# steveschwarcz/Cuda-Path-Tracer-SS

Measured on AMD Instinct MI355X. Metric: Mrays/sec at 1920x1080, 8 bounces, 2072 spp run (BASELINE configs[2] asks 2000 spp; a rate metric); ray = one live ray processed in one bounce, higher is better.
Workload: dtype f32; 1 GPU; configs[2]: 1920x1080 'mixed' preset (22 spheres, 16 triangles, Lambert/Phong/Cook-Torrance/glass/mirror), 8 bounces, 2072 spp = 74 steps x 1 pass(es) x 28 sample lanes per pixel; samples_per_pass=28, frame_lanes=1, lanes_free_run=True, seed=24301

## Files before the change

### cuda-path-tracer-ss_amd/build.py

```python
import os
import shutil
import subprocess
import sys

HERE = os.path.dirname(os.path.abspath(__file__))
ROOT = os.path.dirname(HERE)
INC = os.path.join(ROOT, "include")
CSRC = os.path.join(HERE, "csrc")
HOST = os.path.join(HERE, "host")
LIBDIR = os.path.join(HERE, "lib")

FP_FLAGS = ["-ffp-contract=off", "-fno-fast-math"]
CPU_FLAGS = ["-O2", "-std=c++17", "-fPIC", "-mfma", "-mavx2", "-Wall", "-Wno-unused-function"] + FP_FLAGS
HIP_FLAGS = ["-O3", "-std=c++17", "-fPIC", "--offload-arch=gfx950", "-fhip-fp32-correctly-rounded-divide-sqrt",
             "-fno-gpu-flush-denormals-to-zero", "-fno-slp-vectorize", "-fno-vectorize", "-Wall",
             "-Wno-unused-function"] + FP_FLAGS


def _newer(target, sources):
    if not os.path.exists(target):
        return True
    t = os.path.getmtime(target)
    return any(os.path.getmtime(s) > t for s in sources)


def _run(cmd):
    print("+", " ".join(cmd), flush=True)
    subprocess.check_call(cmd)


def _headers():
    hs = []
    for d in (INC, CSRC, HOST):
        if os.path.isdir(d):
            hs += [os.path.join(d, f) for f in os.listdir(d) if f.endswith(".h")]
    return hs


def build_host(force=False):
    os.makedirs(LIBDIR, exist_ok=True)
    out = os.path.join(LIBDIR, "libptss_host.so")
    srcs = [os.path.join(HOST, f) for f in ("Scene.cpp", "HostOps.cpp", "host_capi.cpp")]
    if force or _newer(out, srcs + _headers()):
        _run(["g++"] + CPU_FLAGS + ["-shared", "-I", INC, "-I", CSRC, "-I", HOST] + srcs + ["-o", out])
    return out


def build_device(force=False, defines=(), name="libptss.so"):
    os.makedirs(LIBDIR, exist_ok=True)
    out = os.path.join(LIBDIR, name)
    srcs = [os.path.join(CSRC, f) for f in sorted(os.listdir(CSRC)) if f.endswith(".hip")]
    hipcc = shutil.which("hipcc") or "/opt/rocm/bin/hipcc"
    if force or _newer(out, srcs + _headers()):
        extra = os.environ.get("PTSS_EXTRA_HIPFLAGS", "").split()
        _run([hipcc] + HIP_FLAGS + extra + ["-D" + d for d in defines] + ["-shared", "-I", INC, "-I", CSRC] + srcs + ["-o", out])
    return out


def build_main(force=False):
    out = os.path.join(LIBDIR, "ptss_main")
    srcs = [os.path.join(HOST, f) for f in ("main.cpp", "CudaTracer.cpp", "MultiGpu.cpp", "Scene.cpp", "HostOps.cpp")]
    if force or _newer(out, srcs + _headers() + [os.path.join(LIBDIR, "libptss.so")]):
        _run(["g++"] + CPU_FLAGS + ["-D__HIP_PLATFORM_AMD__", "-I", INC, "-I", CSRC, "-I", HOST, "-I", "/opt/rocm/include"] + srcs +
             ["-L", LIBDIR, "-lptss", "-L/opt/rocm/lib", "-lamdhip64", "-lrccl", "-Wl,-rpath,$ORIGIN", "-Wl,-rpath,/opt/rocm/lib",
              "-o", out])
    return out


def build_mathcheck(force=False):
    out = os.path.join(LIBDIR, "ptss_mathcheck")
    src = os.path.join(ROOT, "tests", "csrc", "math_exhaustive.hip")
    hipcc = shutil.which("hipcc") or "/opt/rocm/bin/hipcc"
    if force or _newer(out, [src] + _headers()):
        _run([hipcc] + [f for f in HIP_FLAGS if f != "-fPIC"] + ["-I", INC, "-I", CSRC, src, "-o", out])
    return out


def build_all(force=False):
    return [build_host(force), build_device(force), build_main(force), build_mathcheck(force)]


if __name__ == "__main__":
    force = "--force" in sys.argv
    what = [a for a in sys.argv[1:] if not a.startswith("-")]
    table = {"host": build_host, "device": build_device, "main": build_main,
             "mathcheck": build_mathcheck}
    if not what:
        build_all(force)
    for w in what:
        table[w](force)
```

### cuda-path-tracer-ss_amd/csrc/ptmath.h

```cpp
#pragma once
#include <stdint.h>
#include "ptss_types.h"

#if defined(__HIPCC__)
#include <hip/hip_runtime.h>
#define PTM_HD __host__ __device__ __forceinline__
#else
#define PTM_HD inline __attribute__((always_inline))
#endif

namespace ptm {

constexpr float kPi = 3.14159265358979323846f;
constexpr float kInvPi = 0.31830988618f;
constexpr float kRayBump = 1e-4f;
constexpr float kGamma = (1 / 2.2f);

PTM_HD float fma(float a, float b, float c) { return __builtin_fmaf(a, b, c); }
PTM_HD float abs(float x) { return __builtin_fabsf(x); }

#if defined(__HIP_DEVICE_COMPILE__)
PTM_HD unsigned long long lanes(bool directCompare) { return __builtin_amdgcn_ballot_w64(directCompare); }
PTM_HD bool allLanes(unsigned long long m) { return m == __builtin_amdgcn_ballot_w64(true); }
#endif
PTM_HD float sqrt(float x) {
#if defined(__HIP_DEVICE_COMPILE__)
    const float y = __builtin_amdgcn_rsqf(x);
    const float s = x * y;
    const float h = 0.5f * y;
    const float r = __builtin_fmaf(-s, s, x);
    float out = __builtin_fmaf(r, h, s);
    const bool lo = x >= 2.5243549e-29f , hi = x < 7.9228163e28f ;
    if (__builtin_expect(!allLanes(lanes(lo) & lanes(hi)), 0)) out = (lo && hi) ? out : __builtin_sqrtf(x);
    return out;
#else
    return __builtin_sqrtf(x);
#endif
}
PTM_HD float rcp(float x) {
#if defined(__HIP_DEVICE_COMPILE__)
    const float r0 = __builtin_amdgcn_rcpf(x);
    const float e = __builtin_fmaf(-x, r0, 1.0f);
    float out = __builtin_fmaf(e, r0, r0);
    const float ax = __builtin_fabsf(x);
    const bool lo = ax >= 2.3509887e-38f , hi = ax < 8.5070592e37f ;
    if (__builtin_expect(!allLanes(lanes(lo) & lanes(hi)), 0)) out = (lo && hi) ? out : 1.0f / x;
    return out;
#else
    return 1.0f / x;
#endif
}
PTM_HD float rcp_if_above_1em7(float x) {
#if defined(__HIP_DEVICE_COMPILE__)
    const float r0 = __builtin_amdgcn_rcpf(x);
    const float e = __builtin_fmaf(-x, r0, 1.0f);
    float out = __builtin_fmaf(e, r0, r0);
    const bool inRange = __builtin_fabsf(x) < 8.5070592e37f ;
    if (__builtin_expect(!allLanes(lanes(inRange)), 0)) out = inRange ? out : 1.0f / x;
    return out;
#else
    return 1.0f / x;
#endif
}
PTM_HD float rcp_in_range(float x) {
#if defined(__HIP_DEVICE_COMPILE__)
    const float r0 = __builtin_amdgcn_rcpf(x);
    const float e = __builtin_fmaf(-x, r0, 1.0f);
    return __builtin_fmaf(e, r0, r0);
#else
    return 1.0f / x;
#endif
}
PTM_HD uint32_t f2u(float x) { return __builtin_bit_cast(uint32_t, x); }
PTM_HD float u2f(uint32_t x) { return __builtin_bit_cast(float, x); }
PTM_HD float inf() { return u2f(0x7f800000u); }
PTM_HD float qnan() { return u2f(0x7fc00000u); }

#if defined(__HIP_DEVICE_COMPILE__)
PTM_HD bool div_in_range(float x) {
    const float ax = __builtin_fabsf(x);
    return ax >= 8.6736174e-19f  && ax < 1.1529215e18f ;
}
PTM_HD unsigned long long div_range_lanes(float x) {
    const float ax = __builtin_fabsf(x);
    return lanes(ax >= 8.6736174e-19f) & lanes(ax < 1.1529215e18f);
}
PTM_HD float rcp_core(float b) {
    const float r0 = __builtin_amdgcn_rcpf(b);
    const float e = __builtin_fmaf(-b, r0, 1.0f);
    return __builtin_fmaf(e, r0, r0);
}
PTM_HD float div_core(float a, float b, float r) {
    const float q0 = a * r;
    const float rem = __builtin_fmaf(-b, q0, a);
    return __builtin_fmaf(rem, r, q0);
}
#endif
PTM_HD float div(float a, float b) {
#if defined(__HIP_DEVICE_COMPILE__)
    float q = div_core(a, b, rcp_core(b));
    if (__builtin_expect(!allLanes(div_range_lanes(a) & div_range_lanes(b)), 0)) q = (div_in_range(a) && div_in_range(b)) ? q : a / b;
    return q;
#else
    return a / b;
#endif
}
PTM_HD void div3(float ax, float ay, float az, float b, float& qx, float& qy, float& qz) {
#if defined(__HIP_DEVICE_COMPILE__)
    const float r = rcp_core(b);
    qx = div_core(ax, b, r);
    qy = div_core(ay, b, r);
    qz = div_core(az, b, r);
    if (__builtin_expect(!allLanes(div_range_lanes(b) & div_range_lanes(ax) & div_range_lanes(ay) & div_range_lanes(az)), 0)) {
        const bool inRange = div_in_range(b) && div_in_range(ax) && div_in_range(ay) && div_in_range(az);
        qx = inRange ? qx : ax / b;
        qy = inRange ? qy : ay / b;
        qz = inRange ? qz : az / b;
    }
#else
    qx = ax / b;
    qy = ay / b;
    qz = az / b;
#endif
}
PTM_HD float max(float a, float b) { return (a < b) ? b : a; }
PTM_HD float min(float a, float b) { return (b < a) ? b : a; }
PTM_HD float clamp(float x, float lo, float hi) { return min(max(x, lo), hi); }

PTM_HD void sincos(float x, float& s, float& c) {
    if (!(abs(x) <= 1.0e4f)) {
        s = qnan();
        c = qnan();
        return;
    }
    float fn = __builtin_rintf(x * 0.6366197466850281f);
    int n = (int)fn;
    float r = fma(fn, -1.5707963705062866f, x);
    r = fma(fn, 4.371138828673793e-08f, r);
    r = fma(fn, 1.7151245100058819e-15f, r);
    float z = r * r;
    float sp = fma(fma(-1.9515295891e-4f, z, 8.3321608736e-3f), z, -1.6666654611e-1f);
    sp = fma(sp * z, r, r);
    float cp = fma(fma(2.443315711809948e-5f, z, -1.388731625493765e-3f), z, 4.166664568298827e-2f);
    cp = fma(cp * z, z, fma(-0.5f, z, 1.0f));
    float ss = (n & 1) ? cp : sp;
    float cc = (n & 1) ? sp : cp;
    s = (n & 2) ? -ss : ss;
    c = ((n + 1) & 2) ? -cc : cc;
}
PTM_HD float tan(float x) {
    float s, c;
    sincos(x, s, c);
    return div(s, c);
}

PTM_HD float atan(float x) {
    if (x != x) return x;
    float ax = abs(x);
    float y, t;
    if (ax > 2.414213562373095f) {
        y = 1.5707963267948966f;
        t = -rcp(ax);
    } else if (ax > 0.4142135623730950f) {
        y = 0.7853981633974483f;
        t = div(ax - 1.0f, ax + 1.0f);
    } else {
        y = 0.0f;
        t = ax;
    }
    float z = t * t;
    float p = fma(fma(fma(8.05374449538e-2f, z, -1.38776856032e-1f), z, 1.99777106478e-1f), z, -3.33329491539e-1f);
    y = y + fma(p * z, t, t);
    return (x < 0.0f) ? -y : y;
}

PTM_HD float log(float x) {
    if (x != x) return x;
    if (x < 0.0f) return qnan();
    if (x == 0.0f) return -inf();
    if (x == inf()) return x;
    int e = 0;
    if (x < 1.17549435e-38f) {
        x = x * 8388608.0f;
        e = -23;
    }
    uint32_t b = f2u(x);
    e += (int)((b >> 23) & 0xffu) - 126;
    float m = u2f((b & 0x007fffffu) | 0x3f000000u);
    if (m < 0.707106781186547524f) {
        e -= 1;
        m = (m + m) - 1.0f;
    } else {
        m = m - 1.0f;
    }
    float z = m * m;
    float p = 7.0376836292e-2f;
    p = fma(p, m, -1.1514610310e-1f);
    p = fma(p, m, 1.1676998740e-1f);
    p = fma(p, m, -1.2420140846e-1f);
    p = fma(p, m, 1.4249322787e-1f);
    p = fma(p, m, -1.6668057665e-1f);
    p = fma(p, m, 2.0000714765e-1f);
    p = fma(p, m, -2.4999993993e-1f);
    p = fma(p, m, 3.3333331174e-1f);
    float y = (p * m) * z;
    float fe = (float)e;
    y = fma(-2.12194440e-4f, fe, y);
    y = fma(-0.5f, z, y);
    float r = m + y;
    return fma(0.693359375f, fe, r);
}

PTM_HD float exp(float x) {
    if (x != x) return x;
    if (x > 88.72283905206835f) return inf();
    if (x < -87.33654475055310f) return 0.0f;
    float fn = __builtin_rintf(x * 1.4426950216293335f);
    int n = (int)fn;
    float r = fma(fn, -0.693359375f, x);
    r = fma(fn, 2.12194440e-4f, r);
    float z = r * r;
    float p = 1.9875691500e-4f;
    p = fma(p, r, 1.3981999507e-3f);
    p = fma(p, r, 8.3334519073e-3f);
    p = fma(p, r, 4.1665795894e-2f);
    p = fma(p, r, 1.6666665459e-1f);
    p = fma(p, r, 5.0000001201e-1f);
    float y = fma(p, z, r) + 1.0f;
    int h = n / 2;
    float s1 = u2f((uint32_t)(h + 127) << 23);
    float s2 = u2f((uint32_t)((n - h) + 127) << 23);
    return (y * s1) * s2;
}

PTM_HD float pow(float x, float y) {
    if (x != x || y != y) return qnan();
    if (x < 0.0f) return qnan();
    if (y == 0.0f) return 1.0f;
    if (x == 0.0f) return (y > 0.0f) ? 0.0f : inf();
    if (x == 1.0f) return 1.0f;
    return exp(y * log(x));
}

}

namespace ptv {
using vec3 = ::ptss_vec3;
using quat = ::ptss_quat;


PTM_HD vec3 v3(float x, float y, float z) { return vec3{x, y, z}; }
PTM_HD vec3 v3(float s) { return vec3{s, s, s}; }
PTM_HD vec3 operator+(vec3 a, vec3 b) { return vec3{a.x + b.x, a.y + b.y, a.z + b.z}; }
PTM_HD vec3 operator-(vec3 a, vec3 b) { return vec3{a.x - b.x, a.y - b.y, a.z - b.z}; }
PTM_HD vec3 operator-(vec3 a) { return vec3{-a.x, -a.y, -a.z}; }
PTM_HD vec3 operator*(vec3 a, vec3 b) { return vec3{a.x * b.x, a.y * b.y, a.z * b.z}; }
PTM_HD vec3 operator*(vec3 a, float s) { return vec3{a.x * s, a.y * s, a.z * s}; }
PTM_HD vec3 operator*(float s, vec3 a) { return vec3{a.x * s, a.y * s, a.z * s}; }
PTM_HD vec3 operator/(vec3 a, float s) {
    vec3 q;
    ptm::div3(a.x, a.y, a.z, s, q.x, q.y, q.z);
    return q;
}
PTM_HD vec3 madd(vec3 v, float s, vec3 o) { return vec3{ptm::fma(v.x, s, o.x), ptm::fma(v.y, s, o.y), ptm::fma(v.z, s, o.z)}; }
PTM_HD vec3 madd(vec3 a, vec3 b, vec3 o) { return vec3{ptm::fma(a.x, b.x, o.x), ptm::fma(a.y, b.y, o.y), ptm::fma(a.z, b.z, o.z)}; }

PTM_HD float dot(vec3 a, vec3 b) { return ptm::fma(a.z, b.z, ptm::fma(a.y, b.y, a.x * b.x)); }
PTM_HD vec3 cross(vec3 a, vec3 b) {
    return vec3{ptm::fma(a.y, b.z, -(a.z * b.y)), ptm::fma(a.z, b.x, -(a.x * b.z)), ptm::fma(a.x, b.y, -(a.y * b.x))};
}
PTM_HD vec3 normalize(vec3 v) { return v * ptm::rcp(ptm::sqrt(dot(v, v))); }
PTM_HD float length(vec3 v) { return ptm::sqrt(dot(v, v)); }

PTM_HD quat q4(float w, float x, float y, float z) { return quat{x, y, z, w}; }
PTM_HD quat normalize(quat q) {
    float len = ptm::sqrt(ptm::fma(q.w, q.w, ptm::fma(q.z, q.z, ptm::fma(q.y, q.y, q.x * q.x))));
    if (len <= 0.0f) return q4(1, 0, 0, 0);
    float inv = ptm::rcp(len);
    return q4(q.w * inv, q.x * inv, q.y * inv, q.z * inv);
}
PTM_HD vec3 rotate(quat q, vec3 v) {
    vec3 u = v3(q.x, q.y, q.z);
    vec3 uv = cross(u, v);
    vec3 uuv = cross(u, uv);
    uv = uv * (2.0f * q.w);
    uuv = uuv * 2.0f;
    return (v + uv) + uuv;
}
PTM_HD quat mul(quat p, quat q) {
    return q4(p.w * q.w - p.x * q.x - p.y * q.y - p.z * q.z,
              p.w * q.x + p.x * q.w + p.y * q.z - p.z * q.y,
              p.w * q.y + p.y * q.w + p.z * q.x - p.x * q.z,
              p.w * q.z + p.z * q.w + p.x * q.y - p.y * q.x);
}

}
```

### cuda-path-tracer-ss_amd/csrc/ptpack.h

```cpp
#pragma once
#include <stddef.h>
#include <stdint.h>

#include <algorithm>
#include <array>
#include <cmath>
#include <utility>
#include <vector>

#include "ptmath.h"
#include "ptmesh.h"
#include "ptquant.h"
#include "ptscene.h"
#include "ptss_types.h"
#include "pttri.h"

namespace ptpack {
using namespace ptv;
using ptss::SceneLayout;

struct alignas(16) Row {
    float x, y, z, w;
};
static_assert(sizeof(Row) == ptss::kVec4Bytes, "a row is a float4");
// ... 118 lines not shown
            for (size_t q = 0; q < take; ++q) {
                const int b = near[q].second;
                int both[2 * kM], trial[2 * kM], keep[2 * kM];
                for (int j = 0; j < kM; ++j) { both[j] = order[(size_t)a * kM + j]; both[kM + j] = order[(size_t)b * kM + j]; }
                double bestCost = ball[(size_t)a].r * ball[(size_t)a].r + ball[(size_t)b].r * ball[(size_t)b].r;
                const double floor = bestCost * (1 - 1e-9);
                Ball keepA{}, keepB{};
                bool found = false;
                const double join[3] = {ball[(size_t)b].c[0] - ball[(size_t)a].c[0], ball[(size_t)b].c[1] - ball[(size_t)a].c[1], ball[(size_t)b].c[2] - ball[(size_t)a].c[2]};
                const double dirs[7][3] = {{join[0], join[1], join[2]}, {1, 0, 0}, {0, 1, 0}, {0, 0, 1}, {1, 1, 0}, {0, 1, 1}, {1, 0, 1}};
                for (const auto& dir : dirs) {
                    std::copy(both, both + 2 * kM, trial);
                    auto key = [&](int i) { return centre(i, 0) * dir[0] + centre(i, 1) * dir[1] + centre(i, 2) * dir[2]; };
                    std::sort(trial, trial + 2 * kM, [&](int x, int y) { return key(x) < key(y) || (key(x) == key(y) && x < y); });
                    const Ball ta = enclosingBall(s, trial, kM, 48), tb = enclosingBall(s, trial + kM, kM, 48);
                    const double cost = ta.r * ta.r + tb.r * tb.r;
                    if (cost < bestCost && cost < floor) {
                        bestCost = cost; keepA = ta; keepB = tb; found = true;
                        std::copy(trial, trial + 2 * kM, keep);
                    }
                }
                if (found) {
                    for (int j = 0; j < kM; ++j) { order[(size_t)a * kM + j] = keep[j]; order[(size_t)b * kM + j] = keep[kM + j]; }
                    ball[(size_t)a] = keepA; ball[(size_t)b] = keepB;
                    ++improved;
                }
            }
        }
        if (improved == 0) break;
    }
}
inline std::vector<int> spatialOrder(const ptss_scene_desc& s) {
    std::vector<int> order((size_t)s.numSpheres);
    std::vector<Point> centre((size_t)s.numSpheres);
    for (size_t i = 0; i < s.numSpheres; ++i) {
        order[i] = (int)i;
        centre[i] = Point{s.spheres[i].position.x, s.spheres[i].position.y, s.spheres[i].position.z};
    }
    kdOrder(centre, order, 0, (int)s.numSpheres, ptss::kChunkSpheres, 64);
    refineChunks(s, order);
    return order;
}


inline int sphereRowsOf(const SceneLayout& L) { return L.accelSpheres ? L.numChunks * ptss::kChunkSpheres : L.numSpheres; }
inline int sphereAllocOf(const SceneLayout& L) { return L.accelSpheres ? sphereRowsOf(L) : (sphereRowsOf(L) + 3) / 4 * 4; }

inline void setCounts(const ptss_scene_desc& s, bool accel, SceneLayout& L) {
    L.accelSpheres = accel ? 1 : 0;
    L.numChunks = accel ? (int)((s.numSpheres + ptss::kChunkSpheres - 1) / ptss::kChunkSpheres) : 0;
    L.numSpheres = (int)s.numSpheres;
    L.numTriangles = (int)s.numTriangles;
    L.numMaterials = (int)s.numMaterials;
    L.numPointLights = (int)s.numPointLights;
    L.numAreaLights = (int)s.numAreaLights;
}

inline void layoutPlain(const ptss_scene_desc& s, bool accel, SceneLayout& L) {
    setCounts(s, accel, L);
    const int sphereRows = sphereRowsOf(L), sphereAlloc = sphereAllocOf(L);
    int off = 0;
    L.offSphere = off;      off += sphereAlloc;
    if (!accel) { L.offSphereMat = off; off += (sphereRows + 3) / 4; }
    L.offChunk = off;       off += (L.numChunks + 3) / 4 * 4;
    L.offTri = off;         off += 3 * L.numTriangles;
    L.offTriNormal = off;   off += 3 * L.numTriangles;
    L.offTriVert = off;     off += 2 * L.numTriangles;
    L.offMaterial = off;    off += 5 * L.numMaterials;
    L.offPointLight = off;  off += 2 * L.numPointLights;
    L.offAreaLight = off;   off += 2 * L.numAreaLights;
    L.offTriPos = off;      off += (L.numTriangles + 3) / 4;
    L.offQuant = off;       off += ptq::kTableFloats / 4;
    L.offPrimSphere = off;  off += accel ? 0 : sphereAlloc;
    L.offPrimTri = off;     off += 2 * L.numTriangles;
    L.offPrimChunk = off;   off += accel ? (L.numChunks + 3) / 4 * 4 : 0;
    L.ldsVec4 = off;
    if (accel) {
        L.offSphereMat = off;   off += (sphereRows + 3) / 4;
        L.offSphereOrig = off;  off += (sphereRows + 3) / 4;
        L.offSpherePos = off;   off += (L.numSpheres + 3) / 4;
    } else {
        L.offSphereOrig = L.offSpherePos = 0;
    }
    L.totalVec4 = off;
    for (int k = 0; k < 5; ++k) L.triClassPack[k] = 0u;
}

inline void layoutMesh(const ptss_scene_desc& s, SceneLayout& L) {
    setCounts(s, false, L);
    const int sphereRows = sphereRowsOf(L), sphereAlloc = sphereAllocOf(L);
    const int numLeaves = (L.numTriangles + ptss::kMeshLeaf - 1) / ptss::kMeshLeaf;
    const int numGroups = (numLeaves + ptss::kMeshLeaf - 1) / ptss::kMeshLeaf;
    int off = 0;
    L.offSphere = off;      off += sphereAlloc;
    L.offSphereMat = off;   off += (sphereRows + 3) / 4;
    L.offChunk = off;
    const int offGroup = off;   off += 3 * ((numGroups + 3) / 4 * 4);
    const int leafRows = 3 * numLeaves;
    const int rest = 5 * L.numMaterials + 2 * L.numPointLights + 2 * L.numAreaLights + ptq::kTableFloats / 4 + sphereAlloc;
    SceneLayout probe{};
    probe.ldsVec4 = off + leafRows + rest;
    const bool leavesInLds = ptss::bounceLdsBytes(probe, true) <= 64 * 1024;
    int offLeaf = 0;
    if (leavesInLds) { offLeaf = off; off += leafRows; }
    L.offMaterial = off;    off += 5 * L.numMaterials;
    L.offPointLight = off;  off += 2 * L.numPointLights;
    L.offAreaLight = off;   off += 2 * L.numAreaLights;
    L.offQuant = off;       off += ptq::kTableFloats / 4;
    L.offPrimSphere = off;  off += sphereAlloc;
    L.offPrimChunk = off;
    L.ldsVec4 = off;
    if (!leavesInLds) { offLeaf = off; off += leafRows; }
    L.offTri = off;         off += 3 * L.numTriangles;
    L.offTriNormal = off;   off += 3 * L.numTriangles;
    L.offTriVert = off;     off += 2 * L.numTriangles;
    L.offTriPos = off;      off += (L.numTriangles + 3) / 4;
    L.offPrimTri = off;     off += 2 * L.numTriangles;
    L.offSphereOrig = L.offSpherePos = 0;
    L.totalVec4 = off;
    L.mesh.numLeaves = numLeaves;
    L.mesh.numGroups = numGroups;
    L.mesh.offGroup = offGroup;
    L.mesh.offLeaf = offLeaf;
    L.mesh.reserved = 0;
}

inline void setFlags(const ptss_scene_desc& s, SceneLayout& L) {
    auto finite3 = [](const ptss_vec3& v) { return v.x - v.x == 0.0f && v.y - v.y == 0.0f && v.z - v.z == 0.0f; };
    L.neeSkipSafe = 1;
    for (size_t i = 0; i < s.numMaterials; ++i)
        if (!finite3(s.materials[i].diffuseColor) || !(s.materials[i].diffAvg - s.materials[i].diffAvg == 0.0f)) L.neeSkipSafe = 0;
    for (size_t i = 0; i < s.numPointLights; ++i)
        if (!finite3(s.pointLights[i].power)) L.neeSkipSafe = 0;
    for (size_t i = 0; i < s.numAreaLights; ++i)
        if (!finite3(s.areaLights[i].power)) L.neeSkipSafe = 0;
    L.sphereBounded = geometryBounded(s) ? 1 : 0;
    {
        size_t diffuse = 0;
        for (size_t i = 0; i < s.numSpheres; ++i) diffuse += s.materials[s.spheres[i].materialIdx].diffAvg > 0.0f ? 1 : 0;
        for (size_t i = 0; i < s.numTriangles; ++i) diffuse += s.materials[s.triangles[i].materialIdx].diffAvg > 0.0f ? 1 : 0;
        L.neePairs = (L.sphereBounded && s.numPointLights + s.numAreaLights >= 2 && 5 * diffuse >= 4 * (s.numSpheres + s.numTriangles)) ? 1 : 0;
    }
    L.triDetBounded = 1;
    for (size_t i = 0; i < s.numTriangles; ++i) {
        const ptss_triangle& t = s.triangles[i];
        const vec3 e1 = t.vertex1 - t.vertex0, e2 = t.vertex2 - t.vertex0;
        const double n1 = std::sqrt((double)e1.x * e1.x + (double)e1.y * e1.y + (double)e1.z * e1.z);
        const double n2 = std::sqrt((double)e2.x * e2.x + (double)e2.y * e2.y + (double)e2.z * e2.z);
        if (!(n1 * n2 <= 0x1p100)) L.triDetBounded = 0;
    }
    L.triClassed = (L.triDetBounded && L.sphereBounded && L.numTriangles <= 255) ? 1 : 0;
}

inline std::vector<int> orderTriangles(const ptss_scene_desc& s, SceneLayout& L) {
    std::vector<int> triOrder((size_t)L.numTriangles), triCode((size_t)L.numTriangles, 0);
    for (int i = 0; i < L.numTriangles; ++i) {
        triOrder[(size_t)i] = i;
        const ptss_triangle& t = s.triangles[i];
        if (L.triClassed) triCode[(size_t)i] = pttri::triangleClass(t.vertex1 - t.vertex0, t.vertex2 - t.vertex0);
    }
    std::stable_sort(triOrder.begin(), triOrder.end(), [&](int a, int b) { return triCode[(size_t)a] < triCode[(size_t)b]; });
    for (int code = 0, pos = 0; code <= 16 && L.triClassed; ++code) {
        while (pos < L.numTriangles && triCode[(size_t)triOrder[(size_t)pos]] < code) ++pos;
        L.triClassPack[code / 4] |= (uint32_t)pos << (8 * (code % 4));
    }
    if (ptss::meshImage(L)) {
        std::vector<Point> centroid((size_t)L.numTriangles);
        for (int i = 0; i < L.numTriangles; ++i) {
            const ptss_triangle& t = s.triangles[i];
            for (int a = 0; a < 3; ++a) {
                const float* v0 = &t.vertex0.x, *v1 = &t.vertex1.x, *v2 = &t.vertex2.x;
                centroid[(size_t)i][a] = (float)(((double)v0[a] + v1[a] + v2[a]) / 3);
            }
        }
        kdOrder(centroid, triOrder, 0, L.numTriangles, ptss::kMeshLeaf, ptss::kMeshLeaf * ptss::kMeshLeaf);
    }
    return triOrder;
}

inline std::vector<int> packSpheres(const ptss_scene_desc& s, const SceneLayout& L, std::vector<Row>& blob) {
    const bool accel = L.accelSpheres != 0;
    const int sphereRows = sphereRowsOf(L);
    std::vector<int> order;
    if (accel) {
        order = spatialOrder(s);
        while ((int)order.size() < sphereRows) order.push_back(order.back());
    } else {
        order.resize(s.numSpheres);
        for (size_t i = 0; i < s.numSpheres; ++i) order[i] = (int)i;
    }
    for (int i = 0; i < sphereRows; ++i) {
        const ptss_sphere& sp = s.spheres[order[i]];
        blob[L.offSphere + i] = Row{sp.position.x, sp.position.y, sp.position.z, sp.radius * sp.radius};
        intsAt(blob, L.offSphereMat)[i] = sp.materialIdx;
        if (accel) intsAt(blob, L.offSphereOrig)[i] = order[i];
        if (accel && i < L.numSpheres) intsAt(blob, L.offSpherePos)[order[i]] = i;
    }
    return order;
}

inline void packChunkBounds(const ptss_scene_desc& s, const SceneLayout& L, const std::vector<int>& order, std::vector<Row>& blob) {
    for (int k = 0; k < L.numChunks; ++k) {
        const Ball ball = enclosingBall(s, &order[(size_t)k * ptss::kChunkSpheres], ptss::kChunkSpheres, 512);
        const float Cf[3] = {(float)ball.c[0], (float)ball.c[1], (float)ball.c[2]};
        double Rmax = 0;
        for (int j = 0; j < ptss::kChunkSpheres; ++j) {
            const ptss_sphere& sp = s.spheres[order[k * ptss::kChunkSpheres + j]];
            const double dx = (double)sp.position.x - Cf[0], dy = (double)sp.position.y - Cf[1], dz = (double)sp.position.z - Cf[2];
            Rmax = std::max(Rmax, std::sqrt(dx * dx + dy * dy + dz * dz) + std::fabs((double)sp.radius));
        }
        const double infl = Rmax * Rmax * (1 + kAccelM) * (1 + kAccelM) * (1 + kAccelM) * (1 + 4e-6) / (1 - (kAccelM + kAccelM * kAccelM)) * (1 + 1e-9);
        blob[L.offChunk + k] = Row{Cf[0], Cf[1], Cf[2], std::nextafter((float)infl, INFINITY)};
    }
}

inline void packTriangles(const ptss_scene_desc& s, const SceneLayout& L, const std::vector<int>& triOrder, std::vector<Row>& blob) {
    for (int pos = 0; pos < L.numTriangles; ++pos) {
        const int i = triOrder[(size_t)pos];
        const ptss_triangle& t = s.triangles[i];
        const vec3 e1 = t.vertex1 - t.vertex0;
        const vec3 e2 = t.vertex2 - t.vertex0;
        blob[L.offTri + 3 * pos + 0] = Row{t.vertex0.x, t.vertex0.y, t.vertex0.z, u2f((uint32_t)t.materialIdx)};
        blob[L.offTri + 3 * pos + 1] = Row{e1.x, e1.y, e1.z, u2f(0xfffffffeu - (uint32_t)i)};
        blob[L.offTri + 3 * pos + 2] = Row{e2.x, e2.y, e2.z, 0};
        blob[L.offTriNormal + 3 * pos + 0] = Row{t.normal0.x, t.normal0.y, t.normal0.z, 0};
        blob[L.offTriNormal + 3 * pos + 1] = Row{t.normal1.x, t.normal1.y, t.normal1.z, 0};
        blob[L.offTriNormal + 3 * pos + 2] = Row{t.normal2.x, t.normal2.y, t.normal2.z, 0};
        blob[L.offTriVert + 2 * pos + 0] = Row{t.vertex1.x, t.vertex1.y, t.vertex1.z, 0};
        blob[L.offTriVert + 2 * pos + 1] = Row{t.vertex2.x, t.vertex2.y, t.vertex2.z, 0};
        intsAt(blob, L.offTriPos)[i] = pos;
    }
}

inline void packMeshBounds(const ptss_scene_desc& s, const SceneLayout& L, const std::vector<int>& triOrder, std::vector<Row>& blob) {
    auto boundOf = [&](int first, int count, Row* rows) {
        std::vector<float> tri((size_t)count * 9);
        for (int k = 0; k < count; ++k) {
            const ptss_triangle& t = s.triangles[triOrder[(size_t)(first + k)]];
            const vec3 e1 = t.vertex1 - t.vertex0, e2 = t.vertex2 - t.vertex0;
            const float v[9] = {t.vertex0.x, t.vertex0.y, t.vertex0.z, e1.x, e1.y, e1.z, e2.x, e2.y, e2.z};
            std::copy(v, v + 9, tri.begin() + 9 * k);
        }
        float b[12];
        ptmesh::buildBound(tri.data(), count, b);
        for (int r = 0; r < 3; ++r) rows[r] = Row{b[4 * r], b[4 * r + 1], b[4 * r + 2], b[4 * r + 3]};
    };
    constexpr int kGroupTris = ptss::kMeshLeaf * ptss::kMeshLeaf;
    for (int k = 0; k < L.mesh.numLeaves; ++k)
        boundOf(k * ptss::kMeshLeaf, std::min(ptss::kMeshLeaf, L.numTriangles - k * ptss::kMeshLeaf), &blob[(size_t)(L.mesh.offLeaf + 3 * k)]);
    for (int g = 0; g < L.mesh.numGroups; ++g)
        boundOf(g * kGroupTris, std::min(kGroupTris, L.numTriangles - g * kGroupTris), &blob[(size_t)(L.mesh.offGroup + 3 * g)]);
}

inline void packMaterialsAndLights(const ptss_scene_desc& s, const SceneLayout& L, std::vector<Row>& blob) {
    for (int i = 0; i < L.numMaterials; ++i) {
        const ptss_material& m = s.materials[i];
        Row* o = &blob[L.offMaterial + 5 * i];
        o[0] = Row{m.diffuseColor.x, m.diffuseColor.y, m.diffuseColor.z, m.diffAvg};
        o[1] = Row{m.specularColor.x, m.specularColor.y, m.specularColor.z, m.specAvg};
        o[2] = Row{m.absorption.x, m.absorption.y, m.absorption.z, m.refrAvg};
        o[3] = Row{m.emmitance.x, m.emmitance.y, m.emmitance.z, m.roughness};
        o[4] = Row{m.specularExponent, m.indexOfRefraction, u2f((uint32_t)(unsigned char)m.flags), 0};
    }
    for (int i = 0; i < L.numPointLights; ++i) {
        const ptss_point_light& p = s.pointLights[i];
        blob[L.offPointLight + 2 * i + 0] = Row{p.position.x, p.position.y, p.position.z, 0};
        blob[L.offPointLight + 2 * i + 1] = Row{p.power.x, p.power.y, p.power.z, 0};
    }
    for (int i = 0; i < L.numAreaLights; ++i) {
        const ptss_area_light& a = s.areaLights[i];
        const int* triPos = intsAt(blob, L.offTriPos);
        blob[L.offAreaLight + 2 * i] = Row{a.power.x, a.power.y, a.power.z, u2f((uint32_t)triPos[a.triangleIdx])};
        blob[L.offAreaLight + 2 * i + 1] = Row{u2f((uint32_t)triPos[a.triangleIdx + 1]), 0, 0, 0};
    }
}

inline void packScene(const ptss_scene_desc& s, SceneLayout& L, std::vector<Row>& blob, bool accel, bool mesh) {
    if (mesh) layoutMesh(s, L);
    else layoutPlain(s, accel, L);
    setFlags(s, L);
    const std::vector<int> triOrder = orderTriangles(s, L);
    blob.assign((size_t)L.totalVec4 + 1, Row{0, 0, 0, 0});
    ptq::build_thresholds(reinterpret_cast<float*>(&blob[L.offQuant]));
    const std::vector<int> sphereOrder = packSpheres(s, L, blob);
    packChunkBounds(s, L, sphereOrder, blob);
    packTriangles(s, L, triOrder, blob);
    if (mesh) packMeshBounds(s, L, triOrder, blob);
    packMaterialsAndLights(s, L, blob);
}

struct ImagePlan {
    bool accel, mesh;
    int numImages;
};
inline ImagePlan planImages(const ptss_scene_desc& s, bool everySphereLoop) {
    const bool accel = accelEligible(s) && !everySphereLoop;
    const bool mesh = !accel && meshEligible(s) && !everySphereLoop;
    return ImagePlan{accel, mesh, accel ? 2 : 1};
}
struct PackedImage {
    SceneLayout layout{};
    std::vector<Row> blob;
    bool inLds = true;
};
inline std::vector<PackedImage> packImages(const ptss_scene_desc& s, bool everySphereLoop) {
    const ImagePlan plan = planImages(s, everySphereLoop);
// ... 26 lines not shown
```

### cuda-path-tracer-ss_amd/csrc/ptscene.h

```cpp
#pragma once
#include <stddef.h>
#include <stdint.h>

#if defined(__HIPCC__)
#define PTSCENE_HD __host__ __device__
#else
#define PTSCENE_HD
#endif

namespace ptss {

#ifndef PTSS_BLOCK
#define PTSS_BLOCK 256
#endif
#ifndef PTSS_CHUNK
#define PTSS_CHUNK 16
#endif
constexpr int kBlock = PTSS_BLOCK;
constexpr int kChunkSpheres = PTSS_CHUNK;
static_assert((kChunkSpheres & (kChunkSpheres - 1)) == 0, "chunk size must be a power of two");
constexpr int kWaves = kBlock / 64;

struct SceneLayout {
    int numSpheres, numTriangles, numMaterials, numPointLights, numAreaLights;
    int offSphere;
    int offSphereMat;
    int offTri;
    int offTriNormal;
    int offTriVert;
    int offMaterial;
    int offPointLight;
    int offAreaLight;
    int accelSpheres;
    int numChunks;
    int offChunk;
    int offSphereOrig;
    int offSpherePos;
    int offQuant;
    int offPrimSphere;
    int offPrimTri;
    int offPrimChunk;
    int totalVec4;
    int ldsVec4;
    int neeSkipSafe;
    int sphereBounded;
    int neePairs;
    int triDetBounded;
    int triClassed;
    union {
        uint32_t triClassPack[5];
        struct {
            int numLeaves, numGroups;
            int offGroup;
            int offLeaf;
            int reserved;
        } mesh;
    };
    int offTriPos;
};

constexpr int kMeshLeaf = 16;
PTSCENE_HD inline bool meshImage(const SceneLayout& L) { return !L.triClassed && L.mesh.numLeaves > 0; }

constexpr int kNeeLights = 2;
constexpr int kQueueCap = kNeeLights * 64;
constexpr int kWaveLdsWords = 8 * kQueueCap + kNeeLights * 64 / 4;
constexpr int kBlockScratchVec4 = 4;
constexpr int kBlockLdsVec4 = kBlockScratchVec4 + (kWaves * kWaveLdsWords + 3) / 4;

constexpr size_t kVec4Bytes = 16;
inline size_t bounceLdsBytes(const SceneLayout& layout, bool sceneInLds) {
    return ((sceneInLds ? (size_t)layout.ldsVec4 : 0) + kBlockLdsVec4) * kVec4Bytes;
}

}
```

### cuda-path-tracer-ss_amd/csrc/ptshade.h

```cpp
#pragma once
#include "ptaccel.h"
#include "ptquant.h"
#include "ptraypool.h"

namespace ptss {
namespace {

__device__ __forceinline__ void addLambertTerm(vec3& radiance, float cosI, vec3 power, float distance2,
                                               float4 diffuse ) {
    const vec3 L_i = power / (float)(4 * ptm::kPi * distance2);
    radiance.x += cosI * L_i.x * diffuse.x * diffuse.w * ptm::kInvPi;
    radiance.y += cosI * L_i.y * diffuse.y * diffuse.w * ptm::kInvPi;
    radiance.z += cosI * L_i.z * diffuse.z * diffuse.w * ptm::kInvPi;
}

__device__ __forceinline__ quat rotateVectorToVector(vec3 source, vec3 target) {
    const vec3 axis = cross(source, target);
    return normalize(q4(1.0f + dot(source, target), axis.x, axis.y, axis.z));
}

enum LobeKind { kLobeNone = 0, kLobeLambert = 1, kLobePhong = 2, kLobeBeckmann = 3 };

__device__ __forceinline__ vec3 scatter(const float4* mat, RayRegs& ray, vec3 point, vec3 normal, float cosI) {
    const float4 mDiffuse = mat[0];
    const float4 mSpecular = mat[1];
    const float4 mMisc = mat[4];
    const float refrAvg = mat[2].w;
    const int flags = (int)asU(mMisc.z);

    float r = ptrng::uniform(ray.rng);
    PTSS_DIAG_SCATTER(0, true);

    int kind = kLobeNone;
    bool decided = false;
    vec3 axis = normal;
    vec3 result = v3(0, 0, 0);
    const vec3 incident = ray.d;

    if (mDiffuse.w > 0.0f) {
        r -= mDiffuse.w;
        if (r < 0.0f) {
            ray.o = point + ptm::kRayBump * normal;
            kind = kLobeLambert;
            decided = true;
            result = xyz(mDiffuse);
        }
    }

    PTSS_DIAG_SCATTER(1, !decided);
    if (!decided) {
        float n1, n2;
        if (cosI > 0) {
            n2 = mMisc.y;
            n1 = 1.0f;
        } else {
            cosI = -cosI;
            n1 = mMisc.y;
            n2 = 1.0f;
        }
        const bool readsFresnel = (mSpecular.w > 0.0f && !(flags & PTSS_MAT_FLAG_PURE_REFLECTION)) || refrAvg > 0.0f;
        float n = 0.0f, sinT2 = 0.0f;
        float fresnelReflective = 1.0f;
        PTSS_DIAG_SCATTER(2, readsFresnel);
        if (readsFresnel) {
            n = ptm::div(n1, n2);
            sinT2 = n * n * (1.0f - cosI * cosI);
        }
        if (readsFresnel && !(sinT2 > 1.0f)) {
            const float cosT = ptm::sqrt(1.0f - sinT2);
            const float r_s = ptm::div(n1 * cosI - n2 * cosT, n1 * cosI + n2 * cosT);
            const float r_p = ptm::div(n2 * cosI - n1 * cosT, n2 * cosI + n1 * cosT);
            fresnelReflective = (r_s * r_s + r_p * r_p) * 0.5f;
        }

        if (mSpecular.w > 0.0f) {
            if (flags & PTSS_MAT_FLAG_PURE_REFLECTION)
                r -= mSpecular.w;
            else
                r -= mSpecular.w * fresnelReflective;

            if (r < 0.0f) {
                decided = true;
                if (flags & PTSS_MAT_FLAG_COOK_TORRANCE) {
                    kind = kLobeBeckmann;
                } else {
                    ray.d = ray.d - (2 * (-cosI)) * normal;
                    ray.o = point + (normal * ptm::kRayBump);
                    if (mMisc.x != ptm::inf()) {
                        kind = kLobePhong;
                        axis = ray.d;
                    }
                    result = xyz(mSpecular);
                }
            }
        }

        if (!decided && refrAvg > 0.0f) {
            const float fresnelRefractive = 1.0f - fresnelReflective;
            r -= refrAvg * fresnelRefractive;
            PTSS_DIAG_SCATTER(3, r < 0.0f);
            if (r < 0.0f) {
                decided = true;
                if (sinT2 > 1.0f) ray.active = false;
                const float cosT = ptm::sqrt(1.0f - sinT2);
                const vec3 w_o = normalize(n * ray.d + (n * cosI - cosT) * normal);
                ray.o = point + (w_o * ptm::kRayBump);
                ray.d = w_o;
                result = v3(1, 1, 1);
            }
        }

        if (!decided) ray.active = false;
    }

    PTSS_DIAG_SCATTER(4, kind != kLobeNone);
    PTSS_DIAG_SCATTER(5, kind == kLobeBeckmann);
    PTSS_DIAG_SCATTER(6, kind == kLobePhong);
    PTSS_DIAG_SCATTER(7, kind == kLobeLambert);
    if (kind != kLobeNone) {
        const float u1 = ptrng::uniform(ray.rng);
        const float u2 = ptrng::uniform(ray.rng);
        float azimuth, a, y;
        if (kind == kLobeBeckmann) {
            const float roughness = mat[3].w;
            const float theta = ptm::atan(-roughness * roughness * ptm::log(1.0f - u1));
            azimuth = u2 * 2 * ptm::kPi;
            ptm::sincos(theta, a, y);
        } else {
            azimuth = u1 * 2 * ptm::kPi;
            y = (kind == kLobeLambert) ? ptm::sqrt(u2) : ptm::pow(u2, ptm::rcp(mMisc.x + 1));
            a = ptm::sqrt(1 - y * y);
        }
        float sn, cs;
        ptm::sincos(azimuth, sn, cs);
        const vec3 sampled = rotate(rotateVectorToVector(v3(0, 1, 0), axis), v3(a * cs, y, a * sn));
        if (kind == kLobeBeckmann) {
            const vec3 beckmannNormal = sampled;
            const float cosB = ptm::abs(dot(ray.d, beckmannNormal));
            ray.d = ray.d - (2 * (-cosB)) * beckmannNormal;
            ray.o = point + (beckmannNormal * ptm::kRayBump);

            const vec3 half = normalize(ray.d - incident);
            const float nh = ptm::abs(dot(normal, half));
            const float nl = ptm::abs(dot(normal, ray.d));
            const float vh = ptm::abs(dot(incident, half));
            const float nv = ptm::abs(cosI);
            const float geometric = ptm::min(ptm::min(1.0f, ptm::div(2 * nh * nl, vh)), ptm::div(2 * nh * nv, vh));
            result = xyz(mSpecular) * geometric / nv;
        } else {
            ray.d = sampled;
        }
    }
    return result;
}

__device__ __forceinline__ uint32_t quantizeSample(float radiance, const float* T) { return ptq::quantize_fast(radiance, T); }

__device__ __forceinline__ void loadHome(const uint32_t* __restrict__ home, uint32_t p, ptrng::State& s) {
    const uint4 a = reinterpret_cast<const uint4*>(home)[2 * p];
    const uint4 b = reinterpret_cast<const uint4*>(home)[2 * p + 1];
    s.v[0] = a.x; s.v[1] = a.y; s.v[2] = a.z; s.v[3] = a.w;
    s.v[4] = b.x; s.d = b.y;
}
__device__ __forceinline__ void storeHome(uint32_t* __restrict__ home, uint32_t p, const ptrng::State& s) {
    reinterpret_cast<uint4*>(home)[2 * p] = uint4{s.v[0], s.v[1], s.v[2], s.v[3]};
    reinterpret_cast<uint4*>(home)[2 * p + 1] = uint4{s.v[4], s.d, 0u, 0u};
}

struct U3 {
    uint32_t x, y, z;
};

__device__ __forceinline__ void finishPath(const FrameBuffers& fb, const RayRegs& r, const float* quantT) {
    const uint32_t p = pixOf(r.pix), lane = laneOf(r.pix);
    const uint32_t stream = lane * fb.plane + p;
    const uint32_t qx = quantizeSample(r.L0.x, quantT), qy = quantizeSample(r.L0.y, quantT), qz = quantizeSample(r.L0.z, quantT);
    if (fb.samples == 1) {
        U3* acc = reinterpret_cast<U3*>(fb.accum) + p;
        U3 t = *acc;
        t.x += qx;
        t.y += qy;
        t.z += qz;
        *acc = t;
        if (fb.pixels) {
            const uint32_t px = (uint32_t)(unsigned char)(t.x * fb.inverseTicks + 0.5f) |
                                ((uint32_t)(unsigned char)(t.y * fb.inverseTicks + 0.5f) << 8) |
                                ((uint32_t)(unsigned char)(t.z * fb.inverseTicks + 0.5f) << 16) | (255u << 24);
            reinterpret_cast<uint32_t*>(fb.pixels)[p] = px;
        }
    } else {
        fb.staged[stream] = qx | (qy << 8) | (qz << 16);
    }
    if (fb.fsum) {
        float* fs = fb.fsum + 3u * stream;
        fs[0] += r.L0.x;
        fs[1] += r.L0.y;
        fs[2] += r.L0.z;
    }
    storeHome(fb.rngHome, stream, r.rng);
}

constexpr unsigned long long kPeerWaitTicks = 200000000ull;
__device__ __forceinline__ bool peerWaitExpired(unsigned long long& since) {
    const unsigned long long now = wall_clock64();
    if (since == 0ull) {
        since = now | 1ull;
        return false;
    }
    return now > since && now - since > kPeerWaitTicks;
}

__device__ __forceinline__ uint32_t frameLiveCount(const FrameBuffers& fb, int bounce, uint32_t own, const uint32_t* target) {
    uint32_t total = own;
    for (uint32_t p = 0; p < fb.numPeers; ++p) {
        unsigned long long since = 0ull;
        for (;;) {
            uint32_t ended = 0;
            for (int s = 0; s < kShards; ++s)
                ended += __hip_atomic_load(fb.peerDone[p] + countIndex(bounce - 1, s), __ATOMIC_ACQUIRE, __HIP_MEMORY_SCOPE_AGENT);
            if ((int32_t)(ended - target[p]) >= 0) break;
            __builtin_amdgcn_s_sleep(64);
            if (peerWaitExpired(since)) {
                if (threadIdx.x == 0) atomicAdd(fb.guardTimeouts, 1u);
                break;
            }
        }
        for (int s = 0; s < kShards; ++s)
            total += __hip_atomic_load(fb.peerCounts[p] + countIndex(bounce, s), __ATOMIC_RELAXED, __HIP_MEMORY_SCOPE_AGENT);
    }
    return total;
}

}
}
```

### cuda-path-tracer-ss_amd/csrc/ptss_api.hip

```cpp
#include <stdio.h>
#include <stdlib.h>
#include <string.h>

#include <new>
#include <string>
#include <vector>

#include "ptss.h"
#include "ptss_device.h"
#include <algorithm>
#include "ptdenoise.h"
#include "ptreproject.h"
#include "ptspecular.h"
#include "ptpack.h"

using namespace ptv;
using ptpack::cameraInRange;
static_assert(sizeof(ptpack::Row) == sizeof(float4) && alignof(ptpack::Row) == alignof(float4), "a packed row is uploaded as a float4");

#if PTSS_DIAG
namespace ptss { hipError_t readDiagCounters(unsigned long long* out8); }
#endif
namespace {

thread_local std::string g_detail;

int fail(int code, const char* what, hipError_t e = hipSuccess) {
    char buf[512];
    if (e != hipSuccess)
        snprintf(buf, sizeof(buf), "%s: %s (%s)", what, hipGetErrorString(e), hipGetErrorName(e));
    else
        snprintf(buf, sizeof(buf), "%s", what);
    g_detail = buf;
    return code;
}

#define HIP_TRY(expr)                                        \
    do {                                                     \
        hipError_t _e = (expr);                              \
        if (_e != hipSuccess) return fail(PTSS_EHIP, #expr, _e); \
    } while (0)

#define RC_TRY(expr) do { if (int _rc = (expr)) return _rc; } while (0)

struct EventPair {
    hipEvent_t a, b;
};

}

struct Lane {
    hipStream_t stream = nullptr;
    float* dPool[2] = {nullptr, nullptr};
    uint32_t* dCounts[2] = {nullptr, nullptr};
    uint32_t* dShardCount0 = nullptr;
    uint32_t* dLastCounts = nullptr;
    uint32_t* dDone = nullptr;
    uint32_t doneTarget[ptss::kMaxBounces + 1] = {};
    hipEvent_t evDone[2] = {nullptr, nullptr};
    uint32_t regionCap = 0;
    int maxBlocks = 0;
    uint32_t hint[ptss::kMaxBounces + 1] = {0};
    bool haveHint = false;
    uint32_t* hCounts = nullptr;
    hipEvent_t hintEvent[4] = {nullptr, nullptr, nullptr, nullptr};
    bool hintPending[4] = {false, false, false, false};
};

struct SceneImage {
    float4* dBlob = nullptr;
    ptss::SceneLayout layout{};
    bool inLds = true;
    bool oneLaunch = false;
};

struct ptss_context {
    ptss_render_config cfg{};
    hipStream_t stream = nullptr;
    ptss::TileMap tile{};
    SceneImage images[2];
    int active = 0;
    const SceneImage& image() const { return images[active]; }
    std::vector<Lane> lanes;
    hipEvent_t evFork = nullptr;
    int countParity = 0;
    uint32_t* dRngHome = nullptr;
    unsigned long long* dTotal = nullptr;
    uint32_t* dAccumOwned = nullptr;
    uint32_t* dAccum = nullptr;
    float* dFsum = nullptr;
    uint32_t* dStaged = nullptr;
    bool stagedTwice = false;
    hipEvent_t evDisplay[2] = {nullptr, nullptr};
    uint32_t capacity = 0, numPixels = 0;
    uint32_t samples = 1;
    bool cameraDirty = true;
    float defaultColor[3] = {0, 0, 0};
    ptss_camera camera{};
    int lastResetTick = 0;
    int lastTicks = 0;
    unsigned maxIterations = 15;
    bool resetTicksThisFrame = true;
    bool usePathTracer = true;
    hipEvent_t evStart = nullptr, evStop = nullptr;
    float lastMs = 0.0f;
    int gridCap = 0;
    unsigned frameIndex = 0;
    std::vector<EventPair> evFree, evBusy;
    std::vector<std::pair<double, double>> kernelSpans;
    hipEvent_t evEpoch = nullptr;
    unsigned int timeoutsSeen = 0;
    unsigned long long launchedKernels = 0;
    unsigned long long specularFeatureLaunches[2] = {0, 0};
    float4* dDenoise[2] = {nullptr, nullptr};
    int denoiseLastPlane = -1;
    int denoiseLastLevel = -1;
    hipStream_t denoiseStream = nullptr;
    int numCUs = 0;
    hipStream_t updateStream = nullptr;
    bool updated = false;
};
constexpr int kTotalWords = ptss::kMaxLanes + 8 + 1;
constexpr int kRejectedWord = ptss::kMaxLanes;

namespace {

int validateScene(const ptss_scene_desc& s) {
    const char* what = ptpack::validateScene(s);
    return what ? fail(PTSS_EINVAL, what) : PTSS_OK;
}

int localRows(const ptss_render_config& cfg) {
    int rows = 0;
    for (int y = 0; y < cfg.height; ++y)
        if ((y / cfg.bandRows) % cfg.tileWorld == cfg.tileRank) ++rows;
    return rows;
}

int createCheck(hipError_t e, const char* what) { return e == hipSuccess ? PTSS_OK : fail(e == hipErrorOutOfMemory ? PTSS_ENOMEM : PTSS_EHIP, what, e); }
#define ALLOC_TRY(expr) RC_TRY(createCheck((expr), #expr))
template <class T>
hipError_t mallocZeroed(T** p, size_t bytes) {
    const hipError_t e = hipMalloc(p, bytes);
    return e == hipSuccess ? hipMemset(*p, 0, bytes) : e;
}

struct SceneState {
    SceneImage images[2];
    int gridCap = 0;
    float defaultColor[3] = {0, 0, 0};
};
void releaseSceneState(SceneState& st) {
    for (SceneImage& im : st.images) {
        (void)hipFree(im.dBlob);
        im = SceneImage{};
    }
}
int buildSceneState(const ptss_scene_desc& scene, const ptss_render_config& cfg, int numLanes, int maxBlocks0, int numCUs, SceneState& st) {
    std::vector<ptpack::PackedImage> packed;
    try {
        packed = ptpack::packImages(scene, cfg.everySphereLoop != 0);
    } catch (const std::bad_alloc&) {
        return fail(PTSS_ENOMEM, "scene image (host)");
    }
    const int numImages = (int)packed.size();
    for (int i = 0; i < numImages; ++i) {
        SceneImage& im = st.images[i];
        im.layout = packed[(size_t)i].layout;
        im.inLds = packed[(size_t)i].inLds;
        const std::vector<ptpack::Row>& blob = packed[(size_t)i].blob;
        hipError_t e = hipMalloc(&im.dBlob, blob.size() * sizeof(float4));
        if (e == hipSuccess) e = hipMemcpy(im.dBlob, blob.data(), blob.size() * sizeof(float4), hipMemcpyHostToDevice);
        if (e != hipSuccess) {
            releaseSceneState(st);
            return createCheck(e, "scene image (device)");
        }
    }
    st.defaultColor[0] = scene.defaultColor.x;
    st.defaultColor[1] = scene.defaultColor.y;
    st.defaultColor[2] = scene.defaultColor.z;
    const SceneImage& primary = st.images[0];
    const int perCU = ptss::bounceOccupancyBlocksPerCU(primary.layout, primary.inLds, primary.layout.sphereBounded != 0);
    st.gridCap = numCUs * (perCU > 0 ? perCU : 4) * 16 / ptss::kShards;
    auto qualifies = [&](const SceneImage& im) {
        if (cfg.oneLaunchFrames <= 0 || numLanes != 1 || !im.inLds) return false;
        if (ptss::meshImage(im.layout)) return false;
        int perCU = ptss::frameOccupancyBlocksPerCU(im.layout, false);
        if (im.layout.sphereBounded) perCU = std::min(perCU, ptss::frameOccupancyBlocksPerCU(im.layout, true));
        const int resident = perCU - 1;
        return resident >= 1 && maxBlocks0 <= numCUs * resident;
    };
    for (int i = 0; i < numImages; ++i) st.images[i].oneLaunch = qualifies(st.images[i]);
#ifdef PTSS_TUNING_KNOBS
    if (const char* e = getenv("PTSS_SCENE_PATH")) {
        if (!strcmp(e, "scalar"))
            for (int i = 0; i < numImages; ++i) st.images[i].inLds = false;
    }
    if (const char* e = getenv("PTSS_GRID_CAP")) st.gridCap = atoi(e);
#endif
    return PTSS_OK;
}
void adoptSceneState(ptss_context* c, const SceneState& st) {
    for (int i = 0; i < 2; ++i) c->images[i] = st.images[i];
    c->gridCap = st.gridCap;
    for (int k = 0; k < 3; ++k) c->defaultColor[k] = st.defaultColor[k];
    c->active = 0;
}

int allocLane(Lane& ln, const uint32_t (&shardCount0)[ptss::kShards], bool ownStream) {
    const size_t poolBytes = (size_t)ptss::kRayPlanes * ln.regionCap * ptss::kShards * sizeof(float);
    for (float*& pool : ln.dPool) ALLOC_TRY(hipMalloc(&pool, poolBytes));
    for (uint32_t*& counts : ln.dCounts) ALLOC_TRY(mallocZeroed(&counts, ptss::kCountWords * sizeof(uint32_t)));
    ALLOC_TRY(mallocZeroed(&ln.dLastCounts, ptss::kCountWords * sizeof(uint32_t)));
    for (int s = 0; s < ptss::kShards; ++s)
        ALLOC_TRY(hipMemcpy(ln.dCounts[0] + ptss::countIndex(0, s), &shardCount0[s], sizeof(uint32_t), hipMemcpyHostToDevice));
    ALLOC_TRY(hipMalloc(&ln.dShardCount0, sizeof(shardCount0)));
    ALLOC_TRY(hipMemcpy(ln.dShardCount0, shardCount0, sizeof(shardCount0), hipMemcpyHostToDevice));
    ALLOC_TRY(mallocZeroed(&ln.dDone, (ptss::kCountWords + ptss::kCountStride) * sizeof(uint32_t)));
    if (ownStream) {
        ALLOC_TRY(hipStreamCreateWithFlags(&ln.stream, hipStreamNonBlocking));
        for (hipEvent_t& ev : ln.evDone) ALLOC_TRY(hipEventCreateWithFlags(&ev, hipEventDisableTiming));
    }
    ALLOC_TRY(hipHostMalloc(&ln.hCounts, 4 * ptss::kCountWords * sizeof(uint32_t), hipHostMallocDefault));
    for (hipEvent_t& ev : ln.hintEvent) ALLOC_TRY(hipEventCreateWithFlags(&ev, hipEventDisableTiming));
    return PTSS_OK;
}
#undef ALLOC_TRY

hipError_t seedStreams(ptss_context* c, unsigned long long seed, hipStream_t st) {
    std::vector<uint32_t> table(ptrng::kJumpTableWords);
    ptrng::build_subsequence_table(table.data());
    uint32_t* dTable = nullptr;
    hipError_t e = hipMalloc(&dTable, table.size() * sizeof(uint32_t));
    if (e != hipSuccess) return e;
    e = hipMemcpy(dTable, table.data(), table.size() * sizeof(uint32_t), hipMemcpyHostToDevice);
    if (e == hipSuccess && c->numPixels > 0) e = ptss::launchRngInit(st, c->dRngHome, c->capacity, c->samples, c->tile, seed, dTable);
    if (e == hipSuccess) e = hipStreamSynchronize(st);
    (void)hipFree(dTable);
    return e;
}

int quiesce(ptss_context* c) {
    HIP_TRY(hipStreamSynchronize(c->stream));
    for (const Lane& ln : c->lanes)
        if (ln.stream) HIP_TRY(hipStreamSynchronize(ln.stream));
    return PTSS_OK;
}

void releaseLane(Lane& ln) {
    for (hipEvent_t ev : ln.hintEvent)
        if (ev) (void)hipEventDestroy(ev);
    if (ln.hCounts) (void)hipHostFree(ln.hCounts);
    (void)hipFree(ln.dDone);
    for (hipEvent_t ev : ln.evDone)
        if (ev) (void)hipEventDestroy(ev);
    if (ln.stream) (void)hipStreamDestroy(ln.stream);
    for (float* pool : ln.dPool) (void)hipFree(pool);
    for (uint32_t* counts : ln.dCounts) (void)hipFree(counts);
    (void)hipFree(ln.dShardCount0);
    (void)hipFree(ln.dLastCounts);
}

ptss::FrameBuffers frameBuffers(const ptss_context* c, int laneIdx, ptss_uchar4* pixels, int sample) {
    const Lane& ln = c->lanes[(size_t)laneIdx];
    ptss::FrameBuffers fb{};
    fb.pool[0] = ln.dPool[0];
    fb.pool[1] = ln.dPool[1];
    fb.rngHome = c->dRngHome;
    fb.counts = ln.dCounts[c->countParity];
    fb.countsNext = ln.dCounts[1 - c->countParity];
    fb.shardCount0 = ln.dShardCount0;
    fb.lastCounts = ln.dLastCounts;
    fb.totalRayBounces = c->dTotal + laneIdx;
    fb.guardTimeouts = reinterpret_cast<uint32_t*>(c->dTotal + ptss::kMaxLanes + 8);
    fb.accum = c->dAccum;
    fb.fsum = c->dFsum;
    fb.staged = c->dStaged ? c->dStaged + (c->stagedTwice ? (size_t)(c->frameIndex & 1u) * c->capacity * c->samples : 0) : nullptr;
    fb.quantTable = reinterpret_cast<const float*>(c->image().dBlob + c->image().layout.offQuant);
    fb.pixels = pixels;
    fb.regionCap = ln.regionCap;
    fb.numPixels = c->numPixels;
    fb.plane = c->capacity;
    fb.samples = c->samples;
    fb.firstTiles = c->samples * (c->capacity / ptss::kBlock);
    fb.minLive = c->tile.world > 1 ? 0u : ptss::kMinLiveRays;
    fb.inverseTicks = 1.f / (float)((int)c->samples * (sample + 1));
    fb.defaultColor[0] = c->defaultColor[0];
    fb.defaultColor[1] = c->defaultColor[1];
    fb.defaultColor[2] = c->defaultColor[2];
    fb.laneIndex = (uint32_t)laneIdx;
    fb.laneCount = (uint32_t)c->lanes.size();
    fb.frameRays = c->numPixels * c->samples;
    fb.numPeers = fb.laneCount - 1;
    fb.myDone = ln.dDone;
    fb.myFrameDone = ln.dDone + ptss::kCountWords;
    fb.frameSeq = c->frameIndex;
    fb.joinsFrame = (laneIdx + 1 == (int)c->lanes.size()) ? 1u : 0u;
    uint32_t p = 0;
    for (size_t k = 0; k < c->lanes.size(); ++k) {
        if ((int)k == laneIdx) continue;
        fb.peerCounts[p] = c->lanes[k].dCounts[c->countParity];
        fb.peerDone[p] = c->lanes[k].dDone;
        fb.peerFrameDone[p] = c->lanes[k].dDone + ptss::kCountWords;
        ++p;
    }
    return fb;
}

void drainKernelEvents(ptss_context* c, bool wait) {
    size_t k = 0;
    for (size_t i = 0; i < c->evBusy.size(); ++i) {
        EventPair p = c->evBusy[i];
        hipError_t q = wait ? hipEventSynchronize(p.b) : hipEventQuery(p.b);
        if (q == hipSuccess) {
            float start = 0, ms = 0;
            if (hipEventElapsedTime(&start, c->evEpoch, p.a) == hipSuccess && hipEventElapsedTime(&ms, p.a, p.b) == hipSuccess)
            {
                if (c->kernelSpans.size() >= (1u << 20)) c->kernelSpans.clear();
                c->kernelSpans.emplace_back((double)start, (double)start + (double)ms);
            }
            c->evFree.push_back(p);
        } else {
            c->evBusy[k++] = p;
        }
    }
    c->evBusy.resize(k);
    (void)hipGetLastError();
}

int checkLaneTimeouts(ptss_context* c) {
    if (c->lanes.size() < 2 && !c->images[0].oneLaunch && !c->images[1].oneLaunch) return PTSS_OK;
    uint32_t v = 0;
    HIP_TRY(hipMemcpy(&v, c->dTotal + ptss::kMaxLanes + 8, sizeof(v), hipMemcpyDeviceToHost));
    if (v != c->timeoutsSeen) {
        c->timeoutsSeen = v;
        return fail(PTSS_ETIMEOUT, "a bounded wait on the device expired (a frame lane for a peer lane, or a workgroup of the one-launch "
                                   "frame kernel for its shard): the frame was not traced as specified");
    }
    return PTSS_OK;
}

void selectImage(ptss_context* c) {
    if (!c->images[1].dBlob) return;
    const int want = cameraInRange(c->camera) ? 0 : 1;
    if (want != c->active) {
        c->active = want;
        c->cameraDirty = true;
    }
}

ptss::EyeParams eyeParams(const ptss_context* c) {
    return {c->camera, -2 * ptm::tan(c->camera.fieldOfView * 0.5f), (float)c->tile.height / (float)c->tile.width, 1.0f / c->tile.width,
            1.0f / c->tile.height};
}

void harvestHints(ptss_context* c) {
    for (Lane& ln : c->lanes)
        for (int q = 0; q < 4; ++q) {
            if (!ln.hintPending[q] || hipEventQuery(ln.hintEvent[q]) != hipSuccess) continue;
            const uint32_t* src = ln.hCounts + (size_t)q * ptss::kCountWords;
            for (int b = 0; b <= ptss::kMaxBounces; ++b) {
                uint32_t mx = 0;
                for (int s = 0; s < ptss::kShards; ++s) mx = std::max(mx, src[ptss::countIndex(b, s)]);
                ln.hint[b] = mx;
            }
            ln.haveHint = true;
            ln.hintPending[q] = false;
        }
    (void)hipGetLastError();
}

int forkLanes(ptss_context* c, bool forkNeeded) {
    if (c->lanes.size() > 1 && (forkNeeded || c->frameIndex == 0 || !c->cfg.lanesFreeRun)) {
        HIP_TRY(hipEventRecord(c->evFork, c->stream));
        for (Lane& ln : c->lanes) HIP_TRY(hipStreamWaitEvent(ln.stream, c->evFork, 0));
    }
    if (c->stagedTwice && c->frameIndex >= 2)
        for (Lane& ln : c->lanes) HIP_TRY(hipStreamWaitEvent(ln.stream, c->evDisplay[c->frameIndex & 1u], 0));
    return PTSS_OK;
}

template <class Launch>
int timedLaunch(ptss_context* c, hipStream_t s, Launch launch) {
    if (!c->cfg.timeKernels) return launch();
    EventPair ev{nullptr, nullptr};
    if (c->evFree.empty() && c->evBusy.size() >= 4096) drainKernelEvents(c, true);
    if (c->evFree.empty()) {
        HIP_TRY(hipEventCreate(&ev.a));
        HIP_TRY(hipEventCreate(&ev.b));
    } else {
        ev = c->evFree.back();
        c->evFree.pop_back();
    }
    HIP_TRY(hipEventRecord(ev.a, s));
    RC_TRY(launch());
    HIP_TRY(hipEventRecord(ev.b, s));
    c->evBusy.push_back(ev);
    return PTSS_OK;
}

int traceOneLaunch(ptss_context* c, const ptss::FrameBuffers& fb, int numIterations, bool bounded, const ptss::EyeParams& eye) {
    const SceneImage& im = c->image();
    return timedLaunch(c, c->stream, [&] {
        HIP_TRY(ptss::launchFrame(c->stream, fb, im.dBlob, im.layout, numIterations, bounded, c->lanes[0].maxBlocks, c->tile, eye,
                                          &c->launchedKernels));
        return PTSS_OK;
    });
}

int traceBounces(ptss_context* c, ptss::FrameBuffers* fbs, int numIterations, bool bounded, const ptss::EyeParams& eye) {
    const SceneImage& im = c->image();
    const int K = (int)c->lanes.size();
    for (int i = 0; i < numIterations; ++i)
        for (int k = 0; k < K; ++k) {
            Lane& ln = c->lanes[(size_t)k];
            const hipStream_t ls = K > 1 ? ln.stream : c->stream;
            int blocks = ln.maxBlocks;
            if (i > 0 && ln.haveHint) {
                const unsigned long long tilesPerShard = ((unsigned long long)ln.hint[i] * 65 / 64 + ptss::kBlock) / ptss::kBlock + 1;
                const unsigned long long want = tilesPerShard * ptss::kShards;
                if (want < (unsigned long long)blocks) blocks = (int)want;
            }
            if (c->gridCap > 0 && c->gridCap * ptss::kShards < blocks) blocks = c->gridCap * ptss::kShards;
            if (i > 0)
                for (int j = 0, p = 0; j < K; ++j)
                    if (j != k) fbs[k].peerTarget[p++] = c->lanes[(size_t)j].doneTarget[i - 1];
            RC_TRY(timedLaunch(c, ls, [&] {
                HIP_TRY(ptss::launchBounce(ls, fbs[k], im.dBlob, im.layout, i, i == numIterations - 1, im.inLds, bounded, blocks, c->tile, eye,
                                               &c->launchedKernels));
                return PTSS_OK;
            }));
            ln.doneTarget[i] += (uint32_t)blocks;
        }
    return PTSS_OK;
}

int flushAndJoin(ptss_context* c, const ptss::FrameBuffers* fbs, int numIterations) {
    const int K = (int)c->lanes.size();
    for (int k = 0; k < K; ++k) {
        Lane& ln = c->lanes[(size_t)k];
        const hipStream_t ls = K > 1 ? ln.stream : c->stream;
        ptss::FlushTargets targets{};
// ... 319 lines not shown
    HIP_TRY(hipMalloc(out, (size_t)c->capacity * sizeof(ptss_uchar4)));
    HIP_TRY(hipMemset(*out, 0, (size_t)c->capacity * sizeof(ptss_uchar4)));
    return PTSS_OK;
}

int ptss_free_pixels(ptss_context* c, ptss_uchar4* dev) {
    if (!c) return fail(PTSS_EINVAL, "ctx is null");
    HIP_TRY(hipFree(dev));
    return PTSS_OK;
}

int ptss_local_pixels(const ptss_context* c, size_t* out) {
    if (!c || !out) return fail(PTSS_EINVAL, "null argument");
    *out = c->numPixels;
    return PTSS_OK;
}

int ptss_local_rows(const ptss_context* c, int* rows, int cap, int* count) {
    if (!c || !count) return fail(PTSS_EINVAL, "null argument");
    int n = 0;
    for (int y = 0; y < c->tile.height; ++y) {
        if ((y / c->tile.bandRows) % c->tile.world != c->tile.rank) continue;
        if (rows) {
            if (n >= cap) return fail(PTSS_ERANGE, "rows[] too small");
            rows[n] = y;
        }
        ++n;
    }
    *count = n;
    return PTSS_OK;
}

int ptss_synchronize(ptss_context* c) {
    if (!c) return fail(PTSS_EINVAL, "ctx is null");
    HIP_TRY(hipStreamSynchronize(c->stream));
    return checkLaneTimeouts(c);
}

int ptss_read_accumulator(ptss_context* c, uint32_t* host, size_t count) {
    if (!c || !host) return fail(PTSS_EINVAL, "null argument");
    if (count != (size_t)3 * c->numPixels) return fail(PTSS_ERANGE, "count must be 3 * local pixels");
    HIP_TRY(hipStreamSynchronize(c->stream));
    HIP_TRY(hipMemcpy(host, c->dAccum, count * sizeof(uint32_t), hipMemcpyDeviceToHost));
    return checkLaneTimeouts(c);
}

int ptss_read_float_accumulator(ptss_context* c, float* host, size_t count) {
    if (!c || !host) return fail(PTSS_EINVAL, "null argument");
    if (!c->dFsum) return fail(PTSS_EINVAL, "context was created without floatAccumulator");
    if (count != (size_t)3 * c->numPixels) return fail(PTSS_ERANGE, "count must be 3 * local pixels");
    HIP_TRY(hipStreamSynchronize(c->stream));
    if (c->samples == 1) {
        HIP_TRY(hipMemcpy(host, c->dFsum, count * sizeof(float), hipMemcpyDeviceToHost));
    } else {
        std::vector<float> lane(count);
        for (size_t k = 0; k < count; ++k) host[k] = 0.0f;
        for (uint32_t l = 0; l < c->samples; ++l) {
            HIP_TRY(hipMemcpy(lane.data(), c->dFsum + (size_t)3 * l * c->capacity, count * sizeof(float), hipMemcpyDeviceToHost));
            for (size_t k = 0; k < count; ++k) host[k] = host[k] + lane[k];
        }
    }
    return checkLaneTimeouts(c);
}

int ptss_read_pixels(ptss_context* c, const ptss_uchar4* dev, ptss_uchar4* host, size_t count) {
    if (!c || !dev || !host) return fail(PTSS_EINVAL, "null argument");
    if (count > c->numPixels) return fail(PTSS_ERANGE, "count exceeds local pixels");
    HIP_TRY(hipStreamSynchronize(c->stream));
    HIP_TRY(hipMemcpy(host, dev, count * sizeof(ptss_uchar4), hipMemcpyDeviceToHost));
    return checkLaneTimeouts(c);
}

int ptss_read_rng_state(ptss_context* c, size_t local_pixel, uint32_t* out6) { return ptss_read_rng_state_lane(c, local_pixel, 0, out6); }

int ptss_read_rng_state_lane(ptss_context* c, size_t local_pixel, unsigned int lane, uint32_t* out6) {
    if (!c || !out6) return fail(PTSS_EINVAL, "null argument");
    if (local_pixel >= c->numPixels || lane >= c->samples) return fail(PTSS_ERANGE, "pixel or lane out of range");
    HIP_TRY(hipStreamSynchronize(c->stream));
    HIP_TRY(hipMemcpy(out6, c->dRngHome + (size_t)ptss::kHomeWords * ((size_t)lane * c->capacity + local_pixel), 6 * sizeof(uint32_t),
                      hipMemcpyDeviceToHost));
    return PTSS_OK;
}

int ptss_last_pass_ms(ptss_context* c, float* out) {
    if (!c || !out) return fail(PTSS_EINVAL, "null argument");
    *out = c->lastMs;
    return PTSS_OK;
}

int ptss_samples_since_reset(const ptss_context* c, int* out) {
    if (!c || !out) return fail(PTSS_EINVAL, "null argument");
    *out = c->resetTicksThisFrame ? 0 : (c->lastTicks - c->lastResetTick + 1) * (int)c->samples;
    return PTSS_OK;
}

int ptss_live_counts(ptss_context* c, uint32_t* out, int cap, int* n) {
    if (!c || !out || !n) return fail(PTSS_EINVAL, "null argument");
    const int numIterations = c->usePathTracer ? (int)c->maxIterations : 1;
    if (cap < numIterations) return fail(PTSS_ERANGE, "out[] too small");
    std::vector<uint32_t> raw(ptss::kCountWords), sum(ptss::kCountWords, 0u);
    HIP_TRY(hipStreamSynchronize(c->stream));
    for (const Lane& ln : c->lanes) {
        HIP_TRY(hipMemcpy(raw.data(), ln.dLastCounts, raw.size() * sizeof(uint32_t), hipMemcpyDeviceToHost));
        for (size_t k = 0; k < raw.size(); ++k) sum[k] += raw[k];
    }
    bool stopped = false;
    for (int i = 0; i < numIterations; ++i) {
        uint32_t total = 0;
        for (int s = 0; s < ptss::kShards; ++s) total += sum[ptss::countIndex(i, s)];
        if (total <= (c->tile.world > 1 ? 0u : ptss::kMinLiveRays)) stopped = true;
        out[i] = stopped ? 0u : total;
    }
    *n = numIterations;
    return checkLaneTimeouts(c);
}

int ptss_total_ray_bounces(ptss_context* c, unsigned long long* out) {
    if (!c || !out) return fail(PTSS_EINVAL, "null argument");
    HIP_TRY(hipStreamSynchronize(c->stream));
    unsigned long long perLane[ptss::kMaxLanes];
    HIP_TRY(hipMemcpy(perLane, c->dTotal, sizeof(perLane), hipMemcpyDeviceToHost));
    *out = 0;
    for (size_t k = 0; k < c->lanes.size(); ++k) *out += perLane[k];
    return checkLaneTimeouts(c);
}

int ptss_guard_timeouts(ptss_context* c, unsigned int* out) {
    if (!c || !out) return fail(PTSS_EINVAL, "null argument");
    HIP_TRY(hipStreamSynchronize(c->stream));
    uint32_t v = 0;
    HIP_TRY(hipMemcpy(&v, c->dTotal + ptss::kMaxLanes + 8, sizeof(v), hipMemcpyDeviceToHost));
    *out = v;
    return PTSS_OK;
}

int ptss_one_launch_frames(const ptss_context* c, int* out) {
    if (!c || !out) return fail(PTSS_EINVAL, "null argument");
    *out = (c->image().oneLaunch && c->lanes.size() == 1) ? 1 : 0;
    return PTSS_OK;
}

int ptss_frame_lanes(const ptss_context* c, int* out) {
    if (!c || !out) return fail(PTSS_EINVAL, "null argument");
    *out = (int)c->lanes.size();
    return PTSS_OK;
}

int ptss_launched_kernels(const ptss_context* c, unsigned long long* out) {
    if (!c || !out) return fail(PTSS_EINVAL, "null argument");
    *out = c->launchedKernels;
    return PTSS_OK;
}

static int rayQuery(ptss_context* c, bool any, const ptss_ray_query* rays, void* out, size_t n, void* hipStream) {
    if (!c) return fail(PTSS_EINVAL, "ctx is null");
    if (n == 0) return PTSS_OK;
    if (!rays || !out) return fail(PTSS_EINVAL, "null buffer with n > 0");
    if (n >= (size_t(1) << 31)) return fail(PTSS_ERANGE, "n must be below 2^31");
    if (((uintptr_t)rays | (uintptr_t)out) & (any ? 3u : 15u) || (uintptr_t)rays & 15u)
        return fail(PTSS_EINVAL, "rays and hits must be 16-byte aligned, verdicts 4-byte aligned");
    const SceneImage& im = c->images[0];
    if (!im.dBlob) return fail(PTSS_EINVAL, "context has no scene image");
    HIP_TRY(hipSetDevice(c->cfg.device));
    hipStream_t st = hipStream ? static_cast<hipStream_t>(hipStream) : c->stream;
    HIP_TRY(ptss::launchQuery(st, any, im.dBlob, im.layout, im.inLds, rays, out, (uint32_t)n, c->gridCap * ptss::kShards,
                              &c->launchedKernels));
    return PTSS_OK;
}

int ptss_intersect(ptss_context* c, const ptss_ray_query* dev_rays, ptss_ray_hit* dev_hits, size_t n, void* hipStream) {
    return rayQuery(c, false, dev_rays, dev_hits, n, hipStream);
}

int ptss_occluded(ptss_context* c, const ptss_ray_query* dev_rays, uint32_t* dev_occluded, size_t n, void* hipStream) {
    return rayQuery(c, true, dev_rays, dev_occluded, n, hipStream);
}

int ptss_render_features(ptss_context* c, ptss_pixel_feature* dev_features, void* hipStream) {
    if (!c) return fail(PTSS_EINVAL, "ctx is null");
    if (!dev_features) return fail(PTSS_EINVAL, "dev_features is null");
    if ((uintptr_t)dev_features & 15u) return fail(PTSS_EINVAL, "dev_features must be 16-byte aligned");
    if (c->numPixels == 0) return PTSS_OK;
    const SceneImage& im = c->images[0];
    if (!im.dBlob) return fail(PTSS_EINVAL, "context has no scene image");
    HIP_TRY(hipSetDevice(c->cfg.device));
    hipStream_t st = hipStream ? static_cast<hipStream_t>(hipStream) : c->stream;
    const ptss_vec3 defaultColor{c->defaultColor[0], c->defaultColor[1], c->defaultColor[2]};
    HIP_TRY(ptss::launchFeatures(st, im.dBlob, im.layout, im.inLds, c->tile, eyeParams(c), defaultColor, dev_features, c->numPixels,
                                 c->gridCap * ptss::kShards, &c->launchedKernels));
    return PTSS_OK;
}

int ptss_render_features_motion(ptss_context* c, const ptss_triangle* dev_triangles_prev, size_t first, size_t count,
                                ptss_pixel_feature* dev_features, ptss_pixel_motion* dev_motion, void* hipStream) {
    if (!c) return fail(PTSS_EINVAL, "ctx is null");
    if (!dev_features || !dev_motion) return fail(PTSS_EINVAL, "dev_features or dev_motion is null");
    if (count > 0 && !dev_triangles_prev) return fail(PTSS_EINVAL, "dev_triangles_prev is null with count > 0");
    if (((uintptr_t)dev_features | (uintptr_t)dev_motion) & 15u) return fail(PTSS_EINVAL, "dev_features and dev_motion must be 16-byte aligned");
    if ((uintptr_t)dev_triangles_prev & 3u) return fail(PTSS_EINVAL, "dev_triangles_prev must be 4-byte aligned");
    if (count > 0) {
        const size_t T = (size_t)c->images[0].layout.numTriangles;
        if (first >= T || count > T - first) return fail(PTSS_ERANGE, "first .. first + count - 1 leaves the scene's triangles");
    }
    if (c->numPixels == 0) return PTSS_OK;
    const SceneImage& im = c->images[0];
    if (!im.dBlob) return fail(PTSS_EINVAL, "context has no scene image");
    HIP_TRY(hipSetDevice(c->cfg.device));
    hipStream_t st = hipStream ? static_cast<hipStream_t>(hipStream) : c->stream;
    const ptss_vec3 defaultColor{c->defaultColor[0], c->defaultColor[1], c->defaultColor[2]};
    HIP_TRY(ptss::launchFeaturesMotion(st, im.dBlob, im.layout, im.inLds, c->tile, eyeParams(c), defaultColor, dev_features, c->numPixels,
                                       c->gridCap * ptss::kShards, dev_triangles_prev, count ? (uint32_t)first : 0u, (uint32_t)count, dev_motion,
                                       &c->launchedKernels));
    return PTSS_OK;
}

int ptss_render_features_specular(ptss_context* c, int maxSteps, ptss_pixel_feature* dev_features, uint32_t* dev_steps, void* hipStream) {
    if (!c) return fail(PTSS_EINVAL, "ctx is null");
    if (!dev_features) return fail(PTSS_EINVAL, "dev_features is null");
    if (maxSteps < 0 || maxSteps > ptsp::kMaxSteps) return fail(PTSS_EINVAL, "maxSteps must be in [0, 8]");
    if (((uintptr_t)dev_features & 15u) || ((uintptr_t)dev_steps & 3u))
        return fail(PTSS_EINVAL, "dev_features must be 16-byte aligned, dev_steps 4-byte aligned");
    if (c->numPixels == 0) return PTSS_OK;
    const SceneImage& im = c->images[0];
    if (!im.dBlob) return fail(PTSS_EINVAL, "context has no scene image");
    HIP_TRY(hipSetDevice(c->cfg.device));
    hipStream_t st = hipStream ? static_cast<hipStream_t>(hipStream) : c->stream;
    const ptss_vec3 defaultColor{c->defaultColor[0], c->defaultColor[1], c->defaultColor[2]};
    HIP_TRY(ptss::launchFeaturesSpecular(st, im.dBlob, im.layout, im.inLds, c->tile, eyeParams(c), defaultColor, dev_features, dev_steps,
                                         c->numPixels, maxSteps, c->gridCap * ptss::kShards, c->specularFeatureLaunches));
    return PTSS_OK;
}

int ptss_specular_feature_launches(const ptss_context* c, unsigned long long* out2) {
    if (!c || !out2) return fail(PTSS_EINVAL, "null argument");
    out2[0] = c->specularFeatureLaunches[0];
    out2[1] = c->specularFeatureLaunches[1];
    return PTSS_OK;
}

int ptss_default_denoise_params(ptss_denoise_params* p) {
    if (!p) return fail(PTSS_EINVAL, "params is null");
    p->structSize = (unsigned int)sizeof(*p);
    p->levels = 5;
    p->sigmaColor = 64.0f;
    p->sigmaNormal = 0.1f;
    p->sigmaDepth = 4.0f;
    return PTSS_OK;
}

static int denoisePasses(ptss_context* c, const char* what, const void* input, bool fromAccumulator, const ptss_pixel_feature* dev_features,
                         const ptss_denoise_params* params, ptss_uchar4* dev_out, void* hipStream) {
    if (!c) return fail(PTSS_EINVAL, "ctx is null");
    if (!dev_features || !params || !dev_out || (!fromAccumulator && !input)) return fail(PTSS_EINVAL, "null argument");
    if (params->structSize != (unsigned int)sizeof(ptss_denoise_params))
        return fail(PTSS_EINVAL, "params->structSize is not this library's sizeof(ptss_denoise_params): start from ptss_default_denoise_params");
    if (params->levels < 0 || params->levels > PTSS_DENOISE_MAX_LEVELS) return fail(PTSS_EINVAL, "levels must be in [0, 6]");
    if (!(params->sigmaColor > 0.0f) || !(params->sigmaNormal > 0.0f) || !(params->sigmaDepth >= 0.0f))
        return fail(PTSS_EINVAL, "sigmaColor and sigmaNormal must be positive, sigmaDepth not negative");
    if (((uintptr_t)dev_features & 15u) || ((uintptr_t)dev_out & 3u)) return fail(PTSS_EINVAL, "dev_features must be 16-byte aligned, dev_out 4-byte aligned");
    if (!fromAccumulator && ((uintptr_t)input & 15u)) return fail(PTSS_EINVAL, "dev_history must be 16-byte aligned");
    if (c->tile.world > 1)
        return fail(PTSS_EINVAL, (std::string(what) + " needs the whole frame: this context is a pixel-band shard (tileWorld > 1), whose bands of "
                                                       "rows have no neighbours to filter with").c_str());
    if (fromAccumulator) input = c->dAccum;
    HIP_TRY(hipSetDevice(c->cfg.device));
    hipStream_t st = hipStream ? static_cast<hipStream_t>(hipStream) : c->stream;
    const int levels = params->levels;
    if (levels >= 2)
        for (float4*& plane : c->dDenoise)
            if (!plane) {
                const hipError_t e = hipMalloc(&plane, (size_t)c->numPixels * sizeof(float4));
                if (e != hipSuccess) return fail(e == hipErrorOutOfMemory ? PTSS_ENOMEM : PTSS_EHIP, "ptss_denoise: colour planes", e);
            }
    const float inverseTicks = 1.f / (float)((int)c->samples * (c->lastTicks - c->lastResetTick + 1));
    const int width = c->tile.width, height = c->tile.height;
    c->denoiseLastPlane = levels >= 2 ? (levels - 2) & 1 : -1;
    c->denoiseLastLevel = levels - 2;
    c->denoiseStream = st;
    for (int i = 0; i < (levels > 0 ? levels : 1); ++i) {
        const bool first = i == 0, last = i + 1 >= levels;
        const void* src = first ? input : c->dDenoise[(i - 1) & 1];
        void* dst = last ? static_cast<void*>(dev_out) : c->dDenoise[i & 1];
        HIP_TRY(ptss::launchDenoise(st, first && fromAccumulator, last, src, dst, dev_features, width, height, ptdn::levelOf(*params, i), inverseTicks,
                                    &c->launchedKernels));
    }
    return PTSS_OK;
}

int ptss_denoise(ptss_context* c, const ptss_pixel_feature* dev_features, const ptss_denoise_params* params, ptss_uchar4* dev_out,
                 void* hipStream) {
    return denoisePasses(c, "ptss_denoise", nullptr, true, dev_features, params, dev_out, hipStream);
}

int ptss_denoise_history(ptss_context* c, const ptss_history_entry* dev_history, const ptss_pixel_feature* dev_features,
                         const ptss_denoise_params* params, ptss_uchar4* dev_out, void* hipStream) {
    return denoisePasses(c, "ptss_denoise_history", dev_history, false, dev_features, params, dev_out, hipStream);
}

int ptss_default_reproject_params(ptss_reproject_params* p) {
    if (!p) return fail(PTSS_EINVAL, "params is null");
    p->structSize = (unsigned int)sizeof(*p);
    p->cosNormal = 0.9f;
    p->depthTolerance = 0.02f;
    p->maxHistory = 64.0f;
    p->minCoverage = 0.25f;
    return PTSS_OK;
// ... 203 lines not shown
```

### cuda-path-tracer-ss_amd/csrc/ptss_device.h

```cpp
#pragma once
#include <hip/hip_runtime.h>
#include <stdint.h>

#include "ptmath.h"
#include "ptscene.h"
#include "ptss_types.h"
#include "xorwow.h"

namespace ptdn { struct Level; }
namespace ptrp { struct View; struct Params; }

namespace ptss {

enum RayPlane : int {
    kOx = 0, kOy, kOz,
    kDx, kDy, kDz,
    kL0x, kL0y, kL0z,
    kTx, kTy, kTz,
    kPix,
    kR0, kR1, kR2, kR3, kR4,
    kRd,
    kRayPlanes
};
constexpr int kHomeWords = 8;
constexpr int kMaxBounces = 64;
#ifndef PTSS_SHARDS
#define PTSS_SHARDS 16
#endif
#ifndef PTSS_MINWAVES
#define PTSS_MINWAVES 7
#endif
#ifndef PTSS_MINWAVES_BOUNDED
#define PTSS_MINWAVES_BOUNDED 6
#endif
#ifndef PTSS_MINWAVES_FIRST
#define PTSS_MINWAVES_FIRST 6
#endif
#ifndef PTSS_ABLATE
#define PTSS_ABLATE 0
#endif
#ifndef PTSS_DIAG
#define PTSS_DIAG 0
#endif
constexpr int kShards = PTSS_SHARDS;
constexpr int kCountStride = 32;
constexpr int kCountWords = (kMaxBounces + 1) * kShards * kCountStride;
__host__ __device__ inline int countIndex(int bounce, int shard) { return (bounce * kShards + shard) * kCountStride; }
constexpr uint32_t kMinLiveRays = 128;

struct TileMap {
    int width, height;
    int localRows;
    int rank, world, bandRows;
};

struct EyeParams {
    ptss_camera camera;
    float s;
    float aspect;
    float invW, invH;
};

constexpr int kMaxLanes = 4;

struct FrameBuffers {
    float* pool[2];
    uint32_t* rngHome;
    uint32_t* counts;
    uint32_t* countsNext;
    const uint32_t* shardCount0;
    uint32_t* lastCounts;
    unsigned long long* totalRayBounces;
    uint32_t* accum;
    float* fsum;
    const float* quantTable;
    uint32_t* staged;
    ptss_uchar4* pixels;
    uint32_t regionCap;
    uint32_t numPixels;
    uint32_t plane;
    uint32_t samples;
    uint32_t firstTiles;
    uint32_t minLive;
    float inverseTicks;
    float defaultColor[3];
    uint32_t laneIndex, laneCount;
    uint32_t frameRays;
    uint32_t numPeers;
    const uint32_t* peerCounts[kMaxLanes - 1];
    const uint32_t* peerDone[kMaxLanes - 1];
    uint32_t peerTarget[kMaxLanes - 1];
    uint32_t* myDone;
    uint32_t* myFrameDone;
    const uint32_t* peerFrameDone[kMaxLanes - 1];
    uint32_t frameSeq;
    uint32_t joinsFrame;
    uint32_t* guardTimeouts;
};

inline void markLaunched(unsigned long long* launched, int base, int index = 0) { *launched |= 1ull << (base + index); }
hipError_t launchRngInit(hipStream_t st, uint32_t* rngHome, uint32_t plane, uint32_t samples, TileMap tile, uint64_t seed,
                         const uint32_t* jumpTable);
hipError_t launchDisplay(hipStream_t st, const FrameBuffers& fb);
hipError_t launchClear(hipStream_t st, const FrameBuffers& fb);
hipError_t launchPrimaryPrep(hipStream_t st, float4* sceneBlob, const SceneLayout& layout, ptss_vec3 origin);
hipError_t launchBounce(hipStream_t st, const FrameBuffers& fb, const float4* sceneBlob, SceneLayout layout, int bounce,
                        bool isLast, bool sceneInLds, bool bounded, int gridBlocks, TileMap tile, EyeParams eye, unsigned long long* launched);
hipError_t launchFrame(hipStream_t st, const FrameBuffers& fb, const float4* sceneBlob, SceneLayout layout, int numBounces, bool bounded, int gridBlocks,
                       TileMap tile, EyeParams eye, unsigned long long* launched);
int frameOccupancyBlocksPerCU(const SceneLayout& layout, bool bounded);
struct FlushTargets {
    uint32_t target[kMaxLanes - 1][kMaxBounces + 1];
};
hipError_t launchFlush(hipStream_t st, const FrameBuffers& fb, int numBounces, const FlushTargets& targets);
int bounceOccupancyBlocksPerCU(const SceneLayout& layout, bool sceneInLds, bool bounded);
hipError_t launchQuery(hipStream_t st, bool any, const float4* sceneBlob, SceneLayout layout, bool sceneInLds, const void* rays, void* out,
                       uint32_t n, int maxBlocks, unsigned long long* launched);
hipError_t launchFeatures(hipStream_t st, const float4* sceneBlob, SceneLayout layout, bool sceneInLds, TileMap tile, EyeParams eye,
                          ptss_vec3 defaultColor, void* out, uint32_t n, int maxBlocks, unsigned long long* launched);
hipError_t launchFeaturesMotion(hipStream_t st, const float4* sceneBlob, SceneLayout layout, bool sceneInLds, TileMap tile, EyeParams eye,
                                ptss_vec3 defaultColor, void* out, uint32_t n, int maxBlocks, const void* prevRecords, uint32_t first,
                                uint32_t count, void* motionOut, unsigned long long* launched);
hipError_t launchFeaturesSpecular(hipStream_t st, const float4* sceneBlob, SceneLayout layout, bool sceneInLds, TileMap tile, EyeParams eye,
                                  ptss_vec3 defaultColor, void* out, void* steps, uint32_t n, int maxSteps, int maxBlocks,
                                  unsigned long long* launches);
hipError_t launchDenoise(hipStream_t st, bool first, bool last, const void* src, void* dst, const void* features, int width, int height,
                         const ptdn::Level& level, float inverseTicks, unsigned long long* launched);
hipError_t launchSceneUpdate(hipStream_t st, float4* sceneBlob, const SceneLayout& layout, const void* records, uint32_t first, uint32_t count,
                             unsigned long long* rejected, unsigned long long* launched);
hipError_t launchMeshRefit(hipStream_t st, float4* sceneBlob, const SceneLayout& layout, unsigned long long* launched);
hipError_t launchReproject(hipStream_t st, const uint32_t* accum, const void* featuresNow, const void* featuresPrev, const void* historyPrev,
                           void* historyOut, int width, int height, const ptrp::View& now, const ptrp::View& prev, const ptrp::Params& params,
                           float inverseTicks, float n, unsigned long long* launched);
hipError_t launchReprojectMotion(hipStream_t st, const uint32_t* accum, const void* featuresNow, const void* motionNow, const void* featuresPrev,
                                 const void* historyPrev, void* historyOut, int width, int height, const ptrp::View& now, const ptrp::View& prev,
                                 const ptrp::Params& params, float inverseTicks, float n, unsigned long long* launched);

}
```

### cuda-path-tracer-ss_amd/csrc/ptss_diag.h

```cpp
#pragma once

#if PTSS_DIAG
__device__ unsigned long long g_diag[8];
#endif

#if PTSS_DIAG & 1
__device__ __forceinline__ void diagCandidates(uint32_t mask, bool live, int slot) {
    const uint32_t pc = (uint32_t)__builtin_popcount(mask);
    uint32_t mx = 0;
    while (__any(pc > mx)) ++mx;
    uint32_t total = 0;
    for (uint32_t b = 0; b < 6; ++b) total += (uint32_t)__popcll(__ballot((pc >> b) & 1u)) << b;
    if (__lane_id() == 0) {
        atomicAdd(&g_diag[slot + 0], (unsigned long long)mx);
        atomicAdd(&g_diag[slot + 1], (unsigned long long)total);
        atomicAdd(&g_diag[slot + 2], 1ull);
        atomicAdd(&g_diag[slot + 3], (unsigned long long)__popcll(__ballot(live)));
    }
}
#define PTSS_DIAG_CANDIDATES(mask, live, slot) diagCandidates(mask, live, slot)
#else
#define PTSS_DIAG_CANDIDATES(mask, live, slot) do {} while (0)
#endif

#if PTSS_DIAG & 2
#define PTSS_DIAG_SCATTER(k, cond)                                                             \
    do {                                                                                       \
        const unsigned long long _m = __ballot(cond);                                          \
        if (_m != 0ull && __lane_id() == (unsigned)(__ffsll((long long)__ballot(true)) - 1)) { \
            atomicAdd(&g_diag[k], 1ull + ((unsigned long long)__popcll(_m) << 32));            \
        }                                                                                      \
    } while (0)
#else
#define PTSS_DIAG_SCATTER(k, cond) do {} while (0)
#endif

#if PTSS_DIAG & 4
__device__ __forceinline__ void diagCull(const float4* sc, const SceneLayout& L, vec3 o, vec3 d, bool unitDir, bool live, unsigned long long won) {
    const float T = (won == ~0ull) ? ptm::inf() : asF((uint32_t)(won >> 32));
    uint32_t touched = 0, needed = 0;
    for (int g = 0; g < L.numChunks && g < 128; g += 32) {
        const int left = L.numChunks - g;
        const uint32_t bits = live ? chunkMask<false>(sc + L.offChunk + g, left < 32 ? left : 32, o, d, unitDir) : 0u;
        uint32_t rev = 0;
        const int trips = ((left < 32 ? left : 32) + 3) >> 2;
        for (int q = 0; q < 4 * trips; ++q) {
            const float4 b = sc[L.offChunk + g + q];
            const vec3 v = o - xyz(b);
            const float dv = dot(d, v), vv = dot(v, v), a = -dv - T;
            const bool ahead = unitDir && (a > 0.0f) && ((a * a) * (1.0f - 2e-5f) > (1.0f - kAccelMu) * b.w + kAccelMu * vv);
            rev |= ahead ? 0u : (1u << q);
        }
        touched += (uint32_t)__builtin_popcount(bits);
        needed += (uint32_t)__builtin_popcount(bits & rev);
    }
    uint32_t st = 0, sn = 0;
    for (uint32_t bit = 0; bit < 7; ++bit) {
        st += (uint32_t)__popcll(__ballot((touched >> bit) & 1u)) << bit;
        sn += (uint32_t)__popcll(__ballot((needed >> bit) & 1u)) << bit;
    }
    const uint32_t hits = (uint32_t)__popcll(__ballot(live && won != ~0ull));
    const uint32_t rays = (uint32_t)__popcll(__ballot(live));
    if (__lane_id() == 0) {
        atomicAdd(&g_diag[0], (unsigned long long)st);
        atomicAdd(&g_diag[1], (unsigned long long)sn);
        atomicAdd(&g_diag[2], (unsigned long long)rays);
        atomicAdd(&g_diag[3], (unsigned long long)hits);
    }
}
#define PTSS_DIAG_CULL(sc, L, o, d, unitDir, live, won) diagCull(sc, L, o, d, unitDir, live, won)
#else
#define PTSS_DIAG_CULL(sc, L, o, d, unitDir, live, won) do {} while (0)
#endif

#if PTSS_DIAG & 8
#define PTSS_DIAG_PAIRS(needA, needB, lit)                                                                              \
    do {                                                                                                                \
        const unsigned long long _mb = __ballot((needA) && (needB)), _mo = __ballot((needA) != (needB)), _ml = __ballot(lit); \
        if (__lane_id() == 0) {                                                                                         \
            atomicAdd(&g_diag[4], (unsigned long long)__popcll(_mb));                                                   \
            atomicAdd(&g_diag[5], (unsigned long long)__popcll(_mo));                                                   \
            atomicAdd(&g_diag[6], (unsigned long long)__popcll(_ml));                                                   \
            atomicAdd(&g_diag[7], 1ull);                                                                                \
        }                                                                                                               \
    } while (0)
#else
#define PTSS_DIAG_PAIRS(needA, needB, lit) do {} while (0)
#endif

#if PTSS_DIAG & 16
#define PTSS_DIAG_QUEUE(queued)                                                                                               \
    do {                                                                                                                      \
        if (__lane_id() == 0)                                                                                                 \
            atomicAdd(&g_diag[(queued) == 0 ? 0 : ((queued) <= 8 ? 1 : ((queued) <= 16 ? 2 : ((queued) <= 32 ? 3 : ((queued) <= 64 ? 4 : ((queued) <= 72 ? 5 : ((queued) <= 96 ? 6 : 7))))))], 1ull); \
    } while (0)
#else
#define PTSS_DIAG_QUEUE(queued) do {} while (0)
#endif
```

### cuda-path-tracer-ss_amd/csrc/ptss_kernels.hip

```cpp
#include "ptss_device.h"
#include "ptmotion.h"
#include "ptspecular.h"
#include "pthit.h"
#include "ptshade.h"

#include <array>
#include <utility>

namespace ptss {

__global__ void rngInitKernel(uint32_t* __restrict__ rngHome, uint32_t plane, uint32_t samples, TileMap tile, uint64_t seed,
                              const uint32_t* __restrict__ jumpTable) {
    const uint32_t i = blockIdx.x * blockDim.x + threadIdx.x;
    const uint32_t n = (uint32_t)tile.width * (uint32_t)tile.localRows;
    const uint32_t lane = i / plane, p = i - lane * plane;
    if (lane >= samples || p >= n) return;
    const PixelCoord pc = locate(tile, p);
    ptrng::State s = ptrng::seeded(seed);
    ptrng::skip_subsequences(s, pc.globalIndex * samples + lane, jumpTable);
    storeHome(rngHome, i, s);
}

__global__ void clearKernel(FrameBuffers fb) {
    const uint32_t i = blockIdx.x * blockDim.x + threadIdx.x;
// ... 33 lines not shown
        t.y += (q >> 8) & 255u;
        t.z += (q >> 16) & 255u;
    }
    reinterpret_cast<U3*>(fb.accum)[p] = t;
    if (fb.pixels) {
        const uint32_t px = (uint32_t)(unsigned char)(t.x * fb.inverseTicks + 0.5f) |
                            ((uint32_t)(unsigned char)(t.y * fb.inverseTicks + 0.5f) << 8) |
                            ((uint32_t)(unsigned char)(t.z * fb.inverseTicks + 0.5f) << 16) | (255u << 24);
        reinterpret_cast<uint32_t*>(fb.pixels)[p] = px;
    }
}

__global__ void primaryPrepKernel(float4* __restrict__ blob, SceneLayout L, vec3 origin) {
    const int i = blockIdx.x * blockDim.x + threadIdx.x;
    if (i < L.numSpheres && !L.accelSpheres) {
        const float4 sp = blob[L.offSphere + i];
        const vec3 v = origin - xyz(sp);
        blob[L.offPrimSphere + i] = float4{v.x, v.y, v.z, dot(v, v) - sp.w};
    }
    if (L.accelSpheres && i < L.numChunks) {
        const float4 b = blob[L.offChunk + i];
        const vec3 v = origin - xyz(b);
        const float x = dot(v, v) - b.w;
        blob[L.offPrimChunk + i] = float4{v.x, v.y, v.z, x - ptm::abs(x) * 2.4e-7f};
    }
    if (i < L.numTriangles) {
        const vec3 v0 = xyz(blob[L.offTri + 3 * i]), e1 = xyz(blob[L.offTri + 3 * i + 1]), e2 = xyz(blob[L.offTri + 3 * i + 2]);
        const vec3 s = origin - v0;
        const vec3 r = cross(s, e1);
        blob[L.offPrimTri + 2 * i] = float4{s.x, s.y, s.z, dot(e2, r)};
        blob[L.offPrimTri + 2 * i + 1] = float4{r.x, r.y, r.z, 0.0f};
    }
}

struct TileEnv {
    const float4* sc;
    const float4* sceneBlob;
    const float* quantT;
    const float* in;
    float* out;
    float* wq;
    uint32_t* wqOwner;
    unsigned char* wqAnswer;
    uint32_t shard, lane, n;
    int numLights, bounce;
};

template <bool kLast, bool kFirst, bool kAccel, bool kBounded, bool kPairs, bool kCoherentIo, bool kMesh = false>
__device__ __forceinline__ void bounceTile(const FrameBuffers& fb, const SceneLayout& L, const TileMap& tile, const EyeParams& eye, const TileEnv& env,
                                           uint32_t base) {
    const float4* sc = env.sc;
    const float4* sceneBlob = env.sceneBlob;
    const float* quantT = env.quantT;
    const float* __restrict__ in = env.in;
    float* __restrict__ out = env.out;
    float* wq = env.wq;
    uint32_t* wqOwner = env.wqOwner;
    unsigned char* wqAnswer = env.wqAnswer;
    const uint32_t shard = env.shard, lane = env.lane, n = env.n;
    const int numLights = env.numLights, bounce = env.bounce;
    {
        const uint32_t i = base + threadIdx.x;
        uint32_t firstPixel = 0, firstLane = 0;
        bool valid = i < n;
        if constexpr (kFirst) {
            const uint32_t start = (((base / kBlock) * fb.laneCount + fb.laneIndex) * kShards + shard) * kBlock;
            firstLane = start / fb.plane;
            firstPixel = start - firstLane * fb.plane + threadIdx.x;
            valid = firstPixel < fb.numPixels;
        }

        RayRegs ray;
        ray.o = ray.d = ray.L0 = ray.T = v3(0, 0, 0);
        ray.pix = 0;
        ray.active = false;
        if constexpr (kFirst) {
            if (valid) {
                const uint32_t pixel = firstPixel;
                const PixelCoord pc = locate(tile, pixel);
                loadHome(fb.rngHome, firstLane * fb.plane + pixel, ray.rng);
                const float jitteredX = pc.x + ptrng::uniform(ray.rng);
                const float jitteredY = pc.gy + ptrng::uniform(ray.rng);
                const vec3 start = v3(((jitteredX * eye.invW) - 0.5f) * eye.s,
                                      1 * ((jitteredY * eye.invH) - 0.5f) * eye.s * eye.aspect, 1.0f) *
                                   eye.camera.zNear;
                ray.o = eye.camera.position;
                ray.d = normalize(rotate(eye.camera.rotation, start));
                ray.L0 = v3(0, 0, 0);
                ray.T = v3(1, 1, 1);
                ray.pix = pixel | (firstLane << kLaneShift);
                ray.active = true;
            }
        } else {
            if (valid) loadRayGeometry<kCoherentIo>(tileBlock(in, base), threadIdx.x, ray);
        }
#if PTSS_ABLATE & 2
        Hit h;
        h.kind = 2; h.idx = (int)(pixOf(ray.pix) % (uint32_t)L.numTriangles); h.distance = 1.0f + ray.d.x;
        h.w0 = 0.3f; h.w1 = 0.3f; h.w2 = 0.4f;
#else
        const Hit h = closestHit<kFirst, kAccel, kBounded, kMesh>(sc, sceneBlob, L, ray.o, ray.d, valid, reinterpret_cast<uint32_t*>(wq));
#endif
        const bool hit = valid && h.kind != 0;
        if constexpr (!kFirst) {
            if (valid) loadRayRng<kCoherentIo>(tileBlock(in, base), threadIdx.x, ray);
        }
        const float4* td = kMesh ? sceneBlob : sc;
        vec3 point = v3(0, 0, 0), normal = v3(0, 0, 0);
        float cosI = 0;
        int materialIdx = 0;
        if (hit) {
            point = ray.o + ray.d * h.distance;
            if (h.kind == 1) {
                normal = normalize(point - xyz(loadRow16(sc + L.offSphere + h.idx)));
                materialIdx = reinterpret_cast<const int*>((kAccel ? sceneBlob : sc) + L.offSphereMat)[h.idx];
            } else {
                const float4* nn = td + L.offTriNormal + 3 * h.idx;
                normal = (xyz(loadRow16(nn)) * h.w0 + xyz(loadRow16(nn + 1)) * h.w1) + xyz(loadRow16(nn + 2)) * h.w2;
                materialIdx = (int)asU(td[L.offTri + 3 * h.idx].w);
            }
            cosI = dot(-ray.d, normal);
        }
        const bool inside = cosI <= 0.0f;
        const bool lit = hit && !inside && !(PTSS_ABLATE & 1);
        const float4* mat = sc + L.offMaterial + 5 * materialIdx;

        vec3 radiance = v3(0, 0, 0);
        for (int l0 = 0; l0 < numLights; l0 += kNeeLights) {
            uint32_t queued = 0;
            bool need[kNeeLights];
            float cosL[kNeeLights], distance2[kNeeLights];
            [[maybe_unused]] vec3 pairW[kNeeLights];
            [[maybe_unused]] float pairReach[kNeeLights];
#pragma unroll
            for (int k = 0; k < kNeeLights; ++k) {
                need[k] = false;
                cosL[k] = 0;
                distance2[k] = 0;
                pairW[k] = v3(0, 0, 0);
                pairReach[k] = 0;
                const int li = l0 + k;
                if (li >= numLights) continue;
                vec3 lo = v3(0, 0, 0), w_i = v3(0, 0, 0);
                float distance = 0;
                if (lit) {
                    vec3 lightPoint;
                    if (li < L.numPointLights) {
                        lightPoint = xyz(loadRow16(sc + L.offPointLight + 2 * li));
                    } else {
                        const float4 light = sc[L.offAreaLight + 2 * (li - L.numPointLights)];
                        const float u1 = ptrng::uniform(ray.rng);
                        const float u2 = ptrng::uniform(ray.rng);
                        const float u3 = ptrng::uniform(ray.rng);
                        const float inverseTotal = ptm::rcp(u1 + u2 + u3);
                        const float weight0 = u1 * inverseTotal, weight1 = u2 * inverseTotal, weight2 = u3 * inverseTotal;
                        const int tri = (ptrng::uniform(ray.rng) > .5f) ? (int)asU(light.w) : (int)asU(sc[L.offAreaLight + 2 * (li - L.numPointLights) + 1].x);
                        const vec3 a = xyz(loadRow16(td + L.offTri + 3 * tri));
                        const vec3 b = xyz(loadRow16(td + L.offTriVert + 2 * tri));
                        const vec3 c = xyz(loadRow16(td + L.offTriVert + 2 * tri + 1));
                        lightPoint = (a * weight0 + b * weight1) + c * weight2;
                    }
                    const vec3 offset = lightPoint - point;
                    distance2[k] = dot(offset, offset);
                    distance = ptm::sqrt(distance2[k]);
                    w_i = offset / distance;
                    cosL[k] = ptm::max(0.0f, dot(normal, w_i));
                    const bool zeroTerm = L.neeSkipSafe && (distance2[k] > 0.0f) && (distance2[k] < ptm::inf()) &&
                                          (cosL[k] == 0.0f || mat[0].w == 0.0f);
                    need[k] = !zeroTerm;
                    lo = point + (ptm::kRayBump * normal);
                    distance -= 2 * ptm::kRayBump;
                }
                if constexpr (kPairs) {
                    pairW[k] = w_i;
                    pairReach[k] = distance;
                    continue;
                }
                const unsigned long long m = __ballot(need[k]);
                if (need[k]) {
                    const uint32_t slot = queued + __popcll(m & ((1ull << lane) - 1ull));
                    wq[0 * kQueueCap + slot] = lo.x;
                    wq[1 * kQueueCap + slot] = lo.y;
                    wq[2 * kQueueCap + slot] = lo.z;
                    wq[3 * kQueueCap + slot] = w_i.x;
                    wq[4 * kQueueCap + slot] = w_i.y;
                    wq[5 * kQueueCap + slot] = w_i.z;
                    wq[6 * kQueueCap + slot] = distance;
                    wqOwner[slot] = lane | ((uint32_t)k << 8);
                    wqAnswer[k * 64 + lane] = 0;
                }
                queued += (uint32_t)__popcll(m);
            }
            PTSS_DIAG_PAIRS(need[0], need[1], lit);
            waveLdsFence();
            PTSS_DIAG_QUEUE(queued);
            if constexpr (kPairs) {
                constexpr int kPairCap = 64;
                const bool needAny = need[0] || need[1];
                const unsigned long long m = __ballot(needAny);
                const uint32_t pairs = (uint32_t)__popcll(m);
                uint32_t* pairOwner = reinterpret_cast<uint32_t*>(wq + 11 * kPairCap);
                if (needAny) {
                    const uint32_t slot = __popcll(m & ((1ull << lane) - 1ull));
                    const vec3 lo = point + (ptm::kRayBump * normal);
                    wq[0 * kPairCap + slot] = lo.x;
                    wq[1 * kPairCap + slot] = lo.y;
                    wq[2 * kPairCap + slot] = lo.z;
                    wq[3 * kPairCap + slot] = pairW[0].x;
                    wq[4 * kPairCap + slot] = pairW[0].y;
                    wq[5 * kPairCap + slot] = pairW[0].z;
                    wq[6 * kPairCap + slot] = pairReach[0];
                    wq[7 * kPairCap + slot] = pairW[1].x;
                    wq[8 * kPairCap + slot] = pairW[1].y;
                    wq[9 * kPairCap + slot] = pairW[1].z;
                    wq[10 * kPairCap + slot] = pairReach[1];
                    pairOwner[slot] = lane | ((need[0] ? 1u : 0u) << 8) | ((need[1] ? 1u : 0u) << 9);
                    wqAnswer[0 * 64 + lane] = 0;
                    wqAnswer[1 * 64 + lane] = 0;
                }
                waveLdsFence();
                for (uint32_t e0 = 0; e0 < pairs;) {
                    const uint32_t rem = pairs - e0;
                    const uint32_t units = (rem + 7u) >> 3;
                    const int chunkLog = (units >= 7u) ? 6 : (units >= 4u ? 5 : (units >= 2u ? 4 : 3));
                    const int shift = 6 - chunkLog;
                    const uint32_t mine = lane >> shift;
                    const uint32_t sub = lane & ((1u << shift) - 1u);
                    const bool have = mine < rem;
                    const uint32_t es = have ? e0 + mine : 0u;
                    const vec3 lo = v3(wq[0 * kPairCap + es], wq[1 * kPairCap + es], wq[2 * kPairCap + es]);
                    const vec3 wA = v3(wq[3 * kPairCap + es], wq[4 * kPairCap + es], wq[5 * kPairCap + es]);
                    const float dA = wq[6 * kPairCap + es];
                    const vec3 wB = v3(wq[7 * kPairCap + es], wq[8 * kPairCap + es], wq[9 * kPairCap + es]);
                    const float dB = wq[10 * kPairCap + es];
                    const uint32_t ow = pairOwner[es];
                    const bool liveA = have && ((ow >> 8) & 1u) != 0u, liveB = have && ((ow >> 9) & 1u) != 0u;
                    bool occA, occB;
                    if (shift == 0) pairAnyHit<kBounded, false>(sc, L, lo, wA, dA, liveA, wB, dB, liveB, 0, 0, occA, occB);
                    else pairAnyHit<kBounded, true>(sc, L, lo, wA, dA, liveA, wB, dB, liveB, shift, (int)sub, occA, occB);
                    const unsigned long long verdictsA = __ballot(occA), verdictsB = __ballot(occB);
                    const unsigned long long group = ((1ull << (1u << shift)) - 1ull) << (mine << shift);
                    if (have && sub == 0u) {
                        if ((verdictsA & group) != 0ull) wqAnswer[0 * 64 + (ow & 63u)] = 1;
                        if ((verdictsB & group) != 0ull) wqAnswer[1 * 64 + (ow & 63u)] = 1;
                    }
                    e0 += 1u << chunkLog;
                }
            } else {
            for (uint32_t e0 = 0; e0 < queued;) {
                const uint32_t rem = queued - e0;
                const uint32_t units = (rem + 7u) >> 3;
                const int chunkLog = (units >= 7u || kAccel || kMesh) ? 6 : (units >= 4u ? 5 : (units >= 2u ? 4 : 3));
                const int shift = 6 - chunkLog;
                const uint32_t mine = lane >> shift;
                const uint32_t sub = lane & ((1u << shift) - 1u);
                const bool have = mine < rem;
                const uint32_t es = have ? e0 + mine : 0u;
                const vec3 lo = v3(wq[0 * kQueueCap + es], wq[1 * kQueueCap + es], wq[2 * kQueueCap + es]);
                const vec3 wi = v3(wq[3 * kQueueCap + es], wq[4 * kQueueCap + es], wq[5 * kQueueCap + es]);
                const float reach = wq[6 * kQueueCap + es];
                bool occ;
                if (kAccel && (e0 != 0u || queued <= 64u)) {
                    occ = anySpheresHybrid(sc, L, wq + e0, wq + (e0 == 0u ? 64 : 0), lo, wi, reach, have);
                    occ = occ || anyTriangles(sc, L, lo, wi, reach, have && !occ);
                } else {
                    occ = (shift == 0) ? anyHit<kAccel, kBounded, kMesh>(sc, L, lo, wi, reach, have, sceneBlob)
                                       : anyHitSplit<kBounded>(sc, L, lo, wi, reach, have, shift, (int)sub);
                }
                const unsigned long long verdicts = __ballot(occ);
                const unsigned long long group = ((1ull << (1u << shift)) - 1ull) << (mine << shift);
                if (have && sub == 0u && (verdicts & group) != 0ull) {
                    const uint32_t ow = wqOwner[es];
                    wqAnswer[(ow >> 8) * 64 + (ow & 63u)] = 1;
                }
                e0 += 1u << chunkLog;
            }
            }
            waveLdsFence();
#pragma unroll
            for (int k = 0; k < kNeeLights; ++k) {
                const int li = l0 + k;
                if (li >= numLights) continue;
                if (need[k] && wqAnswer[k * 64 + lane] == 0) {
                    const vec3 power = (li < L.numPointLights) ? xyz(loadRow16(sc + L.offPointLight + 2 * li + 1))
                                                               : xyz(loadRow16(sc + L.offAreaLight + 2 * (li - L.numPointLights)));
                    addLambertTerm(radiance, cosL[k], power, distance2[k], mat[0]);
                }
            }
            waveLdsFence();
        }

        bool alive = false;
        if constexpr (!kFirst) {
            if (valid) loadRayRadiance<kCoherentIo>(tileBlock(in, base), threadIdx.x, ray);
        }
        if (valid) {
            if (hit) {
                vec3 directRadiance = v3(0, 0, 0) + xyz(mat[3]);
                if (lit) directRadiance = directRadiance + radiance;
                vec3 indirectRadiance = v3(1, 1, 1);
                if (!kLast && !(PTSS_ABLATE & 4)) indirectRadiance = scatter(mat, ray, point, normal, cosI);
                if (inside) {
                    const float4 ab = mat[2];
                    ray.T = ray.T * v3(ptm::exp(-h.distance * ab.x), ptm::exp(-h.distance * ab.y),
                                       ptm::exp(-h.distance * ab.z));
                }
                ray.L0 = ray.L0 + ray.T * directRadiance;
                ray.T = ray.T * indirectRadiance;
            } else {
                const vec3 dc = v3(fb.defaultColor[0], fb.defaultColor[1], fb.defaultColor[2]);
                ray.L0 = ray.L0 + dc * ray.T;
                ray.active = false;
            }
            alive = ray.active && !kLast;
        }

        uint32_t slot = 0;
        if constexpr (!kLast) {
            const unsigned long long live = __ballot(alive);
            if (live) {
                const int leader = __ffsll((long long)live) - 1;
                uint32_t base0 = 0;
                if ((int)lane == leader)
                    base0 = atomicAdd(&fb.counts[countIndex(bounce + 1, (int)shard)], (uint32_t)__popcll(live));
                slot = base0;
                if (valid && !alive && !(PTSS_ABLATE & 8)) finishPath(fb, ray, quantT);
                slot = __shfl(slot, leader) + __popcll(live & ((1ull << lane) - 1ull));
                if (alive) storeRay<kCoherentIo>(out, slot, ray);
            } else if (valid && !(PTSS_ABLATE & 8)) {
                finishPath(fb, ray, quantT);
            }
        } else {
            if (valid && !(PTSS_ABLATE & 8)) finishPath(fb, ray, quantT);
        }
    }
}

template <bool kLast, bool kSceneInLds, bool kFirst, bool kAccel, bool kBounded, bool kPairsWanted, bool kMesh>
__device__ __forceinline__ void bounceBody(const FrameBuffers& fb, const float4* __restrict__ sceneBlob, const SceneLayout& L, int bounce,
                                           const TileMap& tile, const EyeParams& eye) {
    extern __shared__ __attribute__((aligned(256))) float4 lds[];
    constexpr bool kPairs = kPairsWanted && !kAccel;
    const uint32_t shard = blockIdx.x % kShards;
    const uint32_t n = fb.counts[countIndex(bounce, (int)shard)];
    if constexpr (kFirst) {
        if (fb.frameRays <= fb.minLive) return;
    } else {
        if (n == 0) return;
        if (n <= fb.minLive) {
            uint32_t own = 0;
            for (int s = 0; s < kShards; ++s) own += fb.counts[countIndex(bounce, s)];
            if (own <= fb.minLive && frameLiveCount(fb, bounce, own, fb.peerTarget) <= fb.minLive) return;
        }
    }

    const uint32_t lane = __lane_id();
    const uint32_t wave = threadIdx.x >> 6;
    float4* work = lds + (kSceneInLds ? L.ldsVec4 : 0);
    float* wq = reinterpret_cast<float*>(work + kBlockScratchVec4) + wave * kWaveLdsWords;
    uint32_t* wqOwner = reinterpret_cast<uint32_t*>(wq + 7 * kQueueCap);
    unsigned char* wqAnswer = reinterpret_cast<unsigned char*>(wqOwner + kQueueCap);

    const float4* sc;
    if constexpr (kSceneInLds) {
        for (int k = threadIdx.x; k < L.ldsVec4; k += kBlock) lds[k] = sceneBlob[k];
        __syncthreads();
        sc = lds;
    } else {
        sc = sceneBlob;
    }
    const float* quantT = reinterpret_cast<const float*>(sc + L.offQuant);

    const size_t regionWords = (size_t)fb.regionCap * kRayPlanes;
    const float* __restrict__ in = fb.pool[bounce & 1] + shard * regionWords;
    float* __restrict__ out = fb.pool[(bounce + 1) & 1] + shard * regionWords;
    const int numLights = L.numPointLights + L.numAreaLights;
    const TileEnv env{sc, sceneBlob, quantT, in, out, wq, wqOwner, wqAnswer, shard, lane, n, numLights, bounce};

    const uint32_t roundsOfShard = (fb.firstTiles + kShards - 1 - shard) / kShards;
    const uint32_t span = kFirst ? ((roundsOfShard + fb.laneCount - 1 - fb.laneIndex) / fb.laneCount) * kBlock : n;
    for (uint32_t base = (blockIdx.x / kShards) * kBlock; base < span; base += (gridDim.x / kShards) * kBlock) {
        bounceTile<kLast, kFirst, kAccel, kBounded, kPairs, false, kMesh>(fb, L, tile, eye, env, base);
    }
}

template <bool kLast, bool kSceneInLds, bool kFirst, bool kAccel, bool kBounded, bool kPairs, bool kMesh>
__global__ __launch_bounds__(kBlock, (kAccel || kMesh) ? 4 : (kFirst ? PTSS_MINWAVES_FIRST : (kBounded ? PTSS_MINWAVES_BOUNDED : PTSS_MINWAVES))) void bounceKernel(
    FrameBuffers fb, const float4* __restrict__ sceneBlob, SceneLayout L, int bounce, TileMap tile, EyeParams eye) {
    bounceBody<kLast, kSceneInLds, kFirst, kAccel, kBounded, kPairs, kMesh>(fb, sceneBlob, L, bounce, tile, eye);
    if (fb.numPeers != 0) {
        __syncthreads();
        if (threadIdx.x == 0)
            __hip_atomic_fetch_add(fb.myDone + countIndex(bounce, (int)(blockIdx.x % kShards)), 1u, __ATOMIC_RELAXED, __HIP_MEMORY_SCOPE_AGENT);
    }
}

constexpr int kDoneWord = 1;
static_assert((kShards & (kShards - 1)) == 0 && kShards <= 64, "frameKernel's guard needs a power-of-two shard count of at most 64");

__device__ __forceinline__ bool waitForCount(const uint32_t* word, uint32_t target) {
    unsigned long long since = 0ull;
    while (__hip_atomic_load(word, __ATOMIC_RELAXED, __HIP_MEMORY_SCOPE_AGENT) < target) {
        __builtin_amdgcn_s_sleep(8);
        if (peerWaitExpired(since)) return false;
    }
    return true;
}

template <bool kAccel, bool kBounded, bool kPairsWanted>
__global__ __launch_bounds__(kBlock, kAccel ? 4 : (kBounded ? PTSS_MINWAVES_BOUNDED : PTSS_MINWAVES)) void frameKernel(
    FrameBuffers fb, const float4* __restrict__ sceneBlob, SceneLayout L, int numBounces, TileMap tile, EyeParams eye) {
    extern __shared__ __attribute__((aligned(256))) float4 lds[];
    constexpr bool kPairs = kPairsWanted && !kAccel;
    if (fb.frameRays <= fb.minLive) return;
    const uint32_t shard = blockIdx.x % kShards, myTile = blockIdx.x / kShards;
    const uint32_t rounds = (fb.firstTiles + kShards - 1 - shard) / kShards;
    if (myTile >= rounds) return;

    const uint32_t lane = __lane_id();
    const uint32_t wave = threadIdx.x >> 6;
    float4* work = lds + L.ldsVec4;
    uint32_t* bcast = reinterpret_cast<uint32_t*>(work);
    float* wq = reinterpret_cast<float*>(work + kBlockScratchVec4) + wave * kWaveLdsWords;
    uint32_t* wqOwner = reinterpret_cast<uint32_t*>(wq + 7 * kQueueCap);
    unsigned char* wqAnswer = reinterpret_cast<unsigned char*>(wqOwner + kQueueCap);
    for (int k = threadIdx.x; k < L.ldsVec4; k += kBlock) lds[k] = sceneBlob[k];
    __syncthreads();
    const size_t regionWords = (size_t)fb.regionCap * kRayPlanes;
    TileEnv env{lds, sceneBlob, reinterpret_cast<const float*>(lds + L.offQuant), nullptr, nullptr, wq, wqOwner, wqAnswer, shard, lane, 0u,
                L.numPointLights + L.numAreaLights, 0};
    uint32_t tilesNow = rounds, raysNow = 0;
    int verified = 0;
    for (int b = 0; b < numBounces; ++b) {
        const bool last = b == numBounces - 1;
        env.bounce = b;
        env.n = raysNow;
        env.in = fb.pool[b & 1] + shard * regionWords;
        env.out = fb.pool[(b + 1) & 1] + shard * regionWords;
        const uint32_t base = myTile * kBlock;
        if (b == 0) {
            if (last) bounceTile<true, true, kAccel, kBounded, kPairs, true>(fb, L, tile, eye, env, base);
            else bounceTile<false, true, kAccel, kBounded, kPairs, true>(fb, L, tile, eye, env, base);
        } else if (last) {
            bounceTile<true, false, kAccel, kBounded, kPairs, true>(fb, L, tile, eye, env, base);
        } else {
            bounceTile<false, false, kAccel, kBounded, kPairs, true>(fb, L, tile, eye, env, base);
        }
        if (last) break;
        asm volatile("s_waitcnt vmcnt(0)" ::: "memory");
        __syncthreads();
        if (threadIdx.x == 0) {
            __hip_atomic_fetch_add(fb.counts + countIndex(b, (int)shard) + kDoneWord, 1u, __ATOMIC_RELAXED, __HIP_MEMORY_SCOPE_AGENT);
            const uint32_t* done = fb.counts + countIndex(b, (int)shard) + kDoneWord;
            uint32_t next = ~0u;
// ... 504 lines not shown
```

### cuda-path-tracer-ss_amd/host/host_capi.cpp

```cpp
#include "ptss_host.h"

#include <cstdio>
#include <cstring>
#include <new>
#include <vector>

#include "HostOps.h"
#include "Scene.h"
#include "ptdenoise.h"
#include "ptreproject.h"
#include "ptmotion.h"
#include "ptspecular.h"
#include "ptquant.h"
#include "ptmesh.h"
#include "ptpack.h"
#include "pttri.h"
#include "xorwow.h"

struct ptss_scene {
    Scene scene;
};

namespace {
using namespace ptv;
template <int kC1, int kC2>
void triangleForm(const float* t, const float* o3, const float* d3, float limit, bool primary, float* out) {
    const vec3 v0 = v3(t[0], t[1], t[2]), e1 = v3(t[3], t[4], t[5]), e2 = v3(t[6], t[7], t[8]);
    const vec3 o = v3(o3[0], o3[1], o3[2]), d = v3(d3[0], d3[1], d3[2]);
    pttri::Head h;
    if (primary) {
        const vec3 s = o - v0, r = cross(s, e1);
        h = pttri::head<kC1, kC2, true>(v0, e1, e2, s, r, dot(e2, r), o, d);
    } else {
        h = pttri::head<kC1, kC2, false>(v0, e1, e2, v3(0, 0, 0), v3(0, 0, 0), 0.0f, o, d);
    }
    float b0 = 0, b1 = 0, b2 = 0;
    const bool pass = pttri::passesHead(h, limit);
    if (pass) pttri::weights<kC1, kC2>(h, d, b0, b1, b2);
    out[0] = (pass && pttri::passesWeights(b0, b1, b2)) ? 1.0f : 0.0f;
    out[1] = h.dist;
    out[2] = b0;
    out[3] = b1;
    out[4] = b2;
    out[5] = h.det;
}
}

extern "C" {

int ptss_scene_create(const char* preset, ptss_scene** out) {
    if (!preset || !out) return PTSS_HOST_EINVAL;
    ptss_scene* s = new (std::nothrow) ptss_scene();
    if (!s) return PTSS_HOST_EINVAL;
    if (!s->scene.buildPreset(preset)) {
        delete s;
        return PTSS_HOST_EINVAL;
    }
    *out = s;
    return PTSS_HOST_OK;
}

void ptss_scene_destroy(ptss_scene* s) { delete s; }

int ptss_scene_describe(const ptss_scene* s, ptss_scene_desc* out) {
    if (!s || !out) return PTSS_HOST_EINVAL;
    *out = s->scene.desc();
    return PTSS_HOST_OK;
}

int ptss_scene_add_obj(ptss_scene* s, const char* path, const float* m, int materialIdx, size_t* added) {
    if (!s || !path || materialIdx < 0 || (size_t)materialIdx >= s->scene.materialsVec.size()) return PTSS_HOST_EINVAL;
    mat4 t = mat4::identity();
    if (m)
        for (int r = 0; r < 4; ++r)
            for (int c = 0; c < 4; ++c) t.c[c][r] = m[4 * r + c];
    const long n = s->scene.addObjModel(path, t, materialIdx);
    if (n < 0) return n == -2 ? PTSS_HOST_EIO : PTSS_HOST_EINVAL;
    if (added) *added = (size_t)n;
    return PTSS_HOST_OK;
}

int ptss_camera_default(ptss_camera* out) {
    if (!out) return PTSS_HOST_EINVAL;
    *out = Camera();
    return PTSS_HOST_OK;
}

int ptss_camera_ray(const ptss_camera* cam, int width, int height, int x, int y, float jx, float jy, ptss_ray_query* out) {
    if (!cam || !out || width <= 0 || height <= 0) return PTSS_HOST_EINVAL;
    *out = cameraRay(*cam, width, height, x, y, jx, jy);
    return PTSS_HOST_OK;
}

int ptss_camera_move(ptss_camera* cam, unsigned char key, int* moved) {
    if (!cam) return PTSS_HOST_EINVAL;
    Camera c;
    static_cast<ptss_camera&>(c) = *cam;
    const bool m = moveCamera(c, key);
    *cam = c;
    if (moved) *moved = m ? 1 : 0;
    return PTSS_HOST_OK;
}

int ptss_write_tga(const char* filename, const ptss_uchar4* rgba, int width, int height) {
    if (!filename || !rgba || width <= 0 || height <= 0) return PTSS_HOST_EINVAL;
    return writeTga(filename, rgba, width, height) ? PTSS_HOST_OK : PTSS_HOST_EIO;
}

int ptss_tile_rows(int height, int band_rows, int rank, int world, int* rows, int cap) {
    if (height < 0 || band_rows <= 0 || world <= 0 || rank < 0 || rank >= world) return PTSS_HOST_EINVAL;
    int n = 0;
    for (int y = 0; y < height; ++y) {
        if ((y / band_rows) % world != rank) continue;
        if (rows && n < cap) rows[n] = y;
        ++n;
    }
    return n;
}

int ptss_probe_math(int op, const float* x, const float* y, float* out, size_t n) {
    if (!x || !out) return PTSS_HOST_EINVAL;
    for (size_t i = 0; i < n; ++i) {
        float s, c;
        switch (op) {
            case 0: ptm::sincos(x[i], s, c); out[i] = s; break;
            case 1: ptm::sincos(x[i], s, c); out[i] = c; break;
            case 2: out[i] = ptm::tan(x[i]); break;
            case 3: out[i] = ptm::atan(x[i]); break;
            case 4: out[i] = ptm::log(x[i]); break;
            case 5: out[i] = ptm::exp(x[i]); break;
            case 6: if (!y) return PTSS_HOST_EINVAL; out[i] = ptm::pow(x[i], y[i]); break;
            case 7: out[i] = ptm::sqrt(x[i]); break;
            default: return PTSS_HOST_EINVAL;
        }
    }
    return PTSS_HOST_OK;
}

int ptss_probe_triangle_forms(const float* tri9, const float* o3, const float* d3, const float* limit, int primary, size_t n, int* cls,
                              float* general6, float* classed6) {
    if (!tri9 || !o3 || !d3 || !limit || !cls || !general6 || !classed6) return PTSS_HOST_EINVAL;
    for (size_t i = 0; i < n; ++i) {
        const float* t = tri9 + 9 * i;
        const int c = pttri::triangleClass(v3(t[3], t[4], t[5]), v3(t[6], t[7], t[8]));
        cls[i] = c;
        triangleForm<0, 0>(t, o3 + 3 * i, d3 + 3 * i, limit[i], primary != 0, general6 + 6 * i);
        float* out = classed6 + 6 * i;
        switch (c) {
#define PTSS_TRI_CASE(c1, c2) \
    case (c1) * 4 + (c2): triangleForm<c1, c2>(t, o3 + 3 * i, d3 + 3 * i, limit[i], primary != 0, out); break;
            PTSS_TRI_CASE(0, 1) PTSS_TRI_CASE(0, 2) PTSS_TRI_CASE(0, 3)
            PTSS_TRI_CASE(1, 0) PTSS_TRI_CASE(1, 2) PTSS_TRI_CASE(1, 3)
            PTSS_TRI_CASE(2, 0) PTSS_TRI_CASE(2, 1) PTSS_TRI_CASE(2, 3)
            PTSS_TRI_CASE(3, 0) PTSS_TRI_CASE(3, 1) PTSS_TRI_CASE(3, 2)
#undef PTSS_TRI_CASE
            default: triangleForm<0, 0>(t, o3 + 3 * i, d3 + 3 * i, limit[i], primary != 0, out); break;
        }
    }
    return PTSS_HOST_OK;
}

int ptss_probe_quantize(const float* x, unsigned int* out, size_t n) {
    if (!x || !out) return PTSS_HOST_EINVAL;
    for (size_t i = 0; i < n; ++i) out[i] = ptq::quantize_literal(x[i]);
    return PTSS_HOST_OK;
}

int ptss_probe_quant_table(float* out257) {
    if (!out257) return PTSS_HOST_EINVAL;
    float T[ptq::kTableFloats];
    if (!ptq::build_thresholds(T)) return PTSS_HOST_EINVAL;
    for (int k = 0; k <= 256; ++k) out257[k] = T[k];
    return PTSS_HOST_OK;
}

static const uint32_t* jumpTable() {
    static std::vector<uint32_t> table;
    if (table.empty()) {
        table.resize(ptrng::kJumpTableWords);
        ptrng::build_subsequence_table(table.data());
    }
    return table.data();
}

int ptss_probe_mesh_bound(const float* tri9, size_t ntri, const float* o3, const float* d3, size_t n, float margin, int* out, float* bound12) {
    if (!tri9 || ntri == 0 || ntri > (1u << 20) || (n && (!o3 || !d3 || !out))) return PTSS_HOST_EINVAL;
    float b[12];
    ptmesh::buildBound(tri9, (int)ntri, b);
    if (bound12)
        for (int k = 0; k < 12; ++k) bound12[k] = b[k];
    for (size_t i = 0; i < n; ++i) {
        const vec3 o = v3(o3[3 * i], o3[3 * i + 1], o3[3 * i + 2]), d = v3(d3[3 * i], d3[3 * i + 1], d3[3 * i + 2]);
        out[i] = ptmesh::mayTouch(v3(b[0], b[1], b[2]), b[3], v3(b[4], b[5], b[6]), b[7], b[8], b[9], b[10], b[11], o, d, margin) ? 1 : 0;
    }
    return PTSS_HOST_OK;
}

int ptss_probe_mesh_refit(const float* tri9, size_t ntri, float* bounds12) {
    if (!tri9 || !bounds12 || ntri == 0 || ntri > (1u << 20)) return PTSS_HOST_EINVAL;
    const size_t leaves = (ntri + 15) / 16, groups = (leaves + 15) / 16;
    for (size_t k = 0; k < leaves; ++k)
        ptmesh::refitBound(tri9 + 9 * 16 * k, (int)(ntri - 16 * k < 16 ? ntri - 16 * k : 16), 16, bounds12 + 12 * k);
    for (size_t g = 0; g < groups; ++g)
        ptmesh::refitBound(tri9 + 9 * 256 * g, (int)(ntri - 256 * g < 256 ? ntri - 256 * g : 256), ptmesh::kRefitSlots, bounds12 + 12 * (leaves + g));
    return PTSS_HOST_OK;
}

int ptss_probe_mesh_touch(const float* b, const float* o3, const float* d3, size_t n, float margin, int* out) {
    if (!b || (n && (!o3 || !d3 || !out))) return PTSS_HOST_EINVAL;
    for (size_t i = 0; i < n; ++i) {
        const vec3 o = v3(o3[3 * i], o3[3 * i + 1], o3[3 * i + 2]), d = v3(d3[3 * i], d3[3 * i + 1], d3[3 * i + 2]);
        out[i] = ptmesh::mayTouch(v3(b[0], b[1], b[2]), b[3], v3(b[4], b[5], b[6]), b[7], b[8], b[9], b[10], b[11], o, d, margin) ? 1 : 0;
    }
    return PTSS_HOST_OK;
}

int ptss_probe_pack_scene(const ptss_scene_desc* scene, int everySphereLoop, int image, int* numImages, int* inLds, void* layout,
                          size_t layoutBytes, float* blob, size_t blobCapacity, size_t* blobWords) {
    if (!scene || ptpack::validateScene(*scene) || (everySphereLoop != 0 && everySphereLoop != 1)) return PTSS_HOST_EINVAL;
    const int n = ptpack::planImages(*scene, everySphereLoop != 0).numImages;
    if (numImages) *numImages = n;
    if (image < 0 || image >= n || (layout && layoutBytes != sizeof(ptss::SceneLayout))) return PTSS_HOST_EINVAL;
    if (!layout && !blob && !inLds && !blobWords) return PTSS_HOST_OK;
    std::vector<ptpack::PackedImage> images;
    try {
        images = ptpack::packImages(*scene, everySphereLoop != 0);
    } catch (const std::bad_alloc&) {
        return PTSS_HOST_EINVAL;
    }
    const ptpack::PackedImage& im = images[(size_t)image];
    const size_t words = im.blob.size() * 4;
    if (inLds) *inLds = im.inLds ? 1 : 0;
    if (layout) std::memcpy(layout, &im.layout, sizeof(im.layout));
    if (blobWords) *blobWords = words;
    if (blob) {
        if (blobCapacity < words) return PTSS_HOST_EINVAL;
        std::memcpy(blob, im.blob.data(), words * sizeof(float));
    }
    return PTSS_HOST_OK;
}

static int denoiseColours(std::vector<vec3> (&plane)[2], const ptss_pixel_feature* features, int width, int height, const ptss_denoise_params* params,
                          unsigned char* out_rgba, float* out_float) {
    const size_t n = (size_t)width * (size_t)height;
    auto featureAt = [&](int q) { return ptdn::Feature{features[q].normal, features[q].depth, features[q].materialIdx}; };
    auto depthAt = [&](int q) { return features[q].depth; };
    int cur = 0;
    for (int i = 0; i < params->levels; ++i) {
        const ptdn::Level lv = ptdn::levelOf(*params, i);
        const std::vector<vec3>& src = plane[cur];
        std::vector<vec3>& dst = plane[1 - cur];
        dst.resize(n);
        auto colourAt = [&](int q) { return src[(size_t)q]; };
        for (int y = 0; y < height; ++y)
            for (int x = 0; x < width; ++x) dst[(size_t)y * width + x] = ptdn::filterPixel(x, y, width, height, lv, colourAt, featureAt, depthAt);
        cur = 1 - cur;
    }
    for (size_t p = 0; p < n; ++p) {
        const vec3 v = plane[cur][p];
        if (out_float) { out_float[3 * p] = v.x; out_float[3 * p + 1] = v.y; out_float[3 * p + 2] = v.z; }
        if (out_rgba) { out_rgba[4 * p] = ptdn::toByte(v.x); out_rgba[4 * p + 1] = ptdn::toByte(v.y); out_rgba[4 * p + 2] = ptdn::toByte(v.z); out_rgba[4 * p + 3] = 255; }
    }
    return PTSS_HOST_OK;
}

static bool denoiseArgumentsOk(const void* input, const ptss_pixel_feature* features, int width, int height, const ptss_denoise_params* params) {
    if (!input || !features || !params || width <= 0 || height <= 0) return false;
    if (params->structSize != (unsigned int)sizeof(ptss_denoise_params) || params->levels < 0 || params->levels > PTSS_DENOISE_MAX_LEVELS)
        return false;
    return params->sigmaColor > 0.0f && params->sigmaNormal > 0.0f && params->sigmaDepth >= 0.0f;
// ... 144 lines not shown
```

### cuda-path-tracer-ss_amd/ptss.py

```python
import ctypes as C
import os

import numpy as np

from ptss_types import (KERNEL_BITS, SCENE_LAYOUT_FIELDS, SCENE_LAYOUT_MESH_FIELDS, AreaLight, Camera, DenoiseParams, HistoryEntry, Material, PixelFeature,
                        PixelMotion, PointLight, RayHit, RayQuery, ReprojectParams, SceneDesc, Sphere, Triangle, UChar4, Vec3, struct_to_dict)

_HERE = os.path.dirname(os.path.abspath(__file__))
LIBDIR = os.path.join(_HERE, "lib")
HOST_LIB = os.path.join(LIBDIR, "libptss_host.so")
DEVICE_LIB = os.path.join(LIBDIR, os.environ.get("PTSS_LIBNAME", "libptss.so"))

_u32p = C.POINTER(C.c_uint32)
_f32p = C.POINTER(C.c_float)


class PtssError(RuntimeError):
    pass


class RenderConfig(C.Structure):
    _fields_ = [("structSize", C.c_uint), ("width", C.c_int), ("height", C.c_int), ("seed", C.c_ulonglong), ("maxIterations", C.c_uint),
                ("device", C.c_int), ("tileRank", C.c_int), ("tileWorld", C.c_int), ("bandRows", C.c_int),
                ("syncEachFrame", C.c_int), ("floatAccumulator", C.c_int), ("timeKernels", C.c_int),
                ("samplesPerPass", C.c_int), ("everySphereLoop", C.c_int), ("frameLanes", C.c_int),
                ("lanesFreeRun", C.c_int), ("oneLaunchFrames", C.c_int)]


KERNEL_VARIANTS = ("accel", "bounded+pairs", "bounded", "plain")


def _bounce(variant, j):
    return ("bounce", variant, bool(j & 4), bool(j & 2), bool(j & 1))


_KERNEL_NAMES = {
    "BOUNCE": lambda j: _bounce(KERNEL_VARIANTS[j // 8], j % 8),
    "FRAME": lambda j: ("frame", KERNEL_VARIANTS[j]),
    "BOUNCE_MESH": lambda j: _bounce("mesh", j),
    "QUERY": lambda j: ("query", "any" if j & 2 else "closest", bool(j & 1)),
    "FEATURES": lambda j: ("features", bool(j)),
    "DENOISE": lambda j: ("denoise",),
    "UPDATE": lambda j: ("update",),
    "REFIT": lambda j: ("refit",),
    "REPROJECT": lambda j: ("reproject",),
    "FEATURES_MOTION": lambda j: ("features_motion", bool(j)),
    "REPROJECT_MOTION": lambda j: ("reproject_motion",),
}
KERNEL_OF_BIT = {base + j: _KERNEL_NAMES[rng](j) for rng, (base, width) in KERNEL_BITS.items() for j in range(width)}


def _kernels_of(*ranges):
    return {KERNEL_OF_BIT[KERNEL_BITS[r][0] + j] for r in ranges for j in range(KERNEL_BITS[r][1])}


def decode_launched_kernels(mask):
    return {name for bit, name in KERNEL_OF_BIT.items() if mask >> bit & 1}


def all_kernels():
    return _kernels_of("BOUNCE", "FRAME")


def mesh_kernels():
    return _kernels_of("BOUNCE_MESH")


def query_kernels():
    return _kernels_of("QUERY")


def feature_kernels():
    return _kernels_of("FEATURES")


def reproject_kernels():
    return _kernels_of("REPROJECT")


def motion_kernels():
    return _kernels_of("FEATURES_MOTION", "REPROJECT_MOTION")


_host = None
_dev = None
_hip = None


def _hip_lib():
    global _hip
    if _hip is None:
        device_lib()
        L = C.CDLL("libamdhip64.so.7", mode=C.RTLD_GLOBAL)
        L.hipMalloc.argtypes = [C.POINTER(C.c_void_p), C.c_size_t]
        L.hipFree.argtypes = [C.c_void_p]
        L.hipMemcpy.argtypes = [C.c_void_p, C.c_void_p, C.c_size_t, C.c_int]
        L.hipSetDevice.argtypes = [C.c_int]
        L.hipDeviceSynchronize.argtypes = []
        _hip = L
    return _hip


def _hip_check(rc, what):
    if rc != 0:
        raise PtssError(f"{what} failed (hipError {rc})")


def host_lib():
    global _host
    if _host is None:
        if not os.path.exists(HOST_LIB):
            raise PtssError(f"{HOST_LIB} missing: run `python __graft_entry__.py build` first")
        L = C.CDLL(HOST_LIB)
        L.ptss_scene_create.argtypes = [C.c_char_p, C.POINTER(C.c_void_p)]
        L.ptss_scene_destroy.argtypes = [C.c_void_p]
        L.ptss_scene_destroy.restype = None
        L.ptss_scene_describe.argtypes = [C.c_void_p, C.POINTER(SceneDesc)]
        L.ptss_camera_default.argtypes = [C.POINTER(Camera)]
        L.ptss_camera_move.argtypes = [C.POINTER(Camera), C.c_ubyte, C.POINTER(C.c_int)]
        L.ptss_write_tga.argtypes = [C.c_char_p, C.c_void_p, C.c_int, C.c_int]
        L.ptss_tile_rows.argtypes = [C.c_int, C.c_int, C.c_int, C.c_int, C.POINTER(C.c_int), C.c_int]
        L.ptss_probe_math.argtypes = [C.c_int, _f32p, _f32p, _f32p, C.c_size_t]
        L.ptss_probe_quantize.argtypes = [_f32p, C.POINTER(C.c_uint), C.c_size_t]
        L.ptss_probe_triangle_forms.argtypes = [_f32p, _f32p, _f32p, _f32p, C.c_int, C.c_size_t, C.POINTER(C.c_int), _f32p, _f32p]
        L.ptss_probe_quant_table.argtypes = [_f32p]
        L.ptss_probe_rng_init.argtypes = [C.c_ulonglong, C.c_uint, _u32p]
        L.ptss_scene_add_obj.argtypes = [C.c_void_p, C.c_char_p, _f32p, C.c_int, C.POINTER(C.c_size_t)]
        L.ptss_probe_mesh_bound.argtypes = [_f32p, C.c_size_t, _f32p, _f32p, C.c_size_t, C.c_float, C.POINTER(C.c_int), _f32p]
        L.ptss_probe_rng_draw.argtypes = [_u32p, _u32p, _f32p, C.c_size_t]
        L.ptss_probe_rng_jump_table.argtypes = [_u32p, C.c_size_t]
        L.ptss_camera_ray.argtypes = [C.POINTER(Camera), C.c_int, C.c_int, C.c_int, C.c_int, C.c_float, C.c_float, C.POINTER(RayQuery)]
        L.ptss_probe_mesh_refit.argtypes = [_f32p, C.c_size_t, _f32p]
        L.ptss_probe_mesh_touch.argtypes = [_f32p, _f32p, _f32p, C.c_size_t, C.c_float, C.POINTER(C.c_int)]
        L.ptss_probe_pack_scene.argtypes = [C.POINTER(SceneDesc), C.c_int, C.c_int, C.POINTER(C.c_int), C.POINTER(C.c_int), C.c_void_p,
                                            C.c_size_t, _f32p, C.c_size_t, C.POINTER(C.c_size_t)]
        L.ptss_probe_denoise.argtypes = [_u32p, C.c_float, C.c_void_p, C.c_int, C.c_int, C.POINTER(DenoiseParams), C.c_void_p, _f32p]
        L.ptss_probe_denoise_history.argtypes = [C.c_void_p, C.c_void_p, C.c_int, C.c_int, C.POINTER(DenoiseParams), C.c_void_p, _f32p]
        L.ptss_probe_reproject.argtypes = [_u32p, C.c_float, C.c_int, C.POINTER(Camera), C.POINTER(Camera), C.c_int, C.c_int, C.c_void_p,
                                           C.c_void_p, C.c_void_p, C.POINTER(ReprojectParams), C.c_void_p]
        L.ptss_probe_reproject_motion.argtypes = [_u32p, C.c_float, C.c_int, C.POINTER(Camera), C.POINTER(Camera), C.c_int, C.c_int, C.c_void_p,
                                                  C.c_void_p, C.c_void_p, C.c_void_p, C.POINTER(ReprojectParams), C.c_void_p]
        L.ptss_probe_motion.argtypes = [C.c_void_p, C.c_void_p, C.c_size_t, C.c_void_p, C.c_size_t, C.c_size_t, C.c_size_t, C.c_void_p]
        L.ptss_probe_specular_step.argtypes = [C.c_void_p, C.c_void_p, C.c_size_t, C.c_void_p, C.c_size_t, C.c_void_p, C.POINTER(C.c_int)]
        L.ptss_probe_specular_class.argtypes = [C.c_void_p]
        _host = L
    return _host


def _torch_first():
    import sys
    torch = sys.modules.get("torch")
    if torch is None:
        return
    try:
        if torch.cuda.is_available() and not torch.cuda.is_initialized():
            torch.cuda.init()
    except Exception as e:
        raise PtssError("torch is imported but torch.cuda could not be initialised before libptss.so's HIP runtime "
                        f"(INTEGRATION.md §5, two HIP runtimes in one process): {e}")


def device_lib():
    global _dev
    _torch_first()
    if _dev is None:
        if not os.path.exists(DEVICE_LIB):
            raise PtssError(f"{DEVICE_LIB} missing: the HIP extension was not built (no CPU fallback exists)")
        L = C.CDLL(DEVICE_LIB)
        vp = C.c_void_p
        L.ptss_default_config.argtypes = [C.POINTER(RenderConfig)]
        L.ptss_create.argtypes = [C.POINTER(SceneDesc), C.POINTER(RenderConfig), C.POINTER(vp)]
        L.ptss_destroy.argtypes = [vp]
        L.ptss_generate_frame.argtypes = [vp, vp, C.c_int]
        L.ptss_set_camera.argtypes = [vp, C.POINTER(Camera)]
        L.ptss_get_camera.argtypes = [vp, C.POINTER(Camera)]
        L.ptss_request_reset.argtypes = [vp]
        L.ptss_set_mode.argtypes = [vp, C.c_int]
        L.ptss_set_max_iterations.argtypes = [vp, C.c_uint]
        L.ptss_set_stream.argtypes = [vp, vp]
        L.ptss_bind_accumulator.argtypes = [vp, vp]
        L.ptss_accumulator_devptr.argtypes = [vp, C.POINTER(vp)]
        L.ptss_float_accumulator_devptr.argtypes = [vp, C.POINTER(vp)]
        L.ptss_alloc_pixels.argtypes = [vp, C.POINTER(vp)]
        L.ptss_free_pixels.argtypes = [vp, vp]
        L.ptss_local_pixels.argtypes = [vp, C.POINTER(C.c_size_t)]
        L.ptss_local_rows.argtypes = [vp, C.POINTER(C.c_int), C.c_int, C.POINTER(C.c_int)]
        L.ptss_read_accumulator.argtypes = [vp, _u32p, C.c_size_t]
        L.ptss_read_float_accumulator.argtypes = [vp, _f32p, C.c_size_t]
        L.ptss_read_pixels.argtypes = [vp, vp, vp, C.c_size_t]
        L.ptss_read_rng_state.argtypes = [vp, C.c_size_t, _u32p]
        L.ptss_read_rng_state_lane.argtypes = [vp, C.c_size_t, C.c_uint, _u32p]
        L.ptss_synchronize.argtypes = [vp]
        L.ptss_last_pass_ms.argtypes = [vp, _f32p]
        L.ptss_samples_since_reset.argtypes = [vp, C.POINTER(C.c_int)]
        L.ptss_live_counts.argtypes = [vp, _u32p, C.c_int, C.POINTER(C.c_int)]
        L.ptss_total_ray_bounces.argtypes = [vp, C.POINTER(C.c_ulonglong)]
        L.ptss_frame_lanes.argtypes = [vp, C.POINTER(C.c_int)]
        L.ptss_one_launch_frames.argtypes = [vp, C.POINTER(C.c_int)]
        L.ptss_guard_timeouts.argtypes = [vp, C.POINTER(C.c_uint)]
        L.ptss_bounce_kernel_time.argtypes = [vp, C.POINTER(C.c_double), C.POINTER(C.c_ulonglong)]
        L.ptss_launched_kernels.argtypes = [vp, C.POINTER(C.c_ulonglong)]
        L.ptss_debug_counters.argtypes = [vp, C.POINTER(C.c_ulonglong)]
        L.ptss_triangle_leaves.argtypes = [vp, C.POINTER(C.c_int)]
        L.ptss_intersect.argtypes = [vp, vp, vp, C.c_size_t, vp]
        L.ptss_occluded.argtypes = [vp, vp, vp, C.c_size_t, vp]
        L.ptss_render_features.argtypes = [vp, vp, vp]
        L.ptss_default_denoise_params.argtypes = [C.POINTER(DenoiseParams)]
        L.ptss_denoise.argtypes = [vp, vp, C.POINTER(DenoiseParams), vp, vp]
        L.ptss_read_denoise_plane.argtypes = [vp, _f32p, C.c_size_t, C.POINTER(C.c_int)]
        L.ptss_default_reproject_params.argtypes = [C.POINTER(ReprojectParams)]
        L.ptss_reproject.argtypes = [vp, vp, C.POINTER(Camera), vp, vp, C.POINTER(ReprojectParams), vp, vp]
        L.ptss_denoise_history.argtypes = [vp, vp, vp, C.POINTER(DenoiseParams), vp, vp]
        L.ptss_render_features_motion.argtypes = [vp, vp, C.c_size_t, C.c_size_t, vp, vp, vp]
        L.ptss_reproject_motion.argtypes = [vp, vp, vp, C.POINTER(Camera), vp, vp, C.POINTER(ReprojectParams), vp, vp]
        L.ptss_render_features_specular.argtypes = [vp, C.c_int, vp, vp, vp]
        L.ptss_specular_feature_launches.argtypes = [vp, C.POINTER(C.c_ulonglong)]
        L.ptss_set_scene.argtypes = [vp, C.POINTER(SceneDesc)]
        L.ptss_update_triangles.argtypes = [vp, vp, C.c_size_t, C.c_size_t, vp]
        L.ptss_update_rejected.argtypes = [vp, C.POINTER(C.c_ulonglong)]
        L.ptss_reseed.argtypes = [vp, C.c_ulonglong]
        L.ptss_read_triangle_bounds.argtypes = [vp, _f32p, C.c_size_t]
        L.ptss_read_triangle_positions.argtypes = [vp, C.POINTER(C.c_int), C.c_size_t]
        L.ptss_error_string.argtypes = [C.c_int]
        L.ptss_error_string.restype = C.c_char_p
        L.ptss_last_error_detail.restype = C.c_char_p
        _dev = L
    return _dev


def _check(rc):
    if rc != 0:
        L = device_lib()
        raise PtssError(f"ptss error {rc} ({L.ptss_error_string(rc).decode()}): {L.ptss_last_error_detail().decode()}")


class Scene:

    def __init__(self, preset="default"):
        self._h = C.c_void_p()
        rc = host_lib().ptss_scene_create(preset.encode(), C.byref(self._h))
        if rc != 0:
            raise PtssError(f"unknown scene preset {preset!r}")
        self.preset = preset
        self.desc = SceneDesc()
        host_lib().ptss_scene_describe(self._h, C.byref(self.desc))
        self.desc._owner = self

    def add_obj(self, path, transform=None, material=0):
        m = None
        if transform is not None:
            t = np.ascontiguousarray(np.asarray(transform, dtype=np.float32).reshape(4, 4))
            m = t.ctypes.data_as(_f32p)
        added = C.c_size_t()
        rc = host_lib().ptss_scene_add_obj(self._h, os.fsencode(path), m, int(material), C.byref(added))
        if rc != 0:
            raise PtssError(f"add_obj({path!r}) failed: {'cannot read the file' if rc == -2 else 'malformed OBJ or bad argument'} ({rc})")
        owner = self
        self.desc = SceneDesc()
        host_lib().ptss_scene_describe(self._h, C.byref(self.desc))
        self.desc._owner = owner
        return added.value

    def __del__(self):
        if getattr(self, "_h", None) and self._h.value and host_lib is not None:
            host_lib().ptss_scene_destroy(self._h)
            self._h = C.c_void_p()

    def _arr(self, ptr, n):
        return [ptr[i] for i in range(n)]

    @property
    def spheres(self):
        return self._arr(self.desc.spheres, self.desc.numSpheres)

    @property
    def triangles(self):
        return self._arr(self.desc.triangles, self.desc.numTriangles)

    @property
    def materials(self):
        return self._arr(self.desc.materials, self.desc.numMaterials)

    @property
    def area_lights(self):
        return self._arr(self.desc.areaLights, self.desc.numAreaLights)

    @property
    def point_lights(self):
        return self._arr(self.desc.pointLights, self.desc.numPointLights)

    def table(self):
        return {
            "spheres": [struct_to_dict(s) for s in self.spheres],
            "triangles": [struct_to_dict(s) for s in self.triangles],
            "materials": [struct_to_dict(s) for s in self.materials],
            "pointLights": [struct_to_dict(s) for s in self.point_lights],
            "areaLights": [struct_to_dict(s) for s in self.area_lights],
        }


def probe_mesh_bound(tris, origins, directions, margin=1.0):
    t = np.ascontiguousarray(np.asarray(tris, dtype=np.float32).reshape(-1, 9))
    o = np.ascontiguousarray(np.asarray(origins, dtype=np.float32).reshape(-1, 3))
    d = np.ascontiguousarray(np.asarray(directions, dtype=np.float32).reshape(-1, 3))
    out = np.zeros(len(o), dtype=np.int32)
    bound = np.zeros(12, dtype=np.float32)
    rc = host_lib().ptss_probe_mesh_bound(t.ctypes.data_as(_f32p), len(t), o.ctypes.data_as(_f32p), d.ctypes.data_as(_f32p), len(o),
                                          float(margin), out.ctypes.data_as(C.POINTER(C.c_int)), bound.ctypes.data_as(_f32p))
    if rc != 0:
        raise PtssError(f"ptss_probe_mesh_bound: {rc}")
    return out, bound


def probe_mesh_refit(tris):
    t = np.ascontiguousarray(np.asarray(tris, dtype=np.float32).reshape(-1, 9))
    leaves = (len(t) + 15) // 16
    out = np.zeros((leaves + (leaves + 15) // 16, 12), dtype=np.float32)
    rc = host_lib().ptss_probe_mesh_refit(t.ctypes.data_as(_f32p), len(t), out.ctypes.data_as(_f32p))
    if rc != 0:
        raise PtssError(f"ptss_probe_mesh_refit: {rc}")
    return out


def probe_mesh_touch(bound, origins, directions, margin=1.0):
    b = np.ascontiguousarray(np.asarray(bound, dtype=np.float32).reshape(12))
    o = np.ascontiguousarray(np.asarray(origins, dtype=np.float32).reshape(-1, 3))
    d = np.ascontiguousarray(np.asarray(directions, dtype=np.float32).reshape(-1, 3))
    out = np.zeros(len(o), dtype=np.int32)
    rc = host_lib().ptss_probe_mesh_touch(b.ctypes.data_as(_f32p), o.ctypes.data_as(_f32p), d.ctypes.data_as(_f32p), len(o), float(margin),
                                          out.ctypes.data_as(C.POINTER(C.c_int)))
    if rc != 0:
        raise PtssError(f"ptss_probe_mesh_touch: {rc}")
    return out


def probe_pack_scene_images(scene, every_sphere_loop=False):
    n = C.c_int()
    rc = host_lib().ptss_probe_pack_scene(C.byref(scene.desc), 1 if every_sphere_loop else 0, 0, C.byref(n), None, None, 0, None, 0, None)
    if rc != 0:
        raise PtssError(f"ptss_probe_pack_scene: {rc}")
    return n.value


def probe_pack_scene(scene, every_sphere_loop=False, image=0):
    every = 1 if every_sphere_loop else 0
    raw = np.zeros(len(SCENE_LAYOUT_FIELDS), dtype=np.int32)
    in_lds, words = C.c_int(), C.c_size_t()
    blob = np.empty(1 << 16, dtype=np.float32)
    for _ in range(2):
        rc = host_lib().ptss_probe_pack_scene(C.byref(scene.desc), every, int(image), None, C.byref(in_lds), raw.ctypes.data_as(C.c_void_p),
                                              raw.nbytes, blob.ctypes.data_as(_f32p), blob.size, C.byref(words))
        if rc == 0 or words.value <= blob.size:
            break
        blob = np.empty(words.value, dtype=np.float32)
# ... 238 lines not shown
        cfg.device = device
        cfg.tileRank, cfg.tileWorld, cfg.bandRows = tile_rank, tile_world, band_rows
        cfg.syncEachFrame = 1 if sync_each_frame else 0
        cfg.floatAccumulator = 1 if float_accumulator else 0
        cfg.timeKernels = 1 if time_kernels else 0
        cfg.samplesPerPass = samples_per_pass
        cfg.everySphereLoop = 1 if every_sphere_loop else 0
        cfg.frameLanes = frame_lanes
        cfg.lanesFreeRun = 1 if lanes_free_run else 0
        cfg.oneLaunchFrames = one_launch_frames
        self.cfg = cfg
        self._scene = scene
        self._ctx = C.c_void_p()
        _check(L.ptss_create(C.byref(scene.desc), C.byref(cfg), C.byref(self._ctx)))
        n = C.c_size_t()
        _check(L.ptss_local_pixels(self._ctx, C.byref(n)))
        self.local_pixels = n.value
        self.width, self.height = width, height
        self.local_rows = self.local_pixels // width
        self._own_pixels = None
        self._buffers = {}
        self._have_features = False
        self.ticks = 1

    def close(self):
        if self._ctx:
            L = device_lib()
            if self._own_pixels:
                L.ptss_free_pixels(self._ctx, self._own_pixels)
                self._own_pixels = None
            for p in self._buffers.values():
                _hip_lib().hipFree(p)
            self._buffers = {}
            L.ptss_destroy(self._ctx)
            self._ctx = C.c_void_p()

    def __del__(self):
        try:
            self.close()
        except Exception:
            pass

    def pixels_devptr(self):
        if self._own_pixels is None:
            p = C.c_void_p()
            _check(device_lib().ptss_alloc_pixels(self._ctx, C.byref(p)))
            self._own_pixels = p
        return self._own_pixels

    def set_stream(self, raw_stream):
        _check(device_lib().ptss_set_stream(self._ctx, C.c_void_p(raw_stream)))

    def bind_accumulator(self, devptr):
        _check(device_lib().ptss_bind_accumulator(self._ctx, C.c_void_p(devptr)))

    def rows(self):
        cnt = C.c_int()
        rows = (C.c_int * max(self.local_rows, 1))()
        _check(device_lib().ptss_local_rows(self._ctx, rows, self.local_rows, C.byref(cnt)))
        return np.array(rows[:cnt.value], dtype=np.int64)

    def generate_frame(self, dev_pixels=None, ticks=None):
        if ticks is None:
            ticks = self.ticks
            self.ticks += 1
        if dev_pixels is None:
            dev_pixels = self.pixels_devptr()
        elif isinstance(dev_pixels, int):
            dev_pixels = C.c_void_p(dev_pixels)
        _check(device_lib().ptss_generate_frame(self._ctx, dev_pixels, ticks))

    def set_camera(self, cam):
        _check(device_lib().ptss_set_camera(self._ctx, C.byref(cam)))
        self._have_features = False

    def get_camera(self):
        cam = Camera()
        _check(device_lib().ptss_get_camera(self._ctx, C.byref(cam)))
        return cam

    def request_reset(self):
        _check(device_lib().ptss_request_reset(self._ctx))

    def set_mode(self, use_path_tracer):
        _check(device_lib().ptss_set_mode(self._ctx, 1 if use_path_tracer else 0))

    def set_max_iterations(self, n):
        _check(device_lib().ptss_set_max_iterations(self._ctx, n))

    def synchronize(self):
        _check(device_lib().ptss_synchronize(self._ctx))

    def accumulator(self):
        out = np.empty((self.local_pixels, 3), dtype=np.uint32)
        _check(device_lib().ptss_read_accumulator(self._ctx, out.ctypes.data_as(_u32p), out.size))
        return out

    def float_accumulator(self):
        out = np.empty((self.local_pixels, 3), dtype=np.float32)
        _check(device_lib().ptss_read_float_accumulator(self._ctx, out.ctypes.data_as(_f32p), out.size))
        return out

    def pixels(self, dev_pixels=None):
        if dev_pixels is None:
            dev_pixels = self.pixels_devptr()
        elif isinstance(dev_pixels, int):
            dev_pixels = C.c_void_p(dev_pixels)
        out = np.empty((self.local_pixels, 4), dtype=np.uint8)
        _check(device_lib().ptss_read_pixels(self._ctx, dev_pixels, out.ctypes.data_as(C.c_void_p), self.local_pixels))
        return out

    def rng_state(self, local_pixel, lane=0):
        out = np.empty(6, dtype=np.uint32)
        _check(device_lib().ptss_read_rng_state_lane(self._ctx, local_pixel, lane, out.ctypes.data_as(_u32p)))
        return out

    def last_pass_ms(self):
        v = C.c_float()
        _check(device_lib().ptss_last_pass_ms(self._ctx, C.byref(v)))
        return v.value

    def live_counts(self):
        out = (C.c_uint32 * 65)()
        n = C.c_int()
        _check(device_lib().ptss_live_counts(self._ctx, out, 65, C.byref(n)))
        return np.array(out[:n.value], dtype=np.uint32)

    def total_ray_bounces(self):
        v = C.c_ulonglong()
        _check(device_lib().ptss_total_ray_bounces(self._ctx, C.byref(v)))
        return v.value

    @property
    def one_launch_frames(self):
        v = C.c_int()
        _check(device_lib().ptss_one_launch_frames(self._ctx, C.byref(v)))
        return bool(v.value)

    @property
    def frame_lanes(self):
        v = C.c_int()
        _check(device_lib().ptss_frame_lanes(self._ctx, C.byref(v)))
        return v.value

    def guard_timeouts(self):
        v = C.c_uint()
        _check(device_lib().ptss_guard_timeouts(self._ctx, C.byref(v)))
        return v.value

    def launched_kernels(self):
        v = C.c_ulonglong()
        _check(device_lib().ptss_launched_kernels(self._ctx, C.byref(v)))
        return decode_launched_kernels(v.value)

    def set_scene(self, scene):
        _check(device_lib().ptss_set_scene(self._ctx, C.byref(scene.desc)))
        self._scene = scene
        self._have_features = False

    def update_triangles(self, triangles, first=0, stream=None):
        L = device_lib()
        if type(triangles).__module__.split(".")[0] == "torch":
            import sys
            torch = sys.modules["torch"]
            if triangles.dtype != torch.float32 or not triangles.is_contiguous() or not triangles.is_cuda or triangles.numel() % 19:
                raise ValueError("triangles: a contiguous float32 device tensor of n x 19 words")
            if stream is None:
                stream = torch.cuda.current_stream(triangles.device).cuda_stream
            _check(L.ptss_update_triangles(self._ctx, C.c_void_p(triangles.data_ptr()), first, triangles.numel() // 19, C.c_void_p(stream)))
        else:
            a = np.ascontiguousarray(triangles, dtype=TRIANGLE_DTYPE).reshape(-1)
            d = self._device_buffer_at_least("triangles_upload", a.nbytes) if len(a) else None
            if len(a):
                _hip_check(_hip_lib().hipMemcpy(d, a.ctypes.data, a.nbytes, 1), "hipMemcpy")
            _check(L.ptss_update_triangles(self._ctx, d, first, len(a), C.c_void_p(stream) if stream else None))
            if len(a):
                if stream:
                    _hip_check(_hip_lib().hipDeviceSynchronize(), "hipDeviceSynchronize")
                self.synchronize()
        self._have_features = False

    def reseed(self, seed):
        _check(device_lib().ptss_reseed(self._ctx, seed))

    def update_rejected(self):
        v = C.c_ulonglong()
        _check(device_lib().ptss_update_rejected(self._ctx, C.byref(v)))
        return v.value

    def triangle_bounds(self):
        leaves = self.triangle_leaves()
        out = np.empty((leaves + (leaves + 15) // 16, 12), dtype=np.float32)
        _check(device_lib().ptss_read_triangle_bounds(self._ctx, out.ctypes.data_as(_f32p), out.size))
        return out

    def triangle_positions(self, count):
        out = np.empty(count, dtype=np.int32)
        _check(device_lib().ptss_read_triangle_positions(self._ctx, out.ctypes.data_as(C.POINTER(C.c_int)), out.size))
        return out

    def intersect(self, rays):
        return self._query(rays, any_hit=False)

    def occluded(self, rays):
        return self._query(rays, any_hit=True)

    def _query(self, rays, any_hit):
        L = device_lib()
        fn = L.ptss_occluded if any_hit else L.ptss_intersect
        if type(rays).__module__.split(".")[0] == "torch":
            import sys
            torch = sys.modules["torch"]
            if rays.dtype != torch.float32 or rays.dim() != 2 or rays.shape[1] != 8 or not rays.is_contiguous() or not rays.is_cuda:
                raise ValueError("rays: a contiguous (N, 8) float32 device tensor")
            n = rays.shape[0]
            out = (torch.empty(n, dtype=torch.int32, device=rays.device) if any_hit
                   else torch.empty((n, 12), dtype=torch.float32, device=rays.device))
            stream = torch.cuda.current_stream(rays.device).cuda_stream
            _check(fn(self._ctx, C.c_void_p(rays.data_ptr()), C.c_void_p(out.data_ptr()), n, C.c_void_p(stream)))
            return out
        a = np.asarray(rays)
        if a.dtype == RAY_DTYPE:
            a = np.ascontiguousarray(a).view(np.float32).reshape(-1, 8)
        a = np.ascontiguousarray(a, dtype=np.float32)
        if a.ndim != 2 or a.shape[1] != 8:
            raise ValueError("rays: (N, 8) float32 or (N,) RAY_DTYPE")
        n = a.shape[0]
        out = np.empty(n, dtype=np.uint32) if any_hit else np.empty(n, dtype=HIT_DTYPE)
        if n == 0:
            return out
        H = _hip_lib()
        _hip_check(H.hipSetDevice(self.cfg.device), "hipSetDevice")
        d_rays, d_out = C.c_void_p(), C.c_void_p()
        _hip_check(H.hipMalloc(C.byref(d_rays), a.nbytes), "hipMalloc")
        try:
            _hip_check(H.hipMalloc(C.byref(d_out), out.nbytes), "hipMalloc")
            _hip_check(H.hipMemcpy(d_rays, a.ctypes.data, a.nbytes, 1), "hipMemcpy")
            _check(fn(self._ctx, d_rays, d_out, n, None))
            self.synchronize()
            _hip_check(H.hipMemcpy(out.ctypes.data, d_out, out.nbytes, 2), "hipMemcpy")
        finally:
            H.hipFree(d_rays)
            if d_out:
                H.hipFree(d_out)
        return out

    def _device_buffer(self, name, nbytes):
        bufs = self._buffers
        if name not in bufs:
            H = _hip_lib()
            _hip_check(H.hipSetDevice(self.cfg.device), "hipSetDevice")
            p = C.c_void_p()
            _hip_check(H.hipMalloc(C.byref(p), max(nbytes, 16)), "hipMalloc")
            bufs[name] = p
        return bufs[name]

    def _device_buffer_at_least(self, name, nbytes):
        have = getattr(self, "_buffer_bytes", {})
        if name in self._buffers and have.get(name, 0) < nbytes:
            _hip_lib().hipFree(self._buffers.pop(name))
        have[name] = max(have.get(name, 0), nbytes)
        self._buffer_bytes = have
        return self._device_buffer(name, nbytes)

    def features_devptr(self):
        return self._device_buffer("features", self.local_pixels * FEATURE_DTYPE.itemsize)

    def features(self, stream=None):
        d = self.features_devptr()
        _check(device_lib().ptss_render_features(self._ctx, d, C.c_void_p(stream) if stream else None))
        out = np.empty(self.local_pixels, dtype=FEATURE_DTYPE)
        if self.local_pixels:
            if stream:
                _hip_check(_hip_lib().hipDeviceSynchronize(), "hipDeviceSynchronize")
            self.synchronize()
            _hip_check(_hip_lib().hipMemcpy(out.ctypes.data, d, out.nbytes, 2), "hipMemcpy")
        self._have_features = True
        return out

    def motion_devptr(self):
        return self._device_buffer("motion", self.local_pixels * MOTION_DTYPE.itemsize)

    def features_motion(self, prev_triangles=None, first=0, stream=None):
        L = device_lib()
        d_feat, d_mot = self.features_devptr(), self.motion_devptr()
        if type(prev_triangles).__module__.split(".")[0] == "torch":
            import sys
            torch = sys.modules["torch"]
            t = prev_triangles
            if t.dtype != torch.float32 or not t.is_contiguous() or not t.is_cuda or t.numel() % 19:
                raise ValueError("prev_triangles: a contiguous float32 device tensor of n x 19 words")
            if stream is None:
                stream = torch.cuda.current_stream(t.device).cuda_stream
            d_prev, count = C.c_void_p(t.data_ptr()) if t.numel() else None, t.numel() // 19
        elif prev_triangles is None:
            d_prev, count = None, 0
        else:
            a = np.ascontiguousarray(prev_triangles, dtype=TRIANGLE_DTYPE).reshape(-1)
            d_prev, count = None, len(a)
            if count:
                d_prev = self._device_buffer_at_least("prev_triangles_upload", a.nbytes)
                _hip_check(_hip_lib().hipMemcpy(d_prev, a.ctypes.data, a.nbytes, 1), "hipMemcpy")
        _check(L.ptss_render_features_motion(self._ctx, d_prev, first, count, d_feat, d_mot, C.c_void_p(stream) if stream else None))
        feat = np.empty(self.local_pixels, dtype=FEATURE_DTYPE)
        mot = np.empty(self.local_pixels, dtype=MOTION_DTYPE)
        if self.local_pixels:
# ... 147 lines not shown
```

### include/ptss.h

```cpp
#ifndef PTSS_H
#define PTSS_H

#include "ptss_types.h"

#ifdef __cplusplus
extern "C" {
#endif

#define PTSS_OK 0
#define PTSS_EINVAL (-1)
#define PTSS_EHIP (-2)
#define PTSS_ENODEVICE (-3)
#define PTSS_ENOMEM (-4)
#define PTSS_ERANGE (-5)
#define PTSS_ETIMEOUT (-6)
#define PTSS_VERSION 300

typedef struct ptss_context ptss_context;

typedef struct ptss_render_config {
    unsigned int structSize;
    int width, height;
    unsigned long long seed;
    unsigned int maxIterations;
    int device;
    int tileRank, tileWorld, bandRows;
    int syncEachFrame;
    int floatAccumulator;
    int timeKernels;
    int samplesPerPass;
    int everySphereLoop;
    int frameLanes;
    int lanesFreeRun;
    int oneLaunchFrames;
} ptss_render_config;

int ptss_default_config(ptss_render_config* cfg);

int ptss_create(const ptss_scene_desc* scene, const ptss_render_config* cfg, ptss_context** out);

int ptss_destroy(ptss_context* ctx);

int ptss_generate_frame(ptss_context* ctx, ptss_uchar4* dev_pixels, int ticks);

int ptss_set_camera(ptss_context* ctx, const ptss_camera* camera);
int ptss_get_camera(const ptss_context* ctx, ptss_camera* out);
int ptss_request_reset(ptss_context* ctx);
int ptss_set_mode(ptss_context* ctx, int usePathTracer);
int ptss_set_max_iterations(ptss_context* ctx, unsigned int maxIterations);

int ptss_set_stream(ptss_context* ctx, void* hipStream);
int ptss_bind_accumulator(ptss_context* ctx, uint32_t* dev_uint3);
int ptss_accumulator_devptr(ptss_context* ctx, uint32_t** out);
int ptss_float_accumulator_devptr(ptss_context* ctx, float** out);
int ptss_alloc_pixels(ptss_context* ctx, ptss_uchar4** out_dev);
int ptss_free_pixels(ptss_context* ctx, ptss_uchar4* dev);
int ptss_local_pixels(const ptss_context* ctx, size_t* out);
int ptss_local_rows(const ptss_context* ctx, int* rows, int cap, int* count);

int ptss_read_accumulator(ptss_context* ctx, uint32_t* host_uint3, size_t count);
int ptss_read_float_accumulator(ptss_context* ctx, float* host_float3, size_t count);
int ptss_read_pixels(ptss_context* ctx, const ptss_uchar4* dev_pixels, ptss_uchar4* host, size_t count);
int ptss_read_rng_state(ptss_context* ctx, size_t local_pixel, uint32_t* out6);
int ptss_read_rng_state_lane(ptss_context* ctx, size_t local_pixel, unsigned int lane, uint32_t* out6);
int ptss_synchronize(ptss_context* ctx);

int ptss_last_pass_ms(ptss_context* ctx, float* out_ms);
int ptss_samples_since_reset(const ptss_context* ctx, int* out);
int ptss_live_counts(ptss_context* ctx, uint32_t* out, int cap, int* n);
int ptss_total_ray_bounces(ptss_context* ctx, unsigned long long* out);
int ptss_bounce_kernel_time(ptss_context* ctx, double* total_ms, unsigned long long* launches);

int ptss_one_launch_frames(const ptss_context* ctx, int* out);
int ptss_frame_lanes(const ptss_context* ctx, int* out);
int ptss_guard_timeouts(ptss_context* ctx, unsigned int* out);

int ptss_launched_kernels(const ptss_context* ctx, unsigned long long* out);

int ptss_intersect(ptss_context* ctx, const ptss_ray_query* dev_rays, ptss_ray_hit* dev_hits, size_t n, void* hipStream);
int ptss_occluded(ptss_context* ctx, const ptss_ray_query* dev_rays, uint32_t* dev_occluded, size_t n, void* hipStream);

int ptss_render_features(ptss_context* ctx, ptss_pixel_feature* dev_features, void* hipStream);

int ptss_render_features_motion(ptss_context* ctx, const ptss_triangle* dev_triangles_prev, size_t first, size_t count,
                                ptss_pixel_feature* dev_features, ptss_pixel_motion* dev_motion, void* hipStream);

int ptss_render_features_specular(ptss_context* ctx, int maxSteps, ptss_pixel_feature* dev_features, uint32_t* dev_steps ,
                                  void* hipStream);
int ptss_specular_feature_launches(const ptss_context* ctx, unsigned long long* out2);

int ptss_default_denoise_params(ptss_denoise_params* p);

int ptss_denoise(ptss_context* ctx, const ptss_pixel_feature* dev_features, const ptss_denoise_params* params, ptss_uchar4* dev_out,
                 void* hipStream);

int ptss_read_denoise_plane(ptss_context* ctx, float* host_float3, size_t count, int* level);

int ptss_default_reproject_params(ptss_reproject_params* p);

int ptss_reproject(ptss_context* ctx, const ptss_pixel_feature* dev_features_now, const ptss_camera* prev_camera,
                   const ptss_pixel_feature* dev_features_prev, const ptss_history_entry* dev_history_prev,
                   const ptss_reproject_params* params, ptss_history_entry* dev_history_out, void* hipStream);

int ptss_reproject_motion(ptss_context* ctx, const ptss_pixel_feature* dev_features_now, const ptss_pixel_motion* dev_motion_now,
                          const ptss_camera* prev_camera, const ptss_pixel_feature* dev_features_prev,
                          const ptss_history_entry* dev_history_prev, const ptss_reproject_params* params,
                          ptss_history_entry* dev_history_out, void* hipStream);

int ptss_denoise_history(ptss_context* ctx, const ptss_history_entry* dev_history, const ptss_pixel_feature* dev_features,
                         const ptss_denoise_params* params, ptss_uchar4* dev_out, void* hipStream);

int ptss_triangle_leaves(const ptss_context* ctx, int* out);

int ptss_set_scene(ptss_context* ctx, const ptss_scene_desc* scene);

int ptss_update_triangles(ptss_context* ctx, const ptss_triangle* dev_triangles, size_t first, size_t count, void* hipStream);
int ptss_update_rejected(ptss_context* ctx, unsigned long long* out);

int ptss_reseed(ptss_context* ctx, unsigned long long seed);

int ptss_read_triangle_bounds(ptss_context* ctx, float* host, size_t count);
int ptss_read_triangle_positions(ptss_context* ctx, int* host, size_t count);

int ptss_debug_counters(ptss_context* ctx, unsigned long long* out8);

const char* ptss_error_string(int code);
const char* ptss_last_error_detail(void);
int ptss_version(void);

#ifdef __cplusplus
}
#endif
#endif
```

### include/ptss_host.h

```cpp
#ifndef PTSS_HOST_H
#define PTSS_HOST_H

#include "ptss_types.h"

#ifdef __cplusplus
extern "C" {
#endif

#define PTSS_HOST_OK 0
#define PTSS_HOST_EINVAL (-1)
#define PTSS_HOST_EIO (-2)

typedef struct ptss_scene ptss_scene;

int ptss_scene_create(const char* preset, ptss_scene** out);
void ptss_scene_destroy(ptss_scene* s);
int ptss_scene_describe(const ptss_scene* s, ptss_scene_desc* out);

int ptss_scene_add_obj(ptss_scene* s, const char* path, const float* mat4x4, int materialIdx, size_t* added);

int ptss_camera_default(ptss_camera* out);
int ptss_camera_move(ptss_camera* cam, unsigned char key, int* moved);
int ptss_camera_ray(const ptss_camera* cam, int width, int height, int x, int y, float jx, float jy, ptss_ray_query* out);

int ptss_write_tga(const char* filename, const ptss_uchar4* rgba, int width, int height);

int ptss_tile_rows(int height, int band_rows, int rank, int world, int* rows, int cap);

int ptss_probe_math(int op, const float* x, const float* y, float* out, size_t n);
int ptss_probe_quantize(const float* x, unsigned int* out, size_t n);
int ptss_probe_quant_table(float* out257);
int ptss_probe_triangle_forms(const float* tri9, const float* o3, const float* d3, const float* limit, int primary, size_t n, int* cls,
                              float* general6, float* classed6);
int ptss_probe_mesh_bound(const float* tri9, size_t ntri, const float* o3, const float* d3, size_t n, float margin, int* out, float* bound12);
int ptss_probe_mesh_refit(const float* tri9, size_t ntri, float* bounds12);
int ptss_probe_pack_scene(const ptss_scene_desc* scene, int everySphereLoop, int image, int* numImages, int* inLds, void* layout,
                          size_t layoutBytes, float* blob, size_t blobCapacity, size_t* blobWords);
int ptss_probe_mesh_touch(const float* bound12, const float* o3, const float* d3, size_t n, float margin, int* out);
int ptss_probe_denoise(const uint32_t* accum, float inverseTicks, const ptss_pixel_feature* features, int width, int height,
                       const ptss_denoise_params* params, unsigned char* out_rgba, float* out_float);
int ptss_probe_denoise_history(const ptss_history_entry* history, const ptss_pixel_feature* features, int width, int height,
                               const ptss_denoise_params* params, unsigned char* out_rgba, float* out_float);
int ptss_probe_reproject(const uint32_t* accum, float inverseTicks, int n, const ptss_camera* camera_now, const ptss_camera* camera_prev,
                         int width, int height, const ptss_pixel_feature* features_now, const ptss_pixel_feature* features_prev,
                         const ptss_history_entry* history_prev, const ptss_reproject_params* params, ptss_history_entry* out);
int ptss_probe_reproject_motion(const uint32_t* accum, float inverseTicks, int n, const ptss_camera* camera_now, const ptss_camera* camera_prev,
                                int width, int height, const ptss_pixel_feature* features_now, const ptss_pixel_motion* motion_now,
                                const ptss_pixel_feature* features_prev, const ptss_history_entry* history_prev,
                                const ptss_reproject_params* params, ptss_history_entry* out);
int ptss_probe_motion(const ptss_ray_query* rays, const ptss_ray_hit* hits, size_t n, const ptss_triangle* triangles_prev, size_t first,
                      size_t count, size_t numTriangles, ptss_pixel_motion* out);
int ptss_probe_specular_step(const ptss_ray_query* rays, const ptss_ray_hit* hits, size_t n, const ptss_material* materials, size_t numMaterials,
                             ptss_ray_query* next, int* follows);
int ptss_probe_specular_class(const ptss_material* material);
int ptss_probe_rng_init(unsigned long long seed, unsigned int subsequence, unsigned int* out6);
int ptss_probe_rng_draw(unsigned int* state6, unsigned int* raw, float* uni, size_t n);
int ptss_probe_rng_jump_table(unsigned int* out, size_t words);

#ifdef __cplusplus
}
#endif
#endif
```

Measured before the change: 18550 Mrays/s.

## Skip division and sqrt range fallbacks where scene data proves operands safe

Adds host-computed scene guard flags proving that light powers, refraction indices and Phong exponents lie in ranges where the fast rcp/div sequences are exact, and threads them to the kernel so those sites skip the wave-wide fallback checks. Light sampling now uses a single bit-window test on distance squared before fast sqrt and divide, normalize uses a fused sqrt and reciprocal, and the Lambert sqrt and barycentric rcp drop their guards. The aim is fewer ballots and slow-path branches in shading, at the cost of extra constants and a new flag field. Correctness relies on the range proofs matching IEEE results.

```diff
diff --git a/cuda-path-tracer-ss_amd/build.py b/cuda-path-tracer-ss_amd/build.py
--- a/cuda-path-tracer-ss_amd/build.py
+++ b/cuda-path-tracer-ss_amd/build.py
@@ -76,15 +76,24 @@
     return out
 
 
+def build_guardcheck(force=False):
+    out = os.path.join(LIBDIR, "ptss_guardcheck")
+    src = os.path.join(ROOT, "tests", "csrc", "guards_device.hip")
+    hipcc = shutil.which("hipcc") or "/opt/rocm/bin/hipcc"
+    if force or _newer(out, [src] + _headers()):
+        _run([hipcc] + [f for f in HIP_FLAGS if f != "-fPIC"] + ["-I", INC, "-I", CSRC, src, "-o", out])
+    return out
+
+
 def build_all(force=False):
-    return [build_host(force), build_device(force), build_main(force), build_mathcheck(force)]
+    return [build_host(force), build_device(force), build_main(force), build_mathcheck(force), build_guardcheck(force)]
 
 
 if __name__ == "__main__":
     force = "--force" in sys.argv
     what = [a for a in sys.argv[1:] if not a.startswith("-")]
     table = {"host": build_host, "device": build_device, "main": build_main,
-             "mathcheck": build_mathcheck}
+             "mathcheck": build_mathcheck, "guardcheck": build_guardcheck}
     if not what:
         build_all(force)
     for w in what:
diff --git a/cuda-path-tracer-ss_amd/csrc/ptmath.h b/cuda-path-tracer-ss_amd/csrc/ptmath.h
--- a/cuda-path-tracer-ss_amd/csrc/ptmath.h
+++ b/cuda-path-tracer-ss_amd/csrc/ptmath.h
@@ -73,6 +73,61 @@
 }
 PTM_HD uint32_t f2u(float x) { return __builtin_bit_cast(uint32_t, x); }
 PTM_HD float u2f(uint32_t x) { return __builtin_bit_cast(float, x); }
+
+constexpr float kSqrtLo = 2.5243549e-29f , kSqrtHi = 7.9228163e28f ;
+constexpr float kRcpLo = 2.3509887e-38f , kRcpHi = 8.5070592e37f ;
+constexpr float kDivLo = 8.6736174e-19f , kDivHi = 1.1529215e18f ;
+constexpr float kFourPi = 4 * kPi;
+constexpr float kLightD2Lo = 0x1.45f306p-64f;
+constexpr float kLightD2Hi = 0x1.45f306p+56f;
+constexpr uint32_t kLightD2LoBits = 0x1fa2f983u, kLightD2Span = 0x3c000000u;
+PTM_HD bool in_light_window(float distance2) { return f2u(distance2) - kLightD2LoBits < kLightD2Span; }
+PTM_HD bool every_lane(bool inRange) {
+#if defined(__HIP_DEVICE_COMPILE__)
+    return allLanes(lanes(inRange));
+#else
+    return inRange;
+#endif
+}
+PTM_HD bool every_lane(bool a, bool b) {
+#if defined(__HIP_DEVICE_COMPILE__)
+    return allLanes(lanes(a) & lanes(b));
+#else
+    return a && b;
+#endif
+}
+PTM_HD bool fast_numerator(float a) {
+    const float aa = abs(a);
+    return f2u(a) == 0u || (aa >= kDivLo && aa < kDivHi);
+}
+PTM_HD bool fast_divisor(float b) { return abs(b) >= kDivLo && abs(b) < kDivHi; }
+PTM_HD bool fast_rcp_operand(float x) { return abs(x) >= kRcpLo && abs(x) < kRcpHi; }
+PTM_HD float sqrt_in_range(float x) {
+#if defined(__HIP_DEVICE_COMPILE__)
+    const float y = __builtin_amdgcn_rsqf(x);
+    const float s = x * y;
+    const float h = 0.5f * y;
+    const float r = __builtin_fmaf(-s, s, x);
+    return __builtin_fmaf(r, h, s);
+#else
+    return __builtin_sqrtf(x);
+#endif
+}
+PTM_HD void sqrt_rcp(float x, float& s, float& inv) {
+#if defined(__HIP_DEVICE_COMPILE__)
+    s = sqrt_in_range(x);
+    inv = rcp_in_range(s);
+    const bool lo = x >= kSqrtLo, hi = x < kSqrtHi;
+    if (__builtin_expect(!allLanes(lanes(lo) & lanes(hi)), 0)) {
+        const float si = __builtin_sqrtf(x);
+        s = (lo && hi) ? s : si;
+        inv = (lo && hi) ? inv : 1.0f / si;
+    }
+#else
+    s = __builtin_sqrtf(x);
+    inv = 1.0f / s;
+#endif
+}
 PTM_HD float inf() { return u2f(0x7f800000u); }
 PTM_HD float qnan() { return u2f(0x7fc00000u); }
 
@@ -121,6 +176,25 @@
     qx = ax / b;
     qy = ay / b;
     qz = az / b;
+#endif
+}
+PTM_HD void div3_in_range(float ax, float ay, float az, float b, float& qx, float& qy, float& qz) {
+#if defined(__HIP_DEVICE_COMPILE__)
+    const float r = rcp_core(b);
+    qx = div_core(ax, b, r);
+    qy = div_core(ay, b, r);
+    qz = div_core(az, b, r);
+#else
+    qx = ax / b;
+    qy = ay / b;
+    qz = az / b;
+#endif
+}
+PTM_HD float div_in_range_operands(float a, float b) {
+#if defined(__HIP_DEVICE_COMPILE__)
+    return div_core(a, b, rcp_core(b));
+#else
+    return a / b;
 #endif
 }
 PTM_HD float max(float a, float b) { return (a < b) ? b : a; }
@@ -269,14 +343,18 @@
 PTM_HD vec3 cross(vec3 a, vec3 b) {
     return vec3{ptm::fma(a.y, b.z, -(a.z * b.y)), ptm::fma(a.z, b.x, -(a.x * b.z)), ptm::fma(a.x, b.y, -(a.y * b.x))};
 }
-PTM_HD vec3 normalize(vec3 v) { return v * ptm::rcp(ptm::sqrt(dot(v, v))); }
+PTM_HD vec3 normalize(vec3 v) {
+    float len, inv;
+    ptm::sqrt_rcp(dot(v, v), len, inv);
+    return v * inv;
+}
 PTM_HD float length(vec3 v) { return ptm::sqrt(dot(v, v)); }
 
 PTM_HD quat q4(float w, float x, float y, float z) { return quat{x, y, z, w}; }
 PTM_HD quat normalize(quat q) {
-    float len = ptm::sqrt(ptm::fma(q.w, q.w, ptm::fma(q.z, q.z, ptm::fma(q.y, q.y, q.x * q.x))));
+    float len, inv;
+    ptm::sqrt_rcp(ptm::fma(q.w, q.w, ptm::fma(q.z, q.z, ptm::fma(q.y, q.y, q.x * q.x))), len, inv);
     if (len <= 0.0f) return q4(1, 0, 0, 0);
-    float inv = ptm::rcp(len);
     return q4(q.w * inv, q.x * inv, q.y * inv, q.z * inv);
 }
 PTM_HD vec3 rotate(quat q, vec3 v) {
diff --git a/cuda-path-tracer-ss_amd/csrc/ptpack.h b/cuda-path-tracer-ss_amd/csrc/ptpack.h
--- a/cuda-path-tracer-ss_amd/csrc/ptpack.h
+++ b/cuda-path-tracer-ss_amd/csrc/ptpack.h
@@ -294,6 +294,21 @@
     L.triClassed = (L.triDetBounded && L.sphereBounded && L.numTriangles <= 255) ? 1 : 0;
 }
 
+inline uint32_t sceneGuardFlags(const ptss_scene_desc& s) {
+    uint32_t flags = ptss::kGuardLightPowers | ptss::kGuardRefraction | ptss::kGuardPhongExponent;
+    auto fast3 = [](const ptss_vec3& v) { return ptm::fast_numerator(v.x) && ptm::fast_numerator(v.y) && ptm::fast_numerator(v.z); };
+    for (size_t i = 0; i < s.numPointLights; ++i)
+        if (!fast3(s.pointLights[i].power)) flags &= ~(uint32_t)ptss::kGuardLightPowers;
+    for (size_t i = 0; i < s.numAreaLights; ++i)
+        if (!fast3(s.areaLights[i].power)) flags &= ~(uint32_t)ptss::kGuardLightPowers;
+    for (size_t i = 0; i < s.numMaterials; ++i) {
+        const float n = s.materials[i].indexOfRefraction, e = s.materials[i].specularExponent;
+        if (!ptm::fast_divisor(n)) flags &= ~(uint32_t)ptss::kGuardRefraction;
+        if (!(e == ptm::inf() || ptm::fast_rcp_operand(e + 1))) flags &= ~(uint32_t)ptss::kGuardPhongExponent;
+    }
+    return flags;
+}
+
 inline std::vector<int> orderTriangles(const ptss_scene_desc& s, SceneLayout& L) {
     std::vector<int> triOrder((size_t)L.numTriangles), triCode((size_t)L.numTriangles, 0);
     for (int i = 0; i < L.numTriangles; ++i) {
diff --git a/cuda-path-tracer-ss_amd/csrc/ptscene.h b/cuda-path-tracer-ss_amd/csrc/ptscene.h
--- a/cuda-path-tracer-ss_amd/csrc/ptscene.h
+++ b/cuda-path-tracer-ss_amd/csrc/ptscene.h
@@ -20,6 +20,12 @@
 constexpr int kChunkSpheres = PTSS_CHUNK;
 static_assert((kChunkSpheres & (kChunkSpheres - 1)) == 0, "chunk size must be a power of two");
 constexpr int kWaves = kBlock / 64;
+
+enum GuardFlag : uint32_t {
+    kGuardLightPowers = 1u,
+    kGuardRefraction = 2u,
+    kGuardPhongExponent = 4u,
+};
 
 struct SceneLayout {
     int numSpheres, numTriangles, numMaterials, numPointLights, numAreaLights;
diff --git a/cuda-path-tracer-ss_amd/csrc/ptshade.h b/cuda-path-tracer-ss_amd/csrc/ptshade.h
--- a/cuda-path-tracer-ss_amd/csrc/ptshade.h
+++ b/cuda-path-tracer-ss_amd/csrc/ptshade.h
@@ -6,9 +6,26 @@
 namespace ptss {
 namespace {
 
+__device__ __forceinline__ void lightSample(vec3 offset, float& distance2, float& distance, vec3& w_i) {
+    distance2 = dot(offset, offset);
+    const float least = __builtin_fminf(__builtin_fminf(ptm::abs(offset.x), ptm::abs(offset.y)), ptm::abs(offset.z));
+    PTSS_DIAG_GUARD_LIGHT(offset, distance2, least);
+    if (__builtin_expect(ptm::every_lane(ptm::in_light_window(distance2), least >= ptm::kDivLo), 1)) {
+        distance = ptm::sqrt_in_range(distance2);
+        ptm::div3_in_range(offset.x, offset.y, offset.z, distance, w_i.x, w_i.y, w_i.z);
+    } else {
+        distance = ptm::sqrt(distance2);
+        w_i = offset / distance;
+    }
+}
+
 __device__ __forceinline__ void addLambertTerm(vec3& radiance, float cosI, vec3 power, float distance2,
-                                               float4 diffuse ) {
-    const vec3 L_i = power / (float)(4 * ptm::kPi * distance2);
+                                               float4 diffuse , bool powersProven) {
+    const float divisor = (float)(ptm::kFourPi * distance2);
+    vec3 L_i;
+    PTSS_DIAG_GUARD_POWER(power, divisor);
+    if (powersProven && ptm::every_lane(ptm::in_light_window(distance2))) ptm::div3_in_range(power.x, power.y, power.z, divisor, L_i.x, L_i.y, L_i.z);
+    else L_i = power / divisor;
     radiance.x += cosI * L_i.x * diffuse.x * diffuse.w * ptm::kInvPi;
     radiance.y += cosI * L_i.y * diffuse.y * diffuse.w * ptm::kInvPi;
     radiance.z += cosI * L_i.z * diffuse.z * diffuse.w * ptm::kInvPi;
@@ -21,7 +38,7 @@
 
 enum LobeKind { kLobeNone = 0, kLobeLambert = 1, kLobePhong = 2, kLobeBeckmann = 3 };
 
-__device__ __forceinline__ vec3 scatter(const float4* mat, RayRegs& ray, vec3 point, vec3 normal, float cosI) {
+__device__ __forceinline__ vec3 scatter(const float4* mat, RayRegs& ray, vec3 point, vec3 normal, float cosI, uint32_t guardFlags) {
     const float4 mDiffuse = mat[0];
     const float4 mSpecular = mat[1];
     const float4 mMisc = mat[4];
@@ -63,7 +80,8 @@
         float fresnelReflective = 1.0f;
         PTSS_DIAG_SCATTER(2, readsFresnel);
         if (readsFresnel) {
-            n = ptm::div(n1, n2);
+            PTSS_DIAG_GUARD_DIV(7, n1, n2);
+            n = (guardFlags & kGuardRefraction) ? ptm::div_in_range_operands(n1, n2) : ptm::div(n1, n2);
             sinT2 = n * n * (1.0f - cosI * cosI);
         }
         if (readsFresnel && !(sinT2 > 1.0f)) {
@@ -128,7 +146,8 @@
             ptm::sincos(theta, a, y);
         } else {
             azimuth = u1 * 2 * ptm::kPi;
-            y = (kind == kLobeLambert) ? ptm::sqrt(u2) : ptm::pow(u2, ptm::rcp(mMisc.x + 1));
+            if (kind == kLobeLambert) y = ptm::sqrt_in_range(u2);
+            else y = ptm::pow(u2, (guardFlags & kGuardPhongExponent) ? ptm::rcp_in_range(mMisc.x + 1) : ptm::rcp(mMisc.x + 1));
             a = ptm::sqrt(1 - y * y);
         }
         float sn, cs;
diff --git a/cuda-path-tracer-ss_amd/csrc/ptss_api.hip b/cuda-path-tracer-ss_amd/csrc/ptss_api.hip
--- a/cuda-path-tracer-ss_amd/csrc/ptss_api.hip
+++ b/cuda-path-tracer-ss_amd/csrc/ptss_api.hip
@@ -72,6 +72,7 @@
     ptss::SceneLayout layout{};
     bool inLds = true;
     bool oneLaunch = false;
+    uint32_t guardFlags = 0;
 };
 
 struct ptss_context {
@@ -168,6 +169,7 @@
         SceneImage& im = st.images[i];
         im.layout = packed[(size_t)i].layout;
         im.inLds = packed[(size_t)i].inLds;
+        im.guardFlags = ptpack::sceneGuardFlags(scene);
         const std::vector<ptpack::Row>& blob = packed[(size_t)i].blob;
         hipError_t e = hipMalloc(&im.dBlob, blob.size() * sizeof(float4));
         if (e == hipSuccess) e = hipMemcpy(im.dBlob, blob.data(), blob.size() * sizeof(float4), hipMemcpyHostToDevice);
@@ -288,6 +290,7 @@
     fb.defaultColor[0] = c->defaultColor[0];
     fb.defaultColor[1] = c->defaultColor[1];
     fb.defaultColor[2] = c->defaultColor[2];
+    fb.guardFlags = c->image().guardFlags;
     fb.laneIndex = (uint32_t)laneIdx;
     fb.laneCount = (uint32_t)c->lanes.size();
     fb.frameRays = c->numPixels * c->samples;
@@ -913,6 +916,12 @@
     return PTSS_OK;
 }
 
+int ptss_guard_flags(const ptss_context* c, unsigned int* out) {
+    if (!c || !out) return fail(PTSS_EINVAL, "null argument");
+    *out = c->image().guardFlags;
+    return PTSS_OK;
+}
+
 static int rayQuery(ptss_context* c, bool any, const ptss_ray_query* rays, void* out, size_t n, void* hipStream) {
     if (!c) return fail(PTSS_EINVAL, "ctx is null");
     if (n == 0) return PTSS_OK;
diff --git a/cuda-path-tracer-ss_amd/csrc/ptss_device.h b/cuda-path-tracer-ss_amd/csrc/ptss_device.h
--- a/cuda-path-tracer-ss_amd/csrc/ptss_device.h
+++ b/cuda-path-tracer-ss_amd/csrc/ptss_device.h
@@ -84,6 +84,7 @@
     uint32_t minLive;
     float inverseTicks;
     float defaultColor[3];
+    uint32_t guardFlags;
     uint32_t laneIndex, laneCount;
     uint32_t frameRays;
     uint32_t numPeers;
diff --git a/cuda-path-tracer-ss_amd/csrc/ptss_diag.h b/cuda-path-tracer-ss_amd/csrc/ptss_diag.h
--- a/cuda-path-tracer-ss_amd/csrc/ptss_diag.h
+++ b/cuda-path-tracer-ss_amd/csrc/ptss_diag.h
@@ -97,3 +97,34 @@
 #else
 #define PTSS_DIAG_QUEUE(queued) do {} while (0)
 #endif
+
+#if PTSS_DIAG & 32
+__device__ __forceinline__ void diagGuard(int site, unsigned long long inRange) {
+    const unsigned long long active = __ballot(true);
+    if ((inRange & active) != active && __lane_id() == (unsigned)(__ffsll((long long)active) - 1)) atomicAdd(&g_diag[site], 1ull);
+}
+__device__ __forceinline__ void diagGuardCount(int site) {
+    if (__lane_id() == (unsigned)(__ffsll((long long)__ballot(true)) - 1)) atomicAdd(&g_diag[site], 1ull);
+}
+__device__ __forceinline__ unsigned long long diagDivLanes(float x) { return __ballot(ptm::abs(x) >= ptm::kDivLo && ptm::abs(x) < ptm::kDivHi); }
+#define PTSS_DIAG_GUARD_LIGHT(offset, d2, least)                                                                                   \
+    do {                                                                                                                           \
+        diagGuardCount(0);                                                                                                         \
+        diagGuard(1, __ballot((d2) >= ptm::kSqrtLo && (d2) < ptm::kSqrtHi));                                                       \
+        diagGuard(2, diagDivLanes(__builtin_sqrtf(d2)) & diagDivLanes((offset).x) & diagDivLanes((offset).y) & diagDivLanes((offset).z)); \
+        diagGuard(3, __ballot((d2) >= ptm::kLightD2Lo && (d2) < ptm::kLightD2Hi && (least) >= ptm::kDivLo));                       \
+    } while (0)
+#define PTSS_DIAG_GUARD_POWER(power, divisor)                                                                                      \
+    do {                                                                                                                           \
+        diagGuardCount(4);                                                                                                         \
+        const unsigned long long _den = diagDivLanes(divisor);                                                                     \
+        const unsigned long long _num = diagDivLanes((power).x) & diagDivLanes((power).y) & diagDivLanes((power).z);               \
+        diagGuard(5, _den & _num);                                                                                                 \
+        diagGuard(6, _num | ~_den);                                                                                                \
+    } while (0)
+#define PTSS_DIAG_GUARD_DIV(site, a, b) diagGuard(site, diagDivLanes(a) & diagDivLanes(b))
+#else
+#define PTSS_DIAG_GUARD_LIGHT(offset, d2, least) do {} while (0)
+#define PTSS_DIAG_GUARD_POWER(power, divisor) do {} while (0)
+#define PTSS_DIAG_GUARD_DIV(site, a, b) do {} while (0)
+#endif
diff --git a/cuda-path-tracer-ss_amd/csrc/ptss_kernels.hip b/cuda-path-tracer-ss_amd/csrc/ptss_kernels.hip
--- a/cuda-path-tracer-ss_amd/csrc/ptss_kernels.hip
+++ b/cuda-path-tracer-ss_amd/csrc/ptss_kernels.hip
@@ -209,7 +209,7 @@
                         const float u1 = ptrng::uniform(ray.rng);
                         const float u2 = ptrng::uniform(ray.rng);
                         const float u3 = ptrng::uniform(ray.rng);
-                        const float inverseTotal = ptm::rcp(u1 + u2 + u3);
+                        const float inverseTotal = ptm::rcp_in_range(u1 + u2 + u3);
                         const float weight0 = u1 * inverseTotal, weight1 = u2 * inverseTotal, weight2 = u3 * inverseTotal;
                         const int tri = (ptrng::uniform(ray.rng) > .5f) ? (int)asU(light.w) : (int)asU(sc[L.offAreaLight + 2 * (li - L.numPointLights) + 1].x);
                         const vec3 a = xyz(loadRow16(td + L.offTri + 3 * tri));
@@ -218,9 +218,7 @@
                         lightPoint = (a * weight0 + b * weight1) + c * weight2;
                     }
                     const vec3 offset = lightPoint - point;
-                    distance2[k] = dot(offset, offset);
-                    distance = ptm::sqrt(distance2[k]);
-                    w_i = offset / distance;
+                    lightSample(offset, distance2[k], distance, w_i);
                     cosL[k] = ptm::max(0.0f, dot(normal, w_i));
                     const bool zeroTerm = L.neeSkipSafe && (distance2[k] > 0.0f) && (distance2[k] < ptm::inf()) &&
                                           (cosL[k] == 0.0f || mat[0].w == 0.0f);
@@ -341,7 +339,7 @@
                 if (need[k] && wqAnswer[k * 64 + lane] == 0) {
                     const vec3 power = (li < L.numPointLights) ? xyz(loadRow16(sc + L.offPointLight + 2 * li + 1))
                                                                : xyz(loadRow16(sc + L.offAreaLight + 2 * (li - L.numPointLights)));
-                    addLambertTerm(radiance, cosL[k], power, distance2[k], mat[0]);
+                    addLambertTerm(radiance, cosL[k], power, distance2[k], mat[0], (fb.guardFlags & kGuardLightPowers) != 0u);
                 }
             }
             waveLdsFence();
@@ -356,7 +354,7 @@
                 vec3 directRadiance = v3(0, 0, 0) + xyz(mat[3]);
                 if (lit) directRadiance = directRadiance + radiance;
                 vec3 indirectRadiance = v3(1, 1, 1);
-                if (!kLast && !(PTSS_ABLATE & 4)) indirectRadiance = scatter(mat, ray, point, normal, cosI);
+                if (!kLast && !(PTSS_ABLATE & 4)) indirectRadiance = scatter(mat, ray, point, normal, cosI, fb.guardFlags);
                 if (inside) {
                     const float4 ab = mat[2];
                     ray.T = ray.T * v3(ptm::exp(-h.distance * ab.x), ptm::exp(-h.distance * ab.y),
diff --git a/cuda-path-tracer-ss_amd/host/host_capi.cpp b/cuda-path-tracer-ss_amd/host/host_capi.cpp
--- a/cuda-path-tracer-ss_amd/host/host_capi.cpp
+++ b/cuda-path-tracer-ss_amd/host/host_capi.cpp
@@ -116,6 +116,33 @@
         ++n;
     }
     return n;
+}
+
+int ptss_probe_guard(int op, const float* x, unsigned int* out, size_t n) {
+    if (!x || !out || op < 0 || op > 3) return PTSS_HOST_EINVAL;
+    for (size_t i = 0; i < n; ++i) {
+        switch (op) {
+            case 0: out[i] = ptm::fast_numerator(x[i]) ? 1u : 0u; break;
+            case 1: out[i] = ptm::fast_divisor(x[i]) ? 1u : 0u; break;
+            case 2: out[i] = ptm::fast_rcp_operand(x[i]) ? 1u : 0u; break;
+            default: out[i] = ptm::in_light_window(x[i]) ? 1u : 0u; break;
+        }
+    }
+    return PTSS_HOST_OK;
+}
+
+int ptss_probe_guard_constants(float* out9) {
+    if (!out9) return PTSS_HOST_EINVAL;
+    const float k[9] = {ptm::kSqrtLo, ptm::kSqrtHi, ptm::kRcpLo, ptm::kRcpHi, ptm::kDivLo, ptm::kDivHi, ptm::kLightD2Lo, ptm::kLightD2Hi,
+                        ptm::kFourPi};
+    for (int i = 0; i < 9; ++i) out9[i] = k[i];
+    return PTSS_HOST_OK;
+}
+
+int ptss_probe_scene_guard_flags(const ptss_scene_desc* scene, unsigned int* out) {
+    if (!scene || !out) return PTSS_HOST_EINVAL;
+    *out = ptpack::sceneGuardFlags(*scene);
+    return PTSS_HOST_OK;
 }
 
 int ptss_probe_math(int op, const float* x, const float* y, float* out, size_t n) {
diff --git a/cuda-path-tracer-ss_amd/ptss.py b/cuda-path-tracer-ss_amd/ptss.py
--- a/cuda-path-tracer-ss_amd/ptss.py
+++ b/cuda-path-tracer-ss_amd/ptss.py
@@ -122,6 +122,9 @@
         L.ptss_tile_rows.argtypes = [C.c_int, C.c_int, C.c_int, C.c_int, C.POINTER(C.c_int), C.c_int]
         L.ptss_probe_math.argtypes = [C.c_int, _f32p, _f32p, _f32p, C.c_size_t]
         L.ptss_probe_quantize.argtypes = [_f32p, C.POINTER(C.c_uint), C.c_size_t]
+        L.ptss_probe_guard.argtypes = [C.c_int, _f32p, C.POINTER(C.c_uint), C.c_size_t]
+        L.ptss_probe_guard_constants.argtypes = [_f32p]
+        L.ptss_probe_scene_guard_flags.argtypes = [C.POINTER(SceneDesc), C.POINTER(C.c_uint)]
         L.ptss_probe_triangle_forms.argtypes = [_f32p, _f32p, _f32p, _f32p, C.c_int, C.c_size_t, C.POINTER(C.c_int), _f32p, _f32p]
         L.ptss_probe_quant_table.argtypes = [_f32p]
         L.ptss_probe_rng_init.argtypes = [C.c_ulonglong, C.c_uint, _u32p]
@@ -200,6 +203,7 @@
         L.ptss_guard_timeouts.argtypes = [vp, C.POINTER(C.c_uint)]
         L.ptss_bounce_kernel_time.argtypes = [vp, C.POINTER(C.c_double), C.POINTER(C.c_ulonglong)]
         L.ptss_launched_kernels.argtypes = [vp, C.POINTER(C.c_ulonglong)]
+        L.ptss_guard_flags.argtypes = [vp, C.POINTER(C.c_uint)]
         L.ptss_debug_counters.argtypes = [vp, C.POINTER(C.c_ulonglong)]
         L.ptss_triangle_leaves.argtypes = [vp, C.POINTER(C.c_int)]
         L.ptss_intersect.argtypes = [vp, vp, vp, C.c_size_t, vp]
@@ -744,6 +748,11 @@
         v = C.c_ulonglong()
         _check(device_lib().ptss_launched_kernels(self._ctx, C.byref(v)))
         return decode_launched_kernels(v.value)
+
+    def guard_flags(self):
+        v = C.c_uint()
+        _check(device_lib().ptss_guard_flags(self._ctx, C.byref(v)))
+        return v.value
 
     def set_scene(self, scene):
         _check(device_lib().ptss_set_scene(self._ctx, C.byref(scene.desc)))
diff --git a/include/ptss.h b/include/ptss.h
--- a/include/ptss.h
+++ b/include/ptss.h
@@ -77,6 +77,8 @@
 
 int ptss_launched_kernels(const ptss_context* ctx, unsigned long long* out);
 
+int ptss_guard_flags(const ptss_context* ctx, unsigned int* out);
+
 int ptss_intersect(ptss_context* ctx, const ptss_ray_query* dev_rays, ptss_ray_hit* dev_hits, size_t n, void* hipStream);
 int ptss_occluded(ptss_context* ctx, const ptss_ray_query* dev_rays, uint32_t* dev_occluded, size_t n, void* hipStream);
 
diff --git a/include/ptss_host.h b/include/ptss_host.h
--- a/include/ptss_host.h
+++ b/include/ptss_host.h
@@ -28,6 +28,9 @@
 int ptss_tile_rows(int height, int band_rows, int rank, int world, int* rows, int cap);
 
 int ptss_probe_math(int op, const float* x, const float* y, float* out, size_t n);
+int ptss_probe_guard(int op, const float* x, unsigned int* out, size_t n);
+int ptss_probe_guard_constants(float* out9);
+int ptss_probe_scene_guard_flags(const ptss_scene_desc* scene, unsigned int* out);
 int ptss_probe_quantize(const float* x, unsigned int* out, size_t n);
 int ptss_probe_quant_table(float* out257);
 int ptss_probe_triangle_forms(const float* tri9, const float* o3, const float* d3, const float* limit, int primary, size_t n, int* cls,
```

New measurement: 18840 Mrays/s (median of 6 runs). 1.02x the previous value.
